# jinlinyi/PerspectiveFields

Hardware: NVIDIA H100
Metric: images/sec at 640x480 (Paramnet-360Cities-edina), H100 vs ref CPU (higher is better)
Workload: dtype f32 via 3x bf16 split MMA, fp32 accumulate

## Files before the change

### include/pf_b200.h

```cpp
#ifndef PF_B200_H_
#define PF_B200_H_

#include <stddef.h>
#include <stdint.h>

#ifdef __cplusplus
extern "C" {
#endif

#define PF_ABI_VERSION 2

typedef struct pf_engine* pf_handle;

enum pf_status { PF_OK = 0, PF_ERR_ARG = -1, PF_ERR_CUDA = -2, PF_ERR_WEIGHT = -3, PF_ERR_WORKSPACE = -4 };

enum pf_dtype { PF_F32 = 0, PF_BF16 = 1 };

enum pf_param_net { PF_PARAM_NONE = 0, PF_PARAM_CENTERED = 1 , PF_PARAM_UNCENTERED = 2  };

typedef struct pf_model_desc {
  int gravity_classes;
  int latitude_classes;
  int param_net;
  int param_input_size;
  float pixel_mean[3];
  float pixel_std[3];
} pf_model_desc;

typedef struct pf_batch {
  int n;
  const uint8_t* images_u8;
  const int64_t* image_offset;
  const float* images_chw;
  const int32_t* height;
  const int32_t* width;
  float* pred_gravity;
  float* pred_latitude;
  float* gravity_original;
  const int64_t* gravity_original_offset;
  float* latitude_original;
  const int64_t* latitude_original_offset;
  float* params;
} pf_batch;

int pf_abi_version(void);
const char* pf_last_error(void);

int64_t pf_kernel_launch_count(void);

int pf_create(int device, const pf_model_desc* desc, pf_handle* out);
int pf_destroy(pf_handle h);

int pf_set_weight(pf_handle h, const char* name, const void* dev_ptr, int64_t numel, int dtype);
int pf_finalize(pf_handle h);

int64_t pf_workspace_bytes(pf_handle h, int n, int max_h);

int pf_forward(pf_handle h, const pf_batch* batch, void* workspace, int64_t workspace_bytes, void* stream);

int pf_profile_enable(pf_handle h, int on );
int pf_profile_read(pf_handle h, double* out21);
int pf_profile_kernels_enable(pf_handle h, int max_launches);
int pf_profile_kernels_read(pf_handle h, char* buf, int cap);

int pf_set_option(pf_handle h, const char* name, int value);

int pf_debug_enable(pf_handle h, int on);
int pf_debug_count(pf_handle h);
const char* pf_debug_name(pf_handle h, int i);
int64_t pf_debug_numel(pf_handle h, const char* name);
int pf_debug_copy(pf_handle h, const char* name, float* dst_dev, int64_t numel, void* stream);

typedef struct pf_camera {
  int32_t height, width;
  double focal_rel;
  double elevation, roll;
  double cx_rel, cy_rel;
  int64_t up_offset;
  int64_t lat_offset;
} pf_camera;
int pf_camera_fields(int device, const pf_camera* cams, int n, float* up, float* lat, void* stream);

typedef struct pf_comm* pf_comm_handle;
int pf_comm_unique_id(void* id128);
int pf_comm_create(int device, int rank, int nranks, const void* id128, pf_comm_handle* out);
int pf_comm_destroy(pf_comm_handle c);
int pf_gather(pf_comm_handle c, int root, int count, void* const* dev_ptrs, const int64_t* bytes, const int32_t* peer, void* stream);

typedef struct pf_jpeg* pf_jpeg_handle;
int pf_jpeg_create(int device, int max_threads , pf_jpeg_handle* out);
int pf_jpeg_destroy(pf_jpeg_handle j);
int pf_jpeg_info(pf_jpeg_handle j, const uint8_t* data, int64_t length, int32_t* height, int32_t* width);
int pf_jpeg_decode_batch(pf_jpeg_handle j, int n, const uint8_t* const* data, const int64_t* length, const int32_t* height,
                         const int32_t* width, uint8_t* blob, const int64_t* offset, void* stream);


int pf_op_conv_gemm(const float* x, int B, int H, int W, int Cin, const void* whi, const void* wlo, const float* bias,
                    int N, int KH, int KW, int stride, int pad, int in_relu, int act, const float* res, int res_relu,
                    float* y, void* stream);
typedef struct pf_tma_pred { const float* w; const float* b; float* out; int nc, mode; } pf_tma_pred;
typedef struct pf_tma_op {
  int mode;
  int64_t M; int K;
  int B, H, W, Cin;
  int N, groups;
  const void* a_hi; const void* a_lo; int lda, a_c0, a_gc;
  const void* a2_hi; const void* a2_lo; int lda2, c_split, a2_c0;
  const void* w_hi; const void* w_lo; const float* bias; int bias_mode, bias_gstride;
  int act; const float* gamma;
  const float* res; int ldr, r_coff, r_gcoff, res_relu;
  const float* res2; int ldr2, r2_coff, r2_gcoff;
  float* C; int ldc, c_coff, c_gcoff;
  void* s_hi; void* s_lo; int lds, s_coff, s_gcoff, split_relu;
  int phase4;
  int npred; pf_tma_pred pred[2];
  int force_bn, force_kb;
  int picked_bn, picked_kb;
} pf_tma_op;
int pf_op_tma(pf_tma_op* op, void* stream);
int pf_op_conv1_ring(const void* c_hi, const void* c_lo, int B, int H, int W, const float* wf, const float* bias, float* out,
                     const float* pg_w, const float* pg_b, float* pg_out, const float* pl_w, const float* pl_b, float* pl_out, void* stream);
int pf_tma_pick_tile(int mode, int64_t M, int N, int K, int sm_count, int* bn, int* kb);
int pf_op_layernorm(const float* x, float* y, int64_t rows, int C, const float* w, const float* b, float eps, void* stream);
int pf_op_attention(const float* q, const float* kv, float* out, int B, int N, int C, int heads, void* stream);
int pf_op_attention_mma(const float* q, const float* kv, float* out, int B, int N, int C, int heads, void* stream);
int pf_op_attention_tc(const float* q, const float* kv, float* out, int B, int N, int C, int heads, void* stream);
int pf_op_dwconv3x3_gelu(const float* x, float* y, int B, int H, int W, int C, const float* w9c, const float* bias, void* stream);
int pf_op_dwconv7x7(const float* x, float* y, int B, int H, int W, int C, const float* w49c, const float* bias, void* stream);
int pf_op_upsample2x(const float* x, float* y, int B, int H, int W, int C, void* stream);
int pf_op_preprocess(const uint8_t* img_dev, int H, int W, const float* mean3, const float* std3, float* y, void* stream);
int pf_op_resize_u8(const uint8_t* img_dev, int H, int W, int new_h, int new_w, uint8_t* out_dev, void* stream);
int pf_op_resize_f32(const float* img_dev, int H, int W, int C, int new_h, int new_w, float* out_dev, void* stream);
int pf_op_fill_stream(float* dst, int64_t numel, float value, void* stream);
int pf_op_argmax_decode(const float* logits, float* field, int B, int HW, int NC, int is_gravity, void* stream);
int pf_op_pred_argmax_decode(const float* feat, int ld, int coff, const float* w, const float* bias, float* field, int B, int HW, int NC,
                             int is_gravity, void* stream);
int pf_op_postprocess(const float* vec, const float* lat, int n, const int32_t* height, const int32_t* width,
                      float* gravity_original, const int64_t* gravity_original_offset, float* latitude_original,
                      const int64_t* latitude_original_offset, int lat_is_sin, void* stream);

#ifdef __cplusplus
}
#endif
#endif
```

### perspectivefields_b200/_native.py

```python
import ctypes
import os
import subprocess

_HERE = os.path.dirname(os.path.abspath(__file__))
ROOT = os.path.dirname(_HERE)
LIB_PATH = os.path.join(_HERE, "libpf_b200.so")
SRC_DIR = os.path.join(_HERE, "csrc")
HEADER = os.path.join(ROOT, "include", "pf_b200.h")

PF_F32, PF_BF16 = 0, 1
PF_PARAM_NONE, PF_PARAM_CENTERED, PF_PARAM_UNCENTERED = 0, 1, 2

NVCC_FLAGS = ["-gencode", "arch=compute_90a,code=sm_90a", "-O3", "-lineinfo", "-std=c++17",
              "-Xcompiler", "-fPIC", "-shared", "-ldl"]


class pf_model_desc(ctypes.Structure):
    _fields_ = [("gravity_classes", ctypes.c_int), ("latitude_classes", ctypes.c_int), ("param_net", ctypes.c_int),
                ("param_input_size", ctypes.c_int), ("pixel_mean", ctypes.c_float * 3), ("pixel_std", ctypes.c_float * 3)]


class pf_camera(ctypes.Structure):
    _fields_ = [("height", ctypes.c_int32), ("width", ctypes.c_int32), ("focal_rel", ctypes.c_double), ("elevation", ctypes.c_double),
                ("roll", ctypes.c_double), ("cx_rel", ctypes.c_double), ("cy_rel", ctypes.c_double),
                ("up_offset", ctypes.c_int64), ("lat_offset", ctypes.c_int64)]


class pf_batch(ctypes.Structure):
    _fields_ = [("n", ctypes.c_int),
                ("images_u8", ctypes.c_void_p), ("image_offset", ctypes.POINTER(ctypes.c_int64)),
                ("images_chw", ctypes.c_void_p),
                ("height", ctypes.POINTER(ctypes.c_int32)), ("width", ctypes.POINTER(ctypes.c_int32)),
                ("pred_gravity", ctypes.c_void_p), ("pred_latitude", ctypes.c_void_p),
                ("gravity_original", ctypes.c_void_p), ("gravity_original_offset", ctypes.POINTER(ctypes.c_int64)),
                ("latitude_original", ctypes.c_void_p), ("latitude_original_offset", ctypes.POINTER(ctypes.c_int64)),
                ("params", ctypes.c_void_p)]


class pf_tma_pred(ctypes.Structure):
    _fields_ = [("w", ctypes.c_void_p), ("b", ctypes.c_void_p), ("out", ctypes.c_void_p), ("nc", ctypes.c_int), ("mode", ctypes.c_int)]


def _fields(spec):
    types = {"int": ctypes.c_int, "ptr": ctypes.c_void_p, "i64": ctypes.c_int64}
    out = []
    for decl in spec.split(";"):
        t, names = decl.split(None, 1)
        out += [(n.strip(), types[t]) for n in names.split(",")]
    return out


class pf_tma_op(ctypes.Structure):
    _fields_ = _fields("int mode; i64 M; int K, B, H, W, Cin, N, groups; ptr a_hi, a_lo; int lda, a_c0, a_gc; ptr a2_hi, a2_lo;"
                       "int lda2, c_split, a2_c0; ptr w_hi, w_lo, bias; int bias_mode, bias_gstride, act; ptr gamma, res;"
                       "int ldr, r_coff, r_gcoff, res_relu; ptr res2; int ldr2, r2_coff, r2_gcoff; ptr C; int ldc, c_coff, c_gcoff;"
                       "ptr s_hi, s_lo; int lds, s_coff, s_gcoff, split_relu, phase4, npred") + \
        [("pred", pf_tma_pred * 2)] + _fields("int force_bn, force_kb, picked_bn, picked_kb")


def _sources():
    return sorted(os.path.join(SRC_DIR, f) for f in os.listdir(SRC_DIR) if f.endswith((".cu", ".cuh"))) + [HEADER]


def needs_build():
    if not os.path.exists(LIB_PATH):
        return True
    t = os.path.getmtime(LIB_PATH)
    return any(os.path.getmtime(s) > t for s in _sources())


def build(force=False, verbose=False):
    if not force and not needs_build():
        return LIB_PATH
    nvcc = os.environ.get("NVCC", "/usr/local/cuda/bin/nvcc")
    cmd = [nvcc] + NVCC_FLAGS + [os.path.join(SRC_DIR, "pf_b200.cu"), "-o", LIB_PATH + ".tmp"]
    if verbose:
        cmd.insert(1, "-Xptxas=-v")
    r = subprocess.run(cmd, capture_output=True, text=True)
    if r.returncode != 0:
        raise RuntimeError("nvcc failed:\n" + " ".join(cmd) + "\n" + r.stdout + r.stderr)
    os.replace(LIB_PATH + ".tmp", LIB_PATH)
    if verbose:
        print(r.stderr)
    return LIB_PATH


_lib = None


def lib():
    global _lib
    if _lib is not None:
        return _lib
    if not os.path.exists(LIB_PATH):
        raise RuntimeError(f"{LIB_PATH} is missing: run `python -c 'import __graft_entry__ as g; g.build()'` "
                           "(perspectivefields_b200 has no CPU or PyTorch fallback)")
    L = ctypes.CDLL(os.environ.get("PF_B200_LIB") or LIB_PATH)
    vp, i32, i64, f32 = ctypes.c_void_p, ctypes.c_int, ctypes.c_int64, ctypes.c_float
    sig = {
        "pf_abi_version": (i32, []),
        "pf_last_error": (ctypes.c_char_p, []),
        "pf_kernel_launch_count": (i64, []),
        "pf_create": (i32, [i32, ctypes.POINTER(pf_model_desc), ctypes.POINTER(vp)]),
        "pf_destroy": (i32, [vp]),
        "pf_set_weight": (i32, [vp, ctypes.c_char_p, vp, i64, i32]),
        "pf_finalize": (i32, [vp]),
        "pf_workspace_bytes": (i64, [vp, i32, i32]),
        "pf_forward": (i32, [vp, ctypes.POINTER(pf_batch), vp, i64, vp]),
        "pf_profile_enable": (i32, [vp, i32]),
        "pf_profile_read": (i32, [vp, ctypes.POINTER(ctypes.c_double)]),
        "pf_profile_kernels_enable": (i32, [vp, i32]),
        "pf_profile_kernels_read": (i32, [vp, ctypes.c_char_p, i32]),
        "pf_debug_enable": (i32, [vp, i32]),
        "pf_debug_count": (i32, [vp]),
        "pf_debug_name": (ctypes.c_char_p, [vp, i32]),
        "pf_debug_numel": (i64, [vp, ctypes.c_char_p]),
        "pf_debug_copy": (i32, [vp, ctypes.c_char_p, vp, i64, vp]),
        "pf_op_conv_gemm": (i32, [vp, i32, i32, i32, i32, vp, vp, vp, i32, i32, i32, i32, i32, i32, i32, vp, i32, vp, vp]),
        "pf_op_tma": (i32, [ctypes.POINTER(pf_tma_op), vp]),
        "pf_op_conv1_ring": (i32, [vp, vp, i32, i32, i32, vp, vp, vp, vp, vp, vp, vp, vp, vp, vp]),
        "pf_tma_pick_tile": (i32, [i32, i64, i32, i32, i32, ctypes.POINTER(i32), ctypes.POINTER(i32)]),
        "pf_set_option": (i32, [vp, ctypes.c_char_p, i32]),
        "pf_camera_fields": (i32, [i32, ctypes.POINTER(pf_camera), i32, vp, vp, vp]),
        "pf_op_layernorm": (i32, [vp, vp, i64, i32, vp, vp, f32, vp]),
        "pf_op_attention": (i32, [vp, vp, vp, i32, i32, i32, i32, vp]),
        "pf_op_attention_mma": (i32, [vp, vp, vp, i32, i32, i32, i32, vp]),
        "pf_op_attention_tc": (i32, [vp, vp, vp, i32, i32, i32, i32, vp]),
        "pf_op_dwconv3x3_gelu": (i32, [vp, vp, i32, i32, i32, i32, vp, vp, vp]),
        "pf_op_dwconv7x7": (i32, [vp, vp, i32, i32, i32, i32, vp, vp, vp]),
        "pf_op_upsample2x": (i32, [vp, vp, i32, i32, i32, i32, vp]),
        "pf_op_preprocess": (i32, [vp, i32, i32, ctypes.POINTER(f32), ctypes.POINTER(f32), vp, vp]),
        "pf_op_resize_u8": (i32, [vp, i32, i32, i32, i32, vp, vp]),
        "pf_op_resize_f32": (i32, [vp, i32, i32, i32, i32, i32, vp, vp]),
        "pf_op_argmax_decode": (i32, [vp, vp, i32, i32, i32, i32, vp]),
        "pf_op_fill_stream": (i32, [vp, i64, f32, vp]),
        "pf_op_pred_argmax_decode": (i32, [vp, i32, i32, vp, vp, vp, i32, i32, i32, i32, vp]),
        "pf_op_postprocess": (i32, [vp, vp, i32, ctypes.POINTER(ctypes.c_int32), ctypes.POINTER(ctypes.c_int32), vp, ctypes.POINTER(i64), vp,
                                    ctypes.POINTER(i64), i32, vp]),
        "pf_comm_unique_id": (i32, [vp]),
        "pf_comm_create": (i32, [i32, i32, i32, vp, ctypes.POINTER(vp)]),
        "pf_comm_destroy": (i32, [vp]),
        "pf_gather": (i32, [vp, i32, i32, ctypes.POINTER(vp), ctypes.POINTER(i64), ctypes.POINTER(ctypes.c_int32), vp]),
        "pf_jpeg_create": (i32, [i32, i32, ctypes.POINTER(vp)]),
        "pf_jpeg_destroy": (i32, [vp]),
        "pf_jpeg_info": (i32, [vp, vp, i64, ctypes.POINTER(ctypes.c_int32), ctypes.POINTER(ctypes.c_int32)]),
        "pf_jpeg_decode_batch": (i32, [vp, i32, ctypes.POINTER(vp), ctypes.POINTER(i64), ctypes.POINTER(ctypes.c_int32),
                                       ctypes.POINTER(ctypes.c_int32), vp, ctypes.POINTER(i64), vp]),
    }
    for name, (res, args) in sig.items():
        try:
            fn = getattr(L, name)
        except AttributeError:
            if os.environ.get("PF_B200_LIB"):
                continue
            raise
        fn.restype, fn.argtypes = res, args
    if L.pf_abi_version() != 2:
        raise RuntimeError("libpf_b200.so ABI version mismatch")
    _lib = L
    return L


EXPORTS = ["pf_abi_version", "pf_last_error", "pf_kernel_launch_count", "pf_create", "pf_destroy", "pf_set_weight",
           "pf_finalize", "pf_workspace_bytes", "pf_forward", "pf_profile_enable", "pf_profile_read", "pf_profile_kernels_enable",
           "pf_profile_kernels_read", "pf_set_option", "pf_debug_enable", "pf_debug_count", "pf_debug_name", "pf_debug_numel",
           "pf_debug_copy", "pf_camera_fields", "pf_comm_unique_id", "pf_comm_create", "pf_comm_destroy", "pf_gather",
           "pf_jpeg_create", "pf_jpeg_destroy", "pf_jpeg_info", "pf_jpeg_decode_batch",
           "pf_op_conv_gemm", "pf_op_tma", "pf_op_conv1_ring", "pf_tma_pick_tile", "pf_op_layernorm", "pf_op_attention", "pf_op_attention_mma", "pf_op_attention_tc", "pf_op_dwconv3x3_gelu", "pf_op_dwconv7x7",
           "pf_op_upsample2x", "pf_op_preprocess", "pf_op_fill_stream", "pf_op_resize_u8", "pf_op_resize_f32", "pf_op_argmax_decode",
           "pf_op_pred_argmax_decode", "pf_op_postprocess"]


class PfError(RuntimeError):
    pass


def check(status):
    if status < 0:
        raise PfError(f"libpf_b200: {lib().pf_last_error().decode()} (status {status})")
    return status
```

### perspectivefields_b200/csrc/gemm_tma.cuh

```cuda
#pragma once
#include <cuda.h>

#include "tc_ptx.cuh"

namespace pf {

constexpr int MODE_GEMM = 0, MODE_HALO = 1;
constexpr int kTmaThreads = 384;
constexpr int kHaloBytes = 180 * 128;

struct TmaGemmParams {
  int M;
  int B, H, W;
  int Cin;
  int N, K;
  int a_c0, a_gc;
  int c_split, a2_c0;
  int groups;
  int b_row0;
  const float* bias; int bias_mode, bias_gstride;
  int act; const float* gamma;
  const float* res;  int ldr, r_coff, r_gcoff, res_relu;
  const float* res2; int ldr2, r2_coff, r2_gcoff;
  float* C; int ldc, c_coff, c_gcoff;
  __nv_bfloat16* Shi; __nv_bfloat16* Slo; int lds, s_coff, s_gcoff, split_relu;
  const float* pred_w; const float* pred_b; float* pred_out; int pred_nc, pred_mode;
  int phase4;
};

template <int BN, int MODE, int KB> struct TmaCfg {
  static_assert(KB == 32 || KB == 64, "KB");
  static_assert(BN % 32 == 0 && BN <= 256, "BN");
  static constexpr int kBPlane = BN * KB * 2;
  static constexpr int kAPlane = 128 * KB * 2;
  static constexpr int kStage = (MODE == MODE_GEMM ? 2 * kAPlane : 0) + 2 * kBPlane;
  static constexpr int kABuf = 2 * kHtPlaneBytes;
  static constexpr int kAccPitch = 68;
  static constexpr int kAccStage = 2 * 64 * kAccPitch * 4;
  static constexpr int kBudget = 225 * 1024 - kAccStage - (MODE == MODE_HALO ? 2 * kABuf : 0);
  static constexpr int kStagesRaw = kBudget / kStage;
  static constexpr int kStages = kStagesRaw > 16 ? 16 : kStagesRaw;
  static constexpr int kSmemBytes = (MODE == MODE_HALO ? 2 * kABuf : 0) + kStages * kStage + kAccStage + 512 + 1024;
  static_assert(kStages >= 2, "ring too shallow");
  static_assert(kSmemBytes <= 227 * 1024, "shared memory per block");
};

__device__ __forceinline__ void mbar_expect_tx(uint32_t bar, uint32_t bytes) {
  asm volatile("mbarrier.arrive.expect_tx.shared::cta.b64 _, [%0], %1;\n" ::"r"(bar), "r"(bytes) : "memory");
}
__device__ __forceinline__ void tma_load_2d(uint32_t dst, const CUtensorMap* map, uint32_t bar, int c0, int c1) {
  asm volatile("cp.async.bulk.tensor.2d.shared::cluster.global.mbarrier::complete_tx::bytes [%0], [%1, {%3, %4}], [%2];\n"
               ::"r"(dst), "l"(reinterpret_cast<uint64_t>(map)), "r"(bar), "r"(c0), "r"(c1) : "memory");
}
__device__ __forceinline__ void tma_load_4d(uint32_t dst, const CUtensorMap* map, uint32_t bar, int c0, int c1, int c2, int c3) {
  asm volatile("cp.async.bulk.tensor.4d.shared::cluster.global.mbarrier::complete_tx::bytes [%0], [%1, {%3, %4, %5, %6}], [%2];\n"
               ::"r"(dst), "l"(reinterpret_cast<uint64_t>(map)), "r"(bar), "r"(c0), "r"(c1), "r"(c2), "r"(c3) : "memory");
}
__device__ __forceinline__ void tma_prefetch_desc(const CUtensorMap* map) {
  asm volatile("prefetch.tensormap [%0];\n" ::"l"(reinterpret_cast<uint64_t>(map)) : "memory");
}

struct TmaMaps {
  CUtensorMap a_hi, a_lo, a2_hi, a2_lo, b_hi, b_lo;
};

template <int BN, int MODE, int KB>
__global__ void __launch_bounds__(kTmaThreads, 1) gemm_tma_kernel(const __grid_constant__ TmaMaps maps, const TmaGemmParams p, int tiles_x, int tiles_y) {
  using Cfg = TmaCfg<BN, MODE, KB>;
  constexpr int NS = Cfg::kStages;
  constexpr int SPC = 9 * (64 / KB);
  constexpr int kConsumerWarps = 8;
  extern __shared__ unsigned char smem_dyn[];
  const uint32_t raw = smem_u32(smem_dyn);
  const uint32_t sbase = (raw + 1023u) & ~1023u;
  unsigned char* sm = smem_dyn + (sbase - raw);
  const uint32_t a_base = sbase;
  const uint32_t ring = sbase + (MODE == MODE_HALO ? 2 * Cfg::kABuf : 0);
  const uint32_t acc_base = ring + NS * Cfg::kStage;
  const uint32_t bars = acc_base + Cfg::kAccStage;
  auto full_b = [&](int s) { return bars + 8u * s; };
  auto empty_b = [&](int s) { return bars + 8u * (NS + s); };
  auto full_a = [&](int i) { return bars + 8u * (2 * NS + i); };
  auto empty_a = [&](int i) { return bars + 8u * (2 * NS + 2 + i); };

  const int tid = threadIdx.x, lane = tid & 31, warp = tid >> 5;
  const int n_tiles = cdiv(p.N, BN);
  const int m_tiles = MODE == MODE_GEMM ? cdiv(p.M, 128) : p.B * tiles_x * tiles_y;
  const int total_tiles = m_tiles * n_tiles * p.groups;
  const int nchunks = MODE == MODE_HALO ? p.Cin / 64 : 0;
  const int nk = MODE == MODE_GEMM ? p.K / KB : nchunks * SPC;
  const bool b_resident = MODE == MODE_HALO && nchunks == 1 && SPC <= NS;

  if (tid == 0) {
    tma_prefetch_desc(&maps.a_hi); tma_prefetch_desc(&maps.a_lo); tma_prefetch_desc(&maps.b_hi); tma_prefetch_desc(&maps.b_lo);
    for (int s = 0; s < NS; ++s) { mbar_init(full_b(s), 1); mbar_init(empty_b(s), kConsumerWarps); }
    for (int i = 0; i < 2; ++i) { mbar_init(full_a(i), 1); mbar_init(empty_a(i), kConsumerWarps); }
    fence_mbar_init();
  }
  __syncthreads();
  pdl_wait();
  pdl_launch();

  auto decode = [&](int tile, int& mt, int& g, int& n0) {
    n0 = (tile % n_tiles) * BN;
    tile /= n_tiles;
    g = tile % p.groups;
    mt = tile / p.groups;
  };

  if (warp < 4) {
    asm volatile("setmaxnreg.dec.sync.aligned.u32 40;\n");
    if (warp == 0 && lane == 0) {
      int it = 0;
      for (int tile = blockIdx.x; tile < total_tiles; tile += gridDim.x) {
        int mt, g, n0;
        decode(tile, mt, g, n0);
        const int brow = p.b_row0 + g * p.N + n0;
        if (b_resident && it > 0) break;
        for (int kc = 0; kc < nk; ++kc, ++it) {
          const int s = it % NS;
          mbar_wait(empty_b(s), ((it / NS) & 1) ^ 1);
          mbar_expect_tx(full_b(s), Cfg::kStage);
          const uint32_t st = ring + s * Cfg::kStage;
          int kcol;
          if (MODE == MODE_GEMM) {
            kcol = kc * KB;
            tma_load_2d(st, &maps.a_hi, full_b(s), p.a_c0 + g * p.a_gc + kcol, mt * 128);
            tma_load_2d(st + Cfg::kAPlane, &maps.a_lo, full_b(s), p.a_c0 + g * p.a_gc + kcol, mt * 128);
          } else {
            const int c = kc / SPC, u = kc - c * SPC;
            kcol = KB == 32 ? (u >> 1) * p.Cin + c * 64 + (u & 1) * 32 : u * p.Cin + c * 64;
          }
          const uint32_t bdst = st + (MODE == MODE_GEMM ? 2 * Cfg::kAPlane : 0);
          tma_load_2d(bdst, &maps.b_hi, full_b(s), kcol, brow);
          tma_load_2d(bdst + Cfg::kBPlane, &maps.b_lo, full_b(s), kcol, brow);
        }
      }
    } else if (MODE == MODE_HALO && warp == 1 && lane == 0) {
      int ita = 0;
      for (int tile = blockIdx.x; tile < total_tiles; tile += gridDim.x) {
        int mt, g, n0;
        decode(tile, mt, g, n0);
        const int tx = mt % tiles_x, ty = (mt / tiles_x) % tiles_y, bimg = mt / (tiles_x * tiles_y);
        for (int c = 0; c < nchunks; ++c, ++ita) {
          const int buf = ita & 1;
          mbar_wait(empty_a(buf), ((ita >> 1) & 1) ^ 1);
          mbar_expect_tx(full_a(buf), 2 * kHaloBytes);
          const uint32_t dst = a_base + buf * Cfg::kABuf;
          const int ci = c * 64;
          if (p.c_split > 0 && ci >= p.c_split) {
            tma_load_4d(dst, &maps.a2_hi, full_a(buf), p.a2_c0 + ci - p.c_split, tx * kHtTileW - 1, ty * kHtTileH - 1, bimg);
            tma_load_4d(dst + kHtPlaneBytes, &maps.a2_lo, full_a(buf), p.a2_c0 + ci - p.c_split, tx * kHtTileW - 1, ty * kHtTileH - 1, bimg);
          } else {
            tma_load_4d(dst, &maps.a_hi, full_a(buf), p.a_c0 + g * p.a_gc + ci, tx * kHtTileW - 1, ty * kHtTileH - 1, bimg);
            tma_load_4d(dst + kHtPlaneBytes, &maps.a_lo, full_a(buf), p.a_c0 + g * p.a_gc + ci, tx * kHtTileW - 1, ty * kHtTileH - 1, bimg);
          }
        }
      }
    }
    return;
  }

  asm volatile("setmaxnreg.inc.sync.aligned.u32 232;\n");
  const int wg = (warp >> 2) - 1;
  const int wt = tid & 127;
  float* stage = reinterpret_cast<float*>(sm + (acc_base - sbase)) + wg * 64 * Cfg::kAccPitch;
  const int erow = wt & 63, eh = wt >> 6;
  const int r = wg * 64 + erow;
  float acc[BN / 2];
  int it = 0, ita = 0;
  for (int tile = blockIdx.x, tl = 0; tile < total_tiles; tile += gridDim.x, ++tl) {
    int mt, g, n0;
    decode(tile, mt, g, n0);
    int prev_s = -1, prev_buf = -1;
    fence_regs(acc);
    for (int kc = 0; kc < nk; ++kc, ++it) {
      const int s = it % NS;
      uint32_t a_hi, a_lo;
      bool chunk_end = false;
      int buf = 0;
      if (MODE == MODE_HALO) {
        const int c = kc / SPC, u = kc - c * SPC;
        const int tap = KB == 32 ? (u >> 1) : u, ky = tap / 3, kx = tap - ky * 3;
        buf = ita & 1;
        if (u == 0) mbar_wait(full_a(buf), (ita >> 1) & 1);
        a_hi = a_base + buf * Cfg::kABuf + ((ky + 8 * wg) * kHtHaloW + kx) * 128 + (KB == 32 ? (u & 1) * 64 : 0);
        a_lo = a_hi + kHtPlaneBytes;
        chunk_end = u == SPC - 1;
      } else {
        a_hi = ring + s * Cfg::kStage + wg * 64 * KB * 2;
        a_lo = a_hi + Cfg::kAPlane;
      }
      const int sb = b_resident ? kc : s;
      if (!b_resident || tl == 0) mbar_wait(full_b(sb), b_resident ? 0 : ((it / NS) & 1));
      const uint32_t b_hi = ring + sb * Cfg::kStage + (MODE == MODE_GEMM ? 2 * Cfg::kAPlane : 0);
      const uint64_t dah = MODE == MODE_HALO ? ht_a_desc(a_hi) : wgmma_tile_desc<KB>(a_hi);
      const uint64_t dal = MODE == MODE_HALO ? ht_a_desc(a_lo) : wgmma_tile_desc<KB>(a_lo);
      const uint64_t dbh = wgmma_tile_desc<KB>(b_hi);
      const uint64_t dbl = wgmma_tile_desc<KB>(b_hi + Cfg::kBPlane);
      constexpr uint64_t kChunk = (uint64_t)(64 * KB * 2) >> 4;
      wgmma_fence();
#pragma unroll
      for (int kk = 0; kk < KB / 16; ++kk) {
        const uint32_t first = (kc | kk) ? 1u : 0u;
#pragma unroll
        for (int j = 0; j < BN / 64; ++j) {
          wgmma_n64(acc + 32 * j, dal + 2 * kk, dbh + 2 * kk + j * kChunk, first);
          wgmma_n64(acc + 32 * j, dah + 2 * kk, dbl + 2 * kk + j * kChunk, 1u);
          wgmma_n64(acc + 32 * j, dah + 2 * kk, dbh + 2 * kk + j * kChunk, 1u);
        }
        if constexpr (BN % 64 != 0) {
          constexpr int j = BN / 64;
          wgmma_n32(acc + 32 * j, dal + 2 * kk, dbh + 2 * kk + j * kChunk, first);
          wgmma_n32(acc + 32 * j, dah + 2 * kk, dbl + 2 * kk + j * kChunk, 1u);
          wgmma_n32(acc + 32 * j, dah + 2 * kk, dbh + 2 * kk + j * kChunk, 1u);
        }
      }
      wgmma_commit();
      wgmma_wait<1>();
      if (lane == 0 && prev_s >= 0) {
        if (!b_resident) mbar_arrive(empty_b(prev_s));
        if (MODE == MODE_HALO && prev_buf >= 0) mbar_arrive(empty_a(prev_buf));
      }
      prev_s = s;
      prev_buf = chunk_end ? buf : -1;
      if (MODE == MODE_HALO && chunk_end) ++ita;
    }
    wgmma_wait<0>();
    fence_regs(acc);
    if (lane == 0 && prev_s >= 0) {
      if (!b_resident) mbar_arrive(empty_b(prev_s));
      if (MODE == MODE_HALO && prev_buf >= 0) mbar_arrive(empty_a(prev_buf));
    }

    long long m;
    bool valid;
    int cls_off = 0;
    int bimg = 0, oy = 0, ox = 0;
    if (MODE == MODE_GEMM) {
      m = (long long)mt * 128 + r;
      valid = m < p.M;
    } else {
      const int tx = mt % tiles_x, ty = (mt / tiles_x) % tiles_y;
      bimg = mt / (tiles_x * tiles_y);
      oy = ty * kHtTileH + (r >> 3); ox = tx * kHtTileW + (r & 7);
      valid = oy < p.H && ox < p.W;
      m = ((long long)bimg * p.H + oy) * p.W + ox;
      if (p.bias_mode == 2) {
        const int ry = oy == 0 ? 0 : (oy == p.H - 1 ? 2 : 1);
        const int rx = ox == 0 ? 0 : (ox == p.W - 1 ? 2 : 1);
        cls_off = (ry * 3 + rx) * p.N;
      }
    }
    const float* __restrict__ bias = p.bias ? p.bias + (long long)g * p.bias_gstride : nullptr;
    const int frow = (wt >> 5) * 16 + (lane >> 2), fcol = 2 * (lane & 3);
#pragma unroll
    for (int rd = 0; rd < (BN + 63) / 64; ++rd) {
      named_bar_sync(1 + wg, 128);
#pragma unroll
      for (int jb = 0; jb < 8; ++jb) {
        const int cb = rd * 8 + jb;
        if (cb < BN / 8) {
          float* d0 = stage + frow * Cfg::kAccPitch + jb * 8 + fcol;
          *reinterpret_cast<float2*>(d0) = make_float2(acc[4 * cb], acc[4 * cb + 1]);
          *reinterpret_cast<float2*>(d0 + 8 * Cfg::kAccPitch) = make_float2(acc[4 * cb + 2], acc[4 * cb + 3]);
        }
      }
      named_bar_sync(1 + wg, 128);
      const int ch = 2 * rd + eh;
      if (ch >= BN / 32) continue;
      const int nb = n0 + ch * 32;
      const bool ph4 = MODE == MODE_HALO && BN == 128 && p.phase4;
      const long long mo = ph4 ? ((long long)bimg * 2 * p.H + 2 * oy + (ch >> 1)) * (2 * p.W) + 2 * ox + (ch & 1) : m;
      const int nbo = ph4 ? 0 : nb;
      const bool chunk_ok = nb < p.N;
      float o[32];
      const float* srow = stage + erow * Cfg::kAccPitch + eh * 32;
#pragma unroll
      for (int j = 0; j < 32; j += 4) {
        const float4 t = *reinterpret_cast<const float4*>(srow + j);
        o[j] = t.x; o[j + 1] = t.y; o[j + 2] = t.z; o[j + 3] = t.w;
      }
      if (valid && chunk_ok) {
        if (p.bias_mode) {
#pragma unroll
          for (int j = 0; j < 32; j += 4) {
            const float4 bv = __ldg(reinterpret_cast<const float4*>(bias + cls_off + nb + j));
            o[j] += bv.x; o[j + 1] += bv.y; o[j + 2] += bv.z; o[j + 3] += bv.w;
          }
        }
        if (p.act == 1) {
#pragma unroll
          for (int j = 0; j < 32; ++j) o[j] = fmaxf(o[j], 0.f);
        } else if (p.act == 2) {
#pragma unroll
          for (int j = 0; j < 32; ++j) o[j] = gelu_erf(o[j]);
        }
        if (p.gamma) {
#pragma unroll
          for (int j = 0; j < 32; j += 4) {
            const float4 gv = __ldg(reinterpret_cast<const float4*>(p.gamma + nb + j));
            o[j] *= gv.x; o[j + 1] *= gv.y; o[j + 2] *= gv.z; o[j + 3] *= gv.w;
          }
        }
        if (p.res) {
          const float* rp = p.res + m * p.ldr + p.r_coff + g * p.r_gcoff + nb;
#pragma unroll
          for (int j = 0; j < 32; j += 4) {
            float4 rv = *reinterpret_cast<const float4*>(rp + j);
            if (p.res_relu) { rv.x = fmaxf(rv.x, 0.f); rv.y = fmaxf(rv.y, 0.f); rv.z = fmaxf(rv.z, 0.f); rv.w = fmaxf(rv.w, 0.f); }
            o[j] += rv.x; o[j + 1] += rv.y; o[j + 2] += rv.z; o[j + 3] += rv.w;
          }
        }
        if (p.res2) {
          const float* rp = p.res2 + m * p.ldr2 + p.r2_coff + g * p.r2_gcoff + nb;
#pragma unroll
          for (int j = 0; j < 32; j += 4) {
            const float4 rv = *reinterpret_cast<const float4*>(rp + j);
            o[j] += rv.x; o[j + 1] += rv.y; o[j + 2] += rv.z; o[j + 3] += rv.w;
          }
        }
        if (MODE == MODE_HALO && (BN == 32 || BN == 128) && p.pred_w) {
          float v0 = __ldg(p.pred_b), v1 = p.pred_nc > 1 ? __ldg(p.pred_b + 1) : 0.f;
#pragma unroll
          for (int j = 0; j < 32; j += 4) {
            const float4 w0 = __ldg(reinterpret_cast<const float4*>(p.pred_w + j));
            v0 = fmaf(o[j], w0.x, v0); v0 = fmaf(o[j + 1], w0.y, v0); v0 = fmaf(o[j + 2], w0.z, v0); v0 = fmaf(o[j + 3], w0.w, v0);
            if (p.pred_nc > 1) {
              const float4 w1 = __ldg(reinterpret_cast<const float4*>(p.pred_w + 32 + j));
              v1 = fmaf(o[j], w1.x, v1); v1 = fmaf(o[j + 1], w1.y, v1); v1 = fmaf(o[j + 2], w1.z, v1); v1 = fmaf(o[j + 3], w1.w, v1);
            }
          }
          const long long HWl = (long long)p.H * p.W * (ph4 ? 4 : 1);
          const long long bi = mo / HWl, pix = mo - bi * HWl;
          float* po = p.pred_out + bi * p.pred_nc * HWl + pix;
          if (p.pred_mode == 1) {
            const float nrm = fmaxf(sqrtf(v0 * v0 + v1 * v1), 1e-12f);
            po[0] = v0 / nrm; po[HWl] = v1 / nrm;
          } else {
            po[0] = fminf(fmaxf(v0, -1.f), 1.f);
          }
        }
      }
      if (chunk_ok && (p.C || p.Shi)) {
        const bool odd = lane & 1;
        const bool valid_p = __shfl_xor_sync(0xffffffffu, (int)valid, 1) != 0;
        const long long mo_p = mo + (odd ? -1 : 1) * (ph4 ? 2 : 1);
        const long long moA = odd ? mo_p : mo, moB = odd ? mo : mo_p;
        const bool vA = odd ? valid_p : valid, vB = odd ? valid : valid_p;
        if (p.C) {
          float* cA = p.C + moA * p.ldc + p.c_coff + g * p.c_gcoff + nbo + (odd ? 4 : 0);
          float* cB = p.C + moB * p.ldc + p.c_coff + g * p.c_gcoff + nbo + (odd ? 4 : 0);
#pragma unroll
          for (int t = 0; t < 4; ++t) {
            float k[4], rr[4];
#pragma unroll
            for (int e = 0; e < 4; ++e) {
              k[e] = odd ? o[8 * t + 4 + e] : o[8 * t + e];
              rr[e] = __shfl_xor_sync(0xffffffffu, odd ? o[8 * t + e] : o[8 * t + 4 + e], 1);
            }
            if (vA) *reinterpret_cast<float4*>(cA + 8 * t) = odd ? make_float4(rr[0], rr[1], rr[2], rr[3]) : make_float4(k[0], k[1], k[2], k[3]);
            if (vB) *reinterpret_cast<float4*>(cB + 8 * t) = odd ? make_float4(k[0], k[1], k[2], k[3]) : make_float4(rr[0], rr[1], rr[2], rr[3]);
          }
        }
        if (p.Shi) {
          const long long sA = moA * p.lds + p.s_coff + g * p.s_gcoff + nbo + (odd ? 8 : 0);
          const long long sB = moB * p.lds + p.s_coff + g * p.s_gcoff + nbo + (odd ? 8 : 0);
#pragma unroll
          for (int t = 0; t < 2; ++t) {
            float k[8], rr[8];
#pragma unroll
            for (int e = 0; e < 8; ++e) {
              const float mine = odd ? o[16 * t + 8 + e] : o[16 * t + e], give = odd ? o[16 * t + e] : o[16 * t + 8 + e];
              k[e] = p.split_relu ? fmaxf(mine, 0.f) : mine;
              rr[e] = __shfl_xor_sync(0xffffffffu, p.split_relu ? fmaxf(give, 0.f) : give, 1);
            }
            uint4 kh, kl, rh, rl;
            split_bf16x2(k[0], k[1], kh.x, kl.x); split_bf16x2(k[2], k[3], kh.y, kl.y);
            split_bf16x2(k[4], k[5], kh.z, kl.z); split_bf16x2(k[6], k[7], kh.w, kl.w);
            split_bf16x2(rr[0], rr[1], rh.x, rl.x); split_bf16x2(rr[2], rr[3], rh.y, rl.y);
            split_bf16x2(rr[4], rr[5], rh.z, rl.z); split_bf16x2(rr[6], rr[7], rh.w, rl.w);
            if (vA) {
              *reinterpret_cast<uint4*>(p.Shi + sA + 16 * t) = odd ? rh : kh;
              *reinterpret_cast<uint4*>(p.Slo + sA + 16 * t) = odd ? rl : kl;
            }
            if (vB) {
              *reinterpret_cast<uint4*>(p.Shi + sB + 16 * t) = odd ? kh : rh;
              *reinterpret_cast<uint4*>(p.Slo + sB + 16 * t) = odd ? kl : rl;
            }
          }
        }
      }
    }
  }
}

}
```

### perspectivefields_b200/csrc/pf_b200.cu

```cuda
#include "../../include/pf_b200.h"

#include <cuda_runtime.h>
#include <nvtx3/nvToolsExt.h>

#include <atomic>
#include <cctype>
#include <cmath>
#include <cstdarg>
#include <cstdio>
#include <cstdlib>
#include <cstring>
#include <map>
#include <mutex>
#include <string>
#include <functional>
#include <unordered_map>
#include <vector>

#include "common.cuh"
#include "tma_host.cuh"
#include "attention_mma.cuh"
#include "layers.cuh"
#include "prepost.cuh"
#include "comm.cuh"
#include "jpeg.cuh"

using namespace pf;

static thread_local std::string g_err;
static std::atomic<long long> g_launches{0};

static int fail(int code, const char* fmt, ...) {
  char buf[1024];
  va_list ap;
  va_start(ap, fmt);
  vsnprintf(buf, sizeof(buf), fmt, ap);
  va_end(ap);
  g_err = buf;
  return code;
}
#define CU(expr)                                                                                    \
  do {                                                                                              \
    cudaError_t e__ = (expr);                                                                       \
    if (e__ != cudaSuccess) return fail(PF_ERR_CUDA, "%s: %s (%s:%d)", #expr, cudaGetErrorString(e__), __FILE__, __LINE__); \
  } while (0)
static char g_crumb[96] = "";
static bool sync_debug() {
  static int v = -1;
  if (v < 0) v = getenv("PF_SYNC_DEBUG") ? 1 : 0;
  return v == 1;
}
struct KernelProf {
  bool on = false;
  cudaStream_t st = nullptr;
  std::vector<cudaEvent_t> pool;
  size_t used = 0;
  struct Rec { const char* expr; cudaEvent_t a, b; };
  std::vector<Rec> recs;
  cudaEvent_t next() { return used < pool.size() ? pool[used++] : nullptr; }
};
static thread_local KernelProf* tl_kp = nullptr;
#define LAUNCHED(expr)                                                                              \
  do {                                                                                              \
    KernelProf* kp__ = tl_kp;                                                                       \
    cudaEvent_t ka__ = (kp__ && kp__->on) ? kp__->next() : nullptr;                                 \
    if (ka__) cudaEventRecord(ka__, kp__->st);                                                      \
    cudaError_t e__ = (expr);                                                                       \
    g_launches.fetch_add(1, std::memory_order_relaxed);                                             \
    if (ka__) {                                                                                     \
      cudaEvent_t kb__ = kp__->next();                                                              \
      if (kb__) { cudaEventRecord(kb__, kp__->st); kp__->recs.push_back({#expr, ka__, kb__}); }     \
    }                                                                                               \
    if (e__ == cudaSuccess && sync_debug()) e__ = cudaDeviceSynchronize();                          \
    if (e__ != cudaSuccess) return fail(PF_ERR_CUDA, "%s: %s (%s:%d, after tap '%s')", #expr, cudaGetErrorString(e__), __FILE__, __LINE__, g_crumb); \
  } while (0)
struct NvtxRange {
  explicit NvtxRange(const char* name) { nvtxRangePushA(name); }
  ~NvtxRange() { nvtxRangePop(); }
};
#define TRY(expr)                \
  do {                           \
    int r__ = (expr);            \
    if (r__ != PF_OK) return r__; \
  } while (0)

static const int kMitDims[4] = {64, 128, 320, 512};
static const int kMitHeads[4] = {1, 2, 5, 8};
static const int kMitDepths[4] = {3, 4, 18, 3};
static const int kMitSr[4] = {8, 4, 2, 1};
static const int kMitRes[4] = {80, 40, 20, 10};
static const int kCnxDims[4] = {96, 192, 384, 768};
static const int kCnxDepths[4] = {3, 3, 9, 3};

struct WeightRef { const void* p; long long numel; int dtype; };
struct GemmW { const __nv_bfloat16* hi = nullptr; const __nv_bfloat16* lo = nullptr; const float* b = nullptr; };
struct LnW { const float* w = nullptr; const float* b = nullptr; };

struct MitBlockW { LnW ln1, srln, ln2; GemmW q, sr, kv, proj, fc1, fc2; const float* dw_w; const float* dw_b; };
struct CnxBlockW { const float* dw_w; const float* dw_b; LnW ln; GemmW pw1, pw2; const float* gamma; };

struct Arena {
  char* base = nullptr;
  long long cap = 0, off = 0, peak = 0;
  bool dry = false, keep = false;
  void* alloc(long long bytes) {
    off = (off + 255) & ~255LL;
    void* p = dry ? nullptr : base + off;
    off += bytes;
    if (off > peak) peak = off;
    return p;
  }
  float* f(long long n) { return (float*)alloc(n * 4); }
  long long mark() const { return off; }
  void release(long long m) { if (!keep) off = m; }
};

struct pf_engine {
  int device = 0;
  pf_model_desc desc{};
  bool finalized = false;
  std::unordered_map<std::string, WeightRef> weights;
  const float *embed1_w, *embed1_b, *llenc_w, *llenc_b;
  LnW embed_ln[4], stage_norm[4];
  GemmW embed[4];
  GemmW embed1g, llencg;
  std::vector<MitBlockW> blocks[4];
  GemmW proc[4];
  GemmW rcu[4][2][2];
  GemmW conv0, conv1;
  GemmW conv1p;
  const float *conv1f_w, *conv1f_b;
  bool use_fork = false;
  cudaStream_t side = nullptr;
  cudaEvent_t ev_fork = nullptr, ev_join = nullptr;
  bool use_dwln = false;
  bool use_pdl = true;
  bool decode_only = false;
  bool use_attn_split = true;
  bool use_phase = true;
  const float *pred_g_w, *pred_g_b, *pred_l_w, *pred_l_b;
  const float *pn_stem_w, *pn_stem_b;
  LnW pn_stem_ln, pn_ds_ln[4], pn_norm;
  GemmW pn_ds[4];
  std::vector<CnxBlockW> pn_blocks[4];
  const float *pn_head_w, *pn_head_b;
  struct DevTable { int ksize; int* bounds; int* coeffs; };
  std::map<int, DevTable> tables;
  char* table_dev = nullptr;
  char* table_host = nullptr;
  long long table_off = 0;
  KernelProf kp;
  struct MapKey {
    const void* base; long long d0, d1, d2; int kind, box, kb;
    bool operator==(const MapKey& o) const { return base == o.base && d0 == o.d0 && d1 == o.d1 && d2 == o.d2 && kind == o.kind && box == o.box && kb == o.kb; }
  };
  struct MapKeyHash {
    size_t operator()(const MapKey& k) const {
      size_t h = std::hash<const void*>()(k.base);
      for (long long v : {k.d0, k.d1, k.d2, (long long)k.kind, (long long)k.box, (long long)k.kb}) h = h * 1000003u ^ std::hash<long long>()(v);
      return h;
    }
  };
  std::unordered_map<MapKey, CUtensorMap, MapKeyHash> map_cache;
  bool use_stem_tc = true;
  bool use_attn_mma = true;
  int sm_count = 132;
  bool profile = false;
  struct ProfRec { cudaEvent_t a, b; double flops; int cfg; int M, N, K, KH, stride, groups, Cin; };
  std::vector<ProfRec> prof;
  std::vector<cudaEvent_t> ev_pool;
  bool debug = false;
  std::vector<std::pair<std::string, std::pair<const float*, long long>>> taps;
};

static int get_w(pf_engine* e, const std::string& name, int dtype, long long numel, const void** out) {
  auto it = e->weights.find(name);
  if (it == e->weights.end()) return fail(PF_ERR_WEIGHT, "missing weight '%s'", name.c_str());
  if (it->second.dtype != dtype) return fail(PF_ERR_WEIGHT, "weight '%s': wrong dtype", name.c_str());
  if (it->second.numel != numel) return fail(PF_ERR_WEIGHT, "weight '%s': numel %lld, expected %lld", name.c_str(), it->second.numel, numel);
  *out = it->second.p;
  return PF_OK;
}
static int get_f(pf_engine* e, const std::string& n, long long numel, const float** out) { return get_w(e, n, PF_F32, numel, (const void**)out); }
static int get_gemm(pf_engine* e, const std::string& n, long long N, long long K, long long nbias, GemmW* g, int groups = 1) {
  TRY(get_w(e, n + ".whi", PF_BF16, groups * N * K, (const void**)&g->hi));
  TRY(get_w(e, n + ".wlo", PF_BF16, groups * N * K, (const void**)&g->lo));
  TRY(get_f(e, n + ".b", groups * nbias, &g->b));
  return PF_OK;
}
static int get_ln(pf_engine* e, const std::string& n, int C, LnW* l) {
  TRY(get_f(e, n + ".w", C, &l->w));
  TRY(get_f(e, n + ".b", C, &l->b));
  return PF_OK;
}

static int resolve_weights(pf_engine* e) {
  char nm[128];
  TRY(get_f(e, "embed1.w", 147 * 64, &e->embed1_w));
  TRY(get_f(e, "embed1.b", 64, &e->embed1_b));
  TRY(get_f(e, "llenc.w", 147 * 64, &e->llenc_w));
  TRY(get_f(e, "llenc.b", 64, &e->llenc_b));
  TRY(get_gemm(e, "embed1g", 64, 160, 64, &e->embed1g));
  TRY(get_gemm(e, "llencg", 64, 160, 64, &e->llencg));
  for (int s = 0; s < 4; ++s) {
    const int C = kMitDims[s];
    snprintf(nm, sizeof nm, "embed%d.ln", s + 1);
    TRY(get_ln(e, nm, C, &e->embed_ln[s]));
    if (s > 0) {
      snprintf(nm, sizeof nm, "embed%d", s + 1);
      TRY(get_gemm(e, nm, C, 9LL * kMitDims[s - 1], C, &e->embed[s]));
    }
    e->blocks[s].resize(kMitDepths[s]);
    for (int i = 0; i < kMitDepths[s]; ++i) {
      MitBlockW& b = e->blocks[s][i];
      char p[64];
      snprintf(p, sizeof p, "s%d.b%d.", s + 1, i);
      std::string P(p);
      TRY(get_ln(e, P + "ln1", C, &b.ln1));
      TRY(get_gemm(e, P + "q", C, C, C, &b.q));
      if (kMitSr[s] > 1) {
        TRY(get_gemm(e, P + "sr", C, (long long)kMitSr[s] * kMitSr[s] * C, C, &b.sr));
        TRY(get_ln(e, P + "srln", C, &b.srln));
      }
      TRY(get_gemm(e, P + "kv", 2 * C, C, 2 * C, &b.kv));
      TRY(get_gemm(e, P + "proj", C, C, C, &b.proj));
      TRY(get_ln(e, P + "ln2", C, &b.ln2));
      TRY(get_gemm(e, P + "fc1", 4 * C, C, 4 * C, &b.fc1));
      TRY(get_f(e, P + "dw.w", 9LL * 4 * C, &b.dw_w));
      TRY(get_f(e, P + "dw.b", 4 * C, &b.dw_b));
      TRY(get_gemm(e, P + "fc2", C, 4 * C, C, &b.fc2));
    }
    snprintf(nm, sizeof nm, "s%d.norm", s + 1);
    TRY(get_ln(e, nm, C, &e->stage_norm[s]));
  }
  for (int l = 0; l < 4; ++l) {
    snprintf(nm, sizeof nm, "head.proc%d", l + 1);
    TRY(get_gemm(e, nm, 512, 9LL * kMitDims[l], 9 * 512, &e->proc[l]));
  }
  for (int f = 0; f < 4; ++f)
    for (int u = 0; u < 2; ++u) {
      if (f == 3 && u == 0) continue;
      for (int c = 0; c < 2; ++c) {
        snprintf(nm, sizeof nm, "head.f%d.u%d.c%d", f + 1, u + 1, c + 1);
        TRY(get_gemm(e, nm, 256, 2304, 256, &e->rcu[f][u][c], 2));
      }
    }
  TRY(get_gemm(e, "head.conv0", 64, 9 * 320, 64, &e->conv0, 2));
  TRY(get_gemm(e, "head.conv1", 32, 9 * 64, 32, &e->conv1, 2));
  TRY(get_gemm(e, "head.conv1p", 128, 9 * 64, 128, &e->conv1p, 2));
  TRY(get_f(e, "head.conv1f.w", 2LL * 9 * 64 * 32, &e->conv1f_w));
  TRY(get_f(e, "head.conv1f.b", 64, &e->conv1f_b));
  TRY(get_f(e, "head.pred_g.w", 32LL * e->desc.gravity_classes, &e->pred_g_w));
  TRY(get_f(e, "head.pred_g.b", e->desc.gravity_classes, &e->pred_g_b));
  TRY(get_f(e, "head.pred_l.w", 32LL * e->desc.latitude_classes, &e->pred_l_w));
  TRY(get_f(e, "head.pred_l.b", e->desc.latitude_classes, &e->pred_l_b));
  if (e->desc.param_net != PF_PARAM_NONE) {
    TRY(get_f(e, "pn.stem.w", 48 * 96, &e->pn_stem_w));
    TRY(get_f(e, "pn.stem.b", 96, &e->pn_stem_b));
    TRY(get_ln(e, "pn.stem.ln", 96, &e->pn_stem_ln));
    for (int k = 1; k < 4; ++k) {
      snprintf(nm, sizeof nm, "pn.ds%d.ln", k);
      TRY(get_ln(e, nm, kCnxDims[k - 1], &e->pn_ds_ln[k]));
      snprintf(nm, sizeof nm, "pn.ds%d", k);
      TRY(get_gemm(e, nm, kCnxDims[k], 4LL * kCnxDims[k - 1], kCnxDims[k], &e->pn_ds[k]));
    }
    for (int s = 0; s < 4; ++s) {
      const int C = kCnxDims[s];
      e->pn_blocks[s].resize(kCnxDepths[s]);
      for (int j = 0; j < kCnxDepths[s]; ++j) {
        CnxBlockW& b = e->pn_blocks[s][j];
        char p[64];
        snprintf(p, sizeof p, "pn.s%d.b%d.", s, j);
        std::string P(p);
        TRY(get_f(e, P + "dw.w", 49LL * C, &b.dw_w));
        TRY(get_f(e, P + "dw.b", C, &b.dw_b));
        TRY(get_ln(e, P + "ln", C, &b.ln));
        TRY(get_gemm(e, P + "pw1", 4 * C, C, 4 * C, &b.pw1));
        TRY(get_gemm(e, P + "pw2", C, 4 * C, C, &b.pw2));
        TRY(get_f(e, P + "gamma", C, &b.gamma));
      }
    }
    TRY(get_ln(e, "pn.norm", 768, &e->pn_norm));
    TRY(get_f(e, "pn.head.w", 5 * 768, &e->pn_head_w));
    TRY(get_f(e, "pn.head.b", 5, &e->pn_head_b));
  }
  return PF_OK;
}

struct Fwd {
  pf_engine* e;
  Arena ar;
  cudaStream_t st;
  bool dry;
  int n;

  int tap(const char* name, const float* p, long long numel) {
    if (!e->debug) return PF_OK;
    float* cp = ar.f(numel);
    if (dry) return PF_OK;
    snprintf(g_crumb, sizeof g_crumb, "%s", name);
    if (sync_debug()) fprintf(stderr, "[pf tap] %s cp=%p (+%lld of cap %lld) p=%p numel=%lld\n", name, (void*)cp, (long long)((char*)cp - ar.base), ar.cap, (const void*)p, numel);
    CU(cudaMemcpyAsync(cp, p, numel * 4, cudaMemcpyDeviceToDevice, st));
    if (sync_debug()) CU(cudaDeviceSynchronize());
    e->taps.push_back({name, {cp, numel}});
    return PF_OK;
  }
  int tapf(const float* p, long long numel, const char* fmt, ...) {
    if (!e->debug) return PF_OK;
    char buf[96];
    va_list ap;
    va_start(ap, fmt);
    vsnprintf(buf, sizeof buf, fmt, ap);
    va_end(ap);
    return tap(buf, p, numel);
  }

  SplitT salloc(long long pixels, int ld) {
    SplitT t;
    t.hi = (__nv_bfloat16*)ar.alloc(pixels * ld * 2);
    t.lo = (__nv_bfloat16*)ar.alloc(pixels * ld * 2);
    t.ld = ld;
    return t;
  }
  int tap_split(const char* name, const SplitT& t, long long numel) {
    if (!e->debug) return PF_OK;
    float* cp = ar.f(numel);
    if (dry) return PF_OK;
    snprintf(g_crumb, sizeof g_crumb, "%s", name);
    LAUNCHED((merge_split_kernel<<<(unsigned)cdivl(numel, 256), 256, 0, st>>>(t.hi, t.lo, cp, numel), cudaGetLastError()));
    e->taps.push_back({name, {cp, numel}});
    return PF_OK;
  }
  static cudaError_t gemm_tma_gemm_mode(const TmaMaps& maps, const TmaGemmParams& p, int bn, int kb, int sms, cudaStream_t st, const PredTail* pred) {
    return gemm_tma_launch(MODE_GEMM, maps, p, bn, kb, sms, st, pred);
  }
  static cudaError_t gemm_tma_halo_mode(const TmaMaps& maps, const TmaGemmParams& p, int bn, int kb, int sms, cudaStream_t st, const PredTail* pred) {
    return gemm_tma_launch(MODE_HALO, maps, p, bn, kb, sms, st, pred);
  }
  int force_bn = 0, force_kb = 0;
  int picked_bn = 0, picked_kb = 0;
  int pick_tile(int mode, const TmaGemmParams& p, const PredTail* pred, int& bn, int& kb) {
    tma_pick_tile(mode, p.M, p.N, p.K, e->sm_count, bn, kb);
    if (force_bn) { bn = force_bn; kb = tma_pick_kb(bn, p.K, mode); }
    if (force_kb) kb = force_kb;
    if (const char* msg = gemm_tma_check(mode, p, bn, kb, pred != nullptr)) return fail(PF_ERR_ARG, "TMA engine, %s (bn %d, kb %d): %s", mode == MODE_GEMM ? "GEMM mode" : "halo mode", bn, kb, msg);
    picked_bn = bn; picked_kb = kb;
    return PF_OK;
  }
  int launch_tma(int mode, const TmaMaps& maps, const TmaGemmParams& p, int bn, int kb, const PredTail* pred = nullptr) {
    if (e->profile) {
      pf_engine::ProfRec r{};
      for (cudaEvent_t* ev : {&r.a, &r.b}) {
        if (e->ev_pool.empty()) { CU(cudaEventCreate(ev)); }
        else { *ev = e->ev_pool.back(); e->ev_pool.pop_back(); }
      }
      const double Mrows = mode == MODE_GEMM ? (double)p.M : (double)p.B * p.H * p.W;
      r.flops = 2.0 * Mrows * (double)p.N * (double)p.K * (double)p.groups;
      r.cfg = mode == MODE_GEMM ? 5 : 6;
      r.M = (int)Mrows; r.N = p.N; r.K = p.K; r.KH = mode == MODE_GEMM ? 1 : 3; r.stride = 1; r.groups = p.groups; r.Cin = p.Cin;
      CU(cudaEventRecord(r.a, st));
      if (mode == MODE_GEMM) LAUNCHED(gemm_tma_gemm_mode(maps, p, bn, kb, e->sm_count, st, pred));
      else LAUNCHED(gemm_tma_halo_mode(maps, p, bn, kb, e->sm_count, st, pred));
      CU(cudaEventRecord(r.b, st));
      e->prof.push_back(r);
      return PF_OK;
    }
    if (mode == MODE_GEMM) LAUNCHED(gemm_tma_gemm_mode(maps, p, bn, kb, e->sm_count, st, pred));
    else LAUNCHED(gemm_tma_halo_mode(maps, p, bn, kb, e->sm_count, st, pred));
    return PF_OK;
  }
  struct Epi {
    float* C = nullptr; int ldc = 0, c_coff = 0, c_gcoff = 0;
    SplitT S; int s_coff = 0, s_gcoff = 0, split_relu = 0;
    int act = 0; const float* gamma = nullptr;
    const float* res = nullptr; int ldr = 0, r_coff = 0, r_gcoff = 0, res_relu = 0;
    const float* res2 = nullptr; int ldr2 = 0, r2_coff = 0, r2_gcoff = 0;
    int bias_mode = 1;
    int phase4 = 0;
  };
  static void fill_epi(TmaGemmParams& p, const GemmW& w, const Epi& o, int bias_gstride) {
    p.bias = w.b; p.bias_mode = w.b ? o.bias_mode : 0; p.bias_gstride = bias_gstride;
    p.act = o.act; p.gamma = o.gamma;
    p.res = o.res; p.ldr = o.ldr; p.r_coff = o.r_coff; p.r_gcoff = o.r_gcoff; p.res_relu = o.res_relu;
    p.res2 = o.res2; p.ldr2 = o.ldr2; p.r2_coff = o.r2_coff; p.r2_gcoff = o.r2_gcoff;
    p.C = o.C; p.ldc = o.ldc; p.c_coff = o.c_coff; p.c_gcoff = o.c_gcoff;
    p.Shi = o.S.hi; p.Slo = o.S.lo; p.lds = o.S.ld; p.s_coff = o.s_coff; p.s_gcoff = o.s_gcoff; p.split_relu = o.split_relu;
    p.phase4 = o.phase4;
  }
  template <class F>
  const char* cached_map(CUtensorMap* out, const pf_engine::MapKey& key, F&& make) {
    auto it = e->map_cache.find(key);
    if (it != e->map_cache.end()) { *out = it->second; return nullptr; }
    const char* msg = make(out);
    if (!msg) {
      if (e->map_cache.size() > 20000) e->map_cache.clear();
      e->map_cache.emplace(key, *out);
    }
    return msg;
  }
  const char* map2d(CUtensorMap* m, const void* base, long long cols, long long rows, long long ld, int box_rows, int kb) {
    return cached_map(m, pf_engine::MapKey{base, cols, rows, ld, 0, box_rows, kb}, [&](CUtensorMap* o) { return tma_map_2d(o, base, cols, rows, ld, box_rows, kb); });
  }
  const char* map_halo(CUtensorMap* m, const void* base, int B, int H, int W, int ld) {
    return cached_map(m, pf_engine::MapKey{base, ((long long)B << 32) | (unsigned)H, W, ld, 3, 0, 0}, [&](CUtensorMap* o) { return tma_map_halo(o, base, B, H, W, ld); });
  }
  int tgemm(const SplitT& A, long long M, int K, int a_c0, const GemmW& w, int N, const Epi& o) {
    if (dry) return PF_OK;
    if (K % 32 || N % 32 || A.ld % 8) return fail(PF_ERR_ARG, "tgemm: K/N must be multiples of 32");
    if (o.res2 || o.bias_mode == 2) return fail(PF_ERR_ARG, "tgemm: second residual / border-class bias are halo-mode features");
    TmaGemmParams p{};
    p.M = (int)M; p.Cin = K; p.N = N; p.K = K; p.a_c0 = a_c0; p.groups = 1;
    fill_epi(p, w, o, 0);
    TmaMaps maps{};
    int bn, kb;
    TRY(pick_tile(MODE_GEMM, p, nullptr, bn, kb));
    const char* msg = nullptr;
    if (!msg) msg = map2d(&maps.a_hi, A.hi, A.ld, M, A.ld, 128, kb);
    if (!msg) msg = map2d(&maps.a_lo, A.lo, A.ld, M, A.ld, 128, kb);
    if (!msg) msg = map2d(&maps.b_hi, w.hi, K, N, K, bn, kb);
    if (!msg) msg = map2d(&maps.b_lo, w.lo, K, N, K, bn, kb);
    if (msg) return fail(PF_ERR_CUDA, "%s", msg);
    maps.a2_hi = maps.a_hi; maps.a2_lo = maps.a_lo;
    return launch_tma(MODE_GEMM, maps, p, bn, kb);
  }
  int thalo(const SplitT& A, int a_c0, int a_gc, const SplitT* A2, int c_split, int a2_c0, int B, int H, int W, int Cin, const GemmW& w, int N,
            int groups, int bias_gstride, const Epi& o, const PredTail* pred = nullptr) {
    if (dry) return PF_OK;
    if (Cin % 64 || N % 32 || (A2 && c_split % 64)) return fail(PF_ERR_ARG, "thalo: Cin must be a multiple of 64, N of 32");
    if (w.b && o.bias_mode == 2 && (H < 2 || W < 2)) return fail(PF_ERR_ARG, "thalo: border-class bias needs H, W >= 2 (got %dx%d)", H, W);
    TmaGemmParams p{};
    p.B = B; p.H = H; p.W = W; p.Cin = Cin; p.N = N; p.K = 9 * Cin; p.a_c0 = a_c0; p.a_gc = a_gc; p.groups = groups;
    p.c_split = A2 ? c_split : 0; p.a2_c0 = a2_c0;
    fill_epi(p, w, o, bias_gstride);
    TmaMaps maps{};
    int bn, kb;
    TRY(pick_tile(MODE_HALO, p, pred, bn, kb));
    const char* msg = nullptr;
    if (!msg) msg = map_halo(&maps.a_hi, A.hi, B, H, W, A.ld);
    if (!msg) msg = map_halo(&maps.a_lo, A.lo, B, H, W, A.ld);
    if (A2) {
      if (!msg) msg = map_halo(&maps.a2_hi, A2->hi, B, H, W, A2->ld);
      if (!msg) msg = map_halo(&maps.a2_lo, A2->lo, B, H, W, A2->ld);
    } else { maps.a2_hi = maps.a_hi; maps.a2_lo = maps.a_lo; }
    if (!msg) msg = map2d(&maps.b_hi, w.hi, p.K, (long long)groups * N, p.K, bn, kb);
    if (!msg) msg = map2d(&maps.b_lo, w.lo, p.K, (long long)groups * N, p.K, bn, kb);
    if (msg) return fail(PF_ERR_CUDA, "%s", msg);
    return launch_tma(MODE_HALO, maps, p, bn, kb, pred);
  }
  int tconv_gather(const SplitT& A, int B, int H, int W, int Cin, int KH, int stride, int pad, const GemmW& w, int N, const Epi& o) {
    const int OH = (H + 2 * pad - KH) / stride + 1, OW = (W + 2 * pad - KH) / stride + 1;
    const long long M = (long long)B * OH * OW;
    const int K = KH * KH * Cin;
    const long long m = ar.mark();
    SplitT col = salloc(M, K);
    if (!dry) {
      if (Cin % 8) return fail(PF_ERR_ARG, "tconv_gather: Cin %% 8");
      LAUNCHED(launch_pdl(im2col_split_kernel, dim3(ew_grid(M * K / 8)), dim3(256), 0, st, A.hi, A.lo, A.ld, col.hi, col.lo, B, H, W, Cin, OH, OW, KH, stride, pad));
    }
    int r = tgemm(col, M, K, 0, w, N, o);
    ar.release(m);
    return r;
  }
  int ln_split(const float* x, const SplitT& y, long long rows, int C, const LnW& w, float eps, float* yf = nullptr) {
    if (dry) return PF_OK;
    LAUNCHED(layernorm_launch(x, yf, rows, C, w.w, w.b, eps, st, y));
    return PF_OK;
  }
  int ln_split_patch(const float* x, const SplitT& y, const SplitT& patch, long long rows, int C, const LnW& w, float eps, int R, int sr) {
    if (dry) return PF_OK;
    LAUNCHED(layernorm_launch(x, nullptr, rows, C, w.w, w.b, eps, st, y, patch, R, sr));
    return PF_OK;
  }
  int ln(const float* x, float* y, long long rows, int C, const LnW& w, float eps) {
    if (dry) return PF_OK;
    LAUNCHED(layernorm_launch(x, y, rows, C, w.w, w.b, eps, st));
    return PF_OK;
  }
};

constexpr long long kTableSlabBytes = 8LL << 20;
static int get_table(pf_engine* e, int in_size, pf_engine::DevTable* out, cudaStream_t st) {
  auto it = e->tables.find(in_size);
  if (it == e->tables.end()) {
    ResampleTable t = make_resample_table(in_size, kNet);
    const long long nb = (long long)t.bounds.size() * sizeof(int), nc = (long long)t.coeffs.size() * sizeof(int);
    const long long need = ((nb + 255) & ~255LL) + ((nc + 255) & ~255LL);
    if (need > kTableSlabBytes) return fail(PF_ERR_ARG, "image axis of %d pixels is too long for the resize tables", in_size);
    if (e->table_off + need > kTableSlabBytes) {
      CU(cudaStreamSynchronize(st));
      e->tables.clear();
      e->table_off = 0;
    }
    pf_engine::DevTable d{};
    d.ksize = t.ksize;
    const long long o0 = e->table_off, o1 = o0 + ((nb + 255) & ~255LL);
    memcpy(e->table_host + o0, t.bounds.data(), nb);
    memcpy(e->table_host + o1, t.coeffs.data(), nc);
    d.bounds = (int*)(e->table_dev + o0);
    d.coeffs = (int*)(e->table_dev + o1);
    CU(cudaMemcpyAsync(e->table_dev + o0, e->table_host + o0, need, cudaMemcpyHostToDevice, st));
    e->table_off += need;
    it = e->tables.emplace(in_size, d).first;
  }
  *out = it->second;
  return PF_OK;
}

static int pre_rows_needed(int H) {
  const double scale = (double)H / kNet;
  const double support = scale < 1.0 ? 1.0 : scale;
  return (int)(kPreRows * scale) + 2 * (int)ceil(support) + 3;
}
constexpr int kPreMaxSmemRows = 200 * 1024 / (kNet * 3);

static int fwd_preprocess(Fwd& F, const pf_batch* bt, float*& x0, PreImage*& d_pre, PostImage*& d_post) {
  pf_engine* e = F.e;
  const pf_model_desc& D = e->desc;
  const int n = F.n;
  const bool dry = F.dry;
  cudaStream_t st = F.st;
  Arena& ar = F.ar;
  x0 = ar.f((long long)n * kNet * kNet * 4);
  d_pre = (PreImage*)ar.alloc((long long)n * sizeof(PreImage));
  d_post = (PostImage*)ar.alloc((long long)n * sizeof(PostImage));
  if (!dry) {
    if (bt->images_u8) {
      std::vector<PreImage> pre(n);
      int max_h = 1;
      for (int i = 0; i < n; ++i) {
        const int H = bt->height[i], W = bt->width[i];
        if (H < 1 || W < 1) return fail(PF_ERR_ARG, "image %d has size %dx%d", i, H, W);
        pf_engine::DevTable tx, ty;
        TRY(get_table(e, W, &tx, st));
        TRY(get_table(e, H, &ty, st));
        if (ty.ksize + 1 > kPreMaxSmemRows) return fail(PF_ERR_ARG, "image %d is too tall (%d rows) for the resize kernel", i, H);
        pre[i] = PreImage{bt->image_offset[i], H, W, tx.ksize, ty.ksize, tx.bounds, tx.coeffs, ty.bounds, ty.coeffs};
        if (H > max_h) max_h = H;
      }
      CU(cudaMemcpyAsync(d_pre, pre.data(), n * sizeof(PreImage), cudaMemcpyHostToDevice, st));
      int rows = pre_rows_needed(max_h);
      if (rows > kPreMaxSmemRows) rows = kPreMaxSmemRows;
      const int smem = rows * kNet * 3;
      LAUNCHED((preprocess_kernel<<<dim3(kNet / kPreRows, n), kNet, smem, st>>>(bt->images_u8, d_pre, x0, D.pixel_mean[0], D.pixel_mean[1],
                                                                               D.pixel_mean[2], D.pixel_std[0], D.pixel_std[1], D.pixel_std[2], rows),
                cudaGetLastError()));
    } else {
      const long long total = (long long)n * kNet * kNet;
      LAUNCHED((normalize_chw_kernel<<<(unsigned)cdivl(total, 256), 256, 0, st>>>(bt->images_chw, x0, n, D.pixel_mean[0], D.pixel_mean[1],
                                                                                 D.pixel_mean[2], D.pixel_std[0], D.pixel_std[1], D.pixel_std[2]),
                cudaGetLastError()));
    }
  }
  return PF_OK;
}

static int launch_postprocess(const float* vec, const float* lat, int n, const int32_t* height, const int32_t* width, const int64_t* g_off,
                              const int64_t* l_off, float* g_out, float* l_out, int lat_is_sin, PostImage* d_post, cudaStream_t st) {
  std::vector<PostImage> post(n);
  long long total = 0;
  int max_h = 1, max_wp = 4;
  for (int i = 0; i < n; ++i) {
    if (height[i] < 1 || width[i] < 1) return fail(PF_ERR_ARG, "image %d has size %dx%d", i, height[i], width[i]);
    post[i] = PostImage{height[i], width[i], g_off[i], l_off[i], total};
    total += (long long)height[i] * width[i];
    if (height[i] > max_h) max_h = height[i];
    const int wp = (width[i] + 3) / 4 * 4;
    if (wp <= kPostMaxW && wp > max_wp) max_wp = wp;
  }
  CU(cudaMemcpyAsync(d_post, post.data(), n * sizeof(PostImage), cudaMemcpyHostToDevice, st));
  const int smem = max_wp * 8;
  LAUNCHED((postprocess_kernel<<<dim3((unsigned)cdiv(max_h, kPostBand), (unsigned)n), kPostThreads, smem, st>>>(vec, lat, d_post, g_out, l_out, lat_is_sin),
            cudaGetLastError()));
  return PF_OK;
}

static int fwd_tails_post(Fwd& F, const pf_batch* bt, const float* conv1_out, PostImage* d_post, bool pred_done = false) {
  pf_engine* e = F.e;
  const pf_model_desc& D = e->desc;
  const int n = F.n;
  const bool dry = F.dry;
  cudaStream_t st = F.st;
  Arena& ar = F.ar;
  const int HW = kNet * kNet;
  const bool cls_g = D.gravity_classes != 2, cls_l = D.latitude_classes != 1;
  const bool fused_decode = e->decode_only && (cls_g || cls_l);
  if (e->decode_only && cls_g != cls_l) return fail(PF_ERR_ARG, "decode_only needs both heads to be classification heads");
  const float* vec = dry ? nullptr : bt->pred_gravity;
  const float* lat = dry ? nullptr : bt->pred_latitude;
  if (e->debug) {
    float* rg = ar.f((long long)n * D.gravity_classes * HW);
    float* rl = ar.f((long long)n * D.latitude_classes * HW);
    if (!dry) {
      const unsigned grid = (unsigned)cdivl((long long)n * HW, 128);
      LAUNCHED((pred_tail_kernel<<<grid, 128, D.gravity_classes * 33 * 4, st>>>(conv1_out, 64, 0, e->pred_g_w, e->pred_g_b, rg, n, HW, D.gravity_classes, 0), cudaGetLastError()));
      LAUNCHED((pred_tail_kernel<<<grid, 128, D.latitude_classes * 33 * 4, st>>>(conv1_out, 64, 32, e->pred_l_w, e->pred_l_b, rl, n, HW, D.latitude_classes, 0), cudaGetLastError()));
    }
    TRY(F.tap("head.raw_g", rg, (long long)n * D.gravity_classes * HW));
    TRY(F.tap("head.raw_l", rl, (long long)n * D.latitude_classes * HW));
  }
  if (fused_decode) {
    if (!dry) {
      const unsigned grid = ew_grid((long long)n * HW * 4);
      LAUNCHED((pred_argmax_decode_kernel<<<grid, 256, D.gravity_classes * 37 * 4, st>>>(conv1_out, 64, 0, e->pred_g_w, e->pred_g_b, bt->pred_gravity, n, HW,
                                                                                      D.gravity_classes, 1), cudaGetLastError()));
      LAUNCHED((pred_argmax_decode_kernel<<<grid, 256, D.latitude_classes * 37 * 4, st>>>(conv1_out, 64, 32, e->pred_l_w, e->pred_l_b, bt->pred_latitude, n, HW,
                                                                                       D.latitude_classes, 0), cudaGetLastError()));
    }
  } else {
    if (!dry && !pred_done) {
      const unsigned grid = (unsigned)cdivl((long long)n * HW, 128);
      LAUNCHED((pred_tail_kernel<<<grid, 128, D.gravity_classes * 33 * 4, st>>>(conv1_out, 64, 0, e->pred_g_w, e->pred_g_b, bt->pred_gravity, n, HW,
                                                                             D.gravity_classes, D.gravity_classes == 2 ? 1 : 0), cudaGetLastError()));
      LAUNCHED((pred_tail_kernel<<<grid, 128, D.latitude_classes * 33 * 4, st>>>(conv1_out, 64, 32, e->pred_l_w, e->pred_l_b, bt->pred_latitude, n, HW,
                                                                              D.latitude_classes, D.latitude_classes == 1 ? 2 : 0), cudaGetLastError()));
    }
    if (cls_g) {
      float* dv = ar.f((long long)n * 2 * HW);
      if (!dry) LAUNCHED((argmax_decode_kernel<<<(unsigned)cdivl((long long)n * HW, 256), 256, 0, st>>>(bt->pred_gravity, dv, n, HW, D.gravity_classes, 1), cudaGetLastError()));
      vec = dv;
    }
    if (cls_l) {
      float* dl = ar.f((long long)n * HW);
      if (!dry) LAUNCHED((argmax_decode_kernel<<<(unsigned)cdivl((long long)n * HW, 256), 256, 0, st>>>(bt->pred_latitude, dl, n, HW, D.latitude_classes, 0), cudaGetLastError()));
      lat = dl;
    }
  }
  if (!dry)
    TRY(launch_postprocess(vec, lat, n, bt->height, bt->width, bt->gravity_original_offset, bt->latitude_original_offset, bt->gravity_original,
                           bt->latitude_original, cls_l ? 0 : 1, d_post, st));
  return PF_OK;
}

static int run_forward_tma(Fwd& F, const pf_batch* bt) {
  pf_engine* e = F.e;
  const pf_model_desc& D = e->desc;
  const int n = F.n;
  const bool dry = F.dry;
  cudaStream_t st = F.st;
  Arena& ar = F.ar;
  using Epi = Fwd::Epi;

  float* x0; PreImage* d_pre; PostImage* d_post;
  {
    NvtxRange r_("pf:preprocess");
    TRY(fwd_preprocess(F, bt, x0, d_pre, d_post));
  }
  TRY(F.tap("pre", x0, (long long)n * kNet * kNet * 4));

  NvtxRange* sect = new NvtxRange("pf:ll_enc");
  struct SectGuard { NvtxRange*& p; ~SectGuard() { delete p; } } sect_guard{sect};
  auto section = [&](const char* name) { delete sect; sect = nullptr; sect = new NvtxRange(name); };
  SplitT cfeat[4];
  for (int s = 0; s < 4; ++s) cfeat[s] = F.salloc((long long)n * kMitRes[s] * kMitRes[s], kMitDims[s]);
  SplitT ll = F.salloc((long long)n * 160 * 160, 64);
  if (e->use_stem_tc) {
    const long long m = ar.mark();
    const long long M = (long long)n * 160 * 160;
    SplitT col = F.salloc(M, 160);
    if (!dry) LAUNCHED(launch_pdl(stem_gather_kernel, dim3(ew_grid(stem_gather_threads(n, 160, 160))), dim3(256), 0, st, x0, col.hi, col.lo, n, 160, 160, 2));
    Epi o; o.S = ll; o.act = 1;
    TRY(F.tgemm(col, M, 160, 0, e->llencg, 64, o));
    ar.release(m);
  } else if (!dry) {
    LAUNCHED((stem_conv_launch<7, 7, 2, 3, 64>(x0, 4, n, kNet, kNet, e->llenc_w, e->llenc_b, nullptr, 1, st, ll)));
  }
  TRY(F.tap_split("ll", ll, (long long)n * 160 * 160 * 64));

  for (int s = 0; s < 4; ++s) {
    { char nm[32]; snprintf(nm, sizeof nm, "pf:mit.stage%d", s + 1); section(nm); }
    const int C = kMitDims[s], R = kMitRes[s], N = R * R, heads = kMitHeads[s], sr = kMitSr[s];
    const long long rows = (long long)n * N;
    const long long m = ar.mark();
    float* x = ar.f(rows * C);
    float* tf = ar.f(rows * C);
    SplitT t1 = F.salloc(rows, C);
    SplitT t1p;
    if (sr > 1) t1p = F.salloc((long long)n * 100, sr * sr * C);
    SplitT q = F.salloc(rows, C);
    SplitT a = F.salloc(rows, C);
    float* t2f = ar.f((long long)n * 100 * C);
    SplitT t2 = F.salloc((long long)n * 100, C);
    SplitT kv = F.salloc((long long)n * 100, 2 * C);
    const bool qkv_split = e->use_attn_mma && e->use_attn_split;
    float* qf = qkv_split ? nullptr : ar.f(rows * C);
    float* kvf = qkv_split ? nullptr : ar.f((long long)n * 100 * 2 * C);
    float* h1 = ar.f(rows * 4 * C);
    SplitT h2 = F.salloc(rows, 4 * C);
    if (s == 0 && e->use_stem_tc) {
      const long long mm = ar.mark();
      SplitT col = F.salloc(rows, 160);
      if (!dry) LAUNCHED(launch_pdl(stem_gather_kernel, dim3(ew_grid(stem_gather_threads(n, 80, 80))), dim3(256), 0, st, x0, col.hi, col.lo, n, 80, 80, 4));
      Epi o; o.C = tf; o.ldc = C;
      TRY(F.tgemm(col, rows, 160, 0, e->embed1g, 64, o));
      ar.release(mm);
    } else if (s == 0) {
      if (!dry) LAUNCHED((stem_conv_launch<7, 7, 4, 3, 64>(x0, 4, n, kNet, kNet, e->embed1_w, e->embed1_b, tf, 0, st)));
    } else {
      Epi o; o.C = tf; o.ldc = C;
      TRY(F.tconv_gather(cfeat[s - 1], n, kMitRes[s - 1], kMitRes[s - 1], kMitDims[s - 1], 3, 2, 1, e->embed[s], C, o));
    }
    TRY(F.ln(tf, x, rows, C, e->embed_ln[s], 1e-5f));
    TRY(F.tapf(x, rows * C, "mit.s%d.embed", s + 1));
    for (int i = 0; i < kMitDepths[s]; ++i) {
      const MitBlockW& b = e->blocks[s][i];
      if (sr > 1) TRY(F.ln_split_patch(x, t1, t1p, rows, C, b.ln1, 1e-6f, R, sr));
      else TRY(F.ln_split(x, t1, rows, C, b.ln1, 1e-6f));
      Epi oq, okv;
      if (qkv_split) { oq.S = q; okv.S = kv; } else { oq.C = qf; oq.ldc = C; okv.C = kvf; okv.ldc = 2 * C; }
      const bool fork = !dry && sr > 1 && e->use_fork && e->side && !e->kp.on && !e->profile && !sync_debug() && !e->debug;
      if (fork) {
        CU(cudaEventRecord(e->ev_fork, st));
        CU(cudaStreamWaitEvent(e->side, e->ev_fork, 0));
        F.st = e->side;
      }
      if (sr > 1) {
        { Epi o; o.C = t2f; o.ldc = C; TRY(F.tgemm(t1p, (long long)n * 100, sr * sr * C, 0, b.sr, C, o)); }
        TRY(F.ln_split(t2f, t2, (long long)n * 100, C, b.srln, 1e-5f));
        TRY(F.tgemm(t2, (long long)n * 100, C, 0, b.kv, 2 * C, okv));
      }
      if (fork) {
        CU(cudaEventRecord(e->ev_join, e->side));
        F.st = st;
      }
      TRY(F.tgemm(t1, rows, C, 0, b.q, C, oq));
      if (fork) CU(cudaStreamWaitEvent(st, e->ev_join, 0));
      if (sr > 1) {
      } else {
        TRY(F.tgemm(t1, rows, C, 0, b.kv, 2 * C, okv));
      }
      if (!dry) {
        if (qkv_split) LAUNCHED(attention_mma_launch(nullptr, nullptr, nullptr, n, N, C, heads, st, a, q, kv));
        else if (e->use_attn_mma) LAUNCHED(attention_mma_launch(qf, kvf, nullptr, n, N, C, heads, st, a));
        else LAUNCHED(attention_launch(qf, kvf, nullptr, n, N, C, heads, st, a));
      }
      { Epi o; o.C = x; o.ldc = C; o.res = x; o.ldr = C; TRY(F.tgemm(a, rows, C, 0, b.proj, C, o)); }
      TRY(F.tapf(x, rows * C, "mit.s%d.b%d.attn", s + 1, i));
      TRY(F.ln_split(x, t1, rows, C, b.ln2, 1e-6f));
      { Epi o; o.C = h1; o.ldc = 4 * C; TRY(F.tgemm(t1, rows, C, 0, b.fc1, 4 * C, o)); }
      if (!dry) LAUNCHED(launch_pdl(dwconv3x3_gelu_kernel, dim3(ew_grid((long long)n * ((R + 1) / 2) * ((R + PF_DW3_PX - 1) / PF_DW3_PX) * C)), dim3(256), 0, st, h1, nullptr, n, R, R, 4 * C, b.dw_w, b.dw_b, h2.hi, h2.lo));
      { Epi o; o.C = x; o.ldc = C; o.res = x; o.ldr = C; TRY(F.tgemm(h2, rows, 4 * C, 0, b.fc2, C, o)); }
      TRY(F.tapf(x, rows * C, "mit.s%d.b%d", s + 1, i));
    }
    TRY(F.ln_split(x, cfeat[s], rows, C, e->stage_norm[s], 1e-6f));
    { char nm[32]; snprintf(nm, sizeof nm, "mit.c%d", s + 1); TRY(F.tap_split(nm, cfeat[s], rows * C)); }
    ar.release(m);
  }

  float* conv1_out = ar.f((long long)n * kNet * kNet * 64);
  bool fuse_pred = false;
  {
    const long long m = ar.mark();
    float* fused = nullptr;
    SplitT fused_s;
    for (int lvl = 4; lvl >= 1; --lvl) {
      { char nm[32]; snprintf(nm, sizeof nm, "pf:heads.level%d", lvl); section(nm); }
      const int r = kMitRes[lvl - 1], Cin = kMitDims[lvl - 1];
      const long long px = (long long)n * r * r;
      float* t = ar.f(px * 512);
      SplitT rt = F.salloc(px, 512);
      SplitT u = F.salloc(px, 512);
      float* v = ar.f(px * 512);
      SplitT rv = F.salloc(px, 512);
      float* w2 = ar.f(px * 512);
      {
        Epi o; o.C = t; o.ldc = 512; o.S = rt; o.split_relu = 1; o.bias_mode = 2;
        TRY(F.thalo(cfeat[lvl - 1], 0, 0, nullptr, 0, 0, n, r, r, Cin, e->proc[lvl - 1], 512, 1, 0, o));
        TRY(F.tapf(t, px * 512, "head.proc%d", lvl));
      }
      auto rcu = [&](const SplitT& A, const GemmW& w, Epi o) {
        o.c_gcoff = 256; o.s_gcoff = 256; o.r_gcoff = 256; o.r2_gcoff = 256;
        return F.thalo(A, 0, 256, nullptr, 0, 0, n, r, r, 256, w, 256, 2, 256, o);
      };
      const float* of = t;
      const SplitT* os = &rt;
      if (lvl < 4) {
        { Epi o; o.S = u; o.act = 1; TRY(rcu(rt, e->rcu[lvl - 1][0][0], o)); }
        { Epi o; o.C = v; o.ldc = 512; o.S = rv; o.split_relu = 1; o.res = t; o.ldr = 512; o.res_relu = 1; o.res2 = fused; o.ldr2 = 512;
          TRY(rcu(u, e->rcu[lvl - 1][0][1], o)); }
        of = v; os = &rv;
      }
      { Epi o; o.S = u; o.act = 1; TRY(rcu(*os, e->rcu[lvl - 1][1][0], o)); }
      { Epi o; o.C = w2; o.ldc = 512; o.res = of; o.ldr = 512; o.res_relu = 1; TRY(rcu(u, e->rcu[lvl - 1][1][1], o)); }
      if (lvl > 1) {
        float* up = ar.f(px * 4 * 512);
        if (!dry) LAUNCHED(launch_pdl(upsample2x_kernel, dim3(ew_grid(upsample2x_threads(n, r, r, 512))), dim3(256), 0, st, w2, 512, 0, up, 512, 0, n, r, r, 512, nullptr, nullptr));
        fused = up;
        TRY(F.tapf(up, px * 4 * 512, "head.fusion%d", lvl));
      } else {
        fused_s = F.salloc(px * 4, 512);
        if (!dry) LAUNCHED(launch_pdl(upsample2x_kernel, dim3(ew_grid(upsample2x_threads(n, r, r, 512))), dim3(256), 0, st, w2, 512, 0, nullptr, 512, 0, n, r, r, 512, fused_s.hi, fused_s.lo));
        TRY(F.tap_split("head.fusion1", fused_s, px * 4 * 512));
      }
    }
    section("pf:heads.fuse_convs");
    fuse_pred = D.gravity_classes == 2 && D.latitude_classes == 1;
    const bool keep_conv1 = !fuse_pred || e->debug;
    PredTail pt[2] = {{e->pred_g_w, e->pred_g_b, dry ? nullptr : bt->pred_gravity, 2, 1}, {e->pred_l_w, e->pred_l_b, dry ? nullptr : bt->pred_latitude, 1, 2}};
    if (e->use_phase) {
      SplitT c0s = F.salloc((long long)n * 160 * 160, 128);
      {
        Epi o; o.S = c0s; o.s_gcoff = 64; o.act = 1;
        TRY(F.thalo(fused_s, 0, 256, &ll, 256, 0, n, 160, 160, 320, e->conv0, 64, 2, 64, o));
        TRY(F.tap_split("head.conv0", c0s, (long long)n * 160 * 160 * 128));
      }
      Epi o; o.ldc = 64; o.c_gcoff = 32; o.act = 1; o.phase4 = 1;
      if (keep_conv1) o.C = conv1_out;
      TRY(F.thalo(c0s, 0, 64, nullptr, 0, 0, n, 160, 160, 64, e->conv1p, 128, 2, 128, o, fuse_pred ? pt : nullptr));
      if (!dry) {
        const dim3 grid((unsigned)cdiv(conv1_ring_count(kNet, kNet), kRingPx), (unsigned)n);
        LAUNCHED((conv1_ring_kernel<<<grid, 256, kRingSmem, st>>>(c0s.hi, c0s.lo, 160, 160, e->conv1f_w, e->conv1f_b, keep_conv1 ? conv1_out : nullptr,
                                                                 fuse_pred ? e->pred_g_w : nullptr, e->pred_g_b, bt->pred_gravity,
                                                                 fuse_pred ? e->pred_l_w : nullptr, e->pred_l_b, bt->pred_latitude), cudaGetLastError()));
      }
    } else {
      float* c0 = ar.f((long long)n * 160 * 160 * 128);
      {
        Epi o; o.C = c0; o.ldc = 128; o.c_gcoff = 64; o.act = 1;
        TRY(F.thalo(fused_s, 0, 256, &ll, 256, 0, n, 160, 160, 320, e->conv0, 64, 2, 64, o));
        TRY(F.tap("head.conv0", c0, (long long)n * 160 * 160 * 128));
      }
      SplitT c0u = F.salloc((long long)n * kNet * kNet, 128);
      if (!dry) LAUNCHED(launch_pdl(upsample2x_kernel, dim3(ew_grid(upsample2x_threads(n, 160, 160, 128))), dim3(256), 0, st, c0, 128, 0, nullptr, 128, 0, n, 160, 160, 128, c0u.hi, c0u.lo));
      Epi o; o.ldc = 64; o.c_gcoff = 32; o.act = 1;
      if (keep_conv1) o.C = conv1_out;
      TRY(F.thalo(c0u, 0, 64, nullptr, 0, 0, n, kNet, kNet, 64, e->conv1, 32, 2, 32, o, fuse_pred ? pt : nullptr));
    }
    if (keep_conv1) TRY(F.tap("head.conv1", conv1_out, (long long)n * kNet * kNet * 64));
    ar.release(m);
  }
  section("pf:tails_postprocess");
  TRY(fwd_tails_post(F, bt, conv1_out, d_post, fuse_pred));

  if (D.param_net != PF_PARAM_NONE) {
    section("pf:paramnet");
    if (D.gravity_classes != 2 || D.latitude_classes != 1) return fail(PF_ERR_ARG, "ParamNet needs regression heads");
    const int S = D.param_net == PF_PARAM_CENTERED ? kNet : D.param_input_size;
    float* pin = ar.f((long long)n * S * S * 4);
    if (!dry) LAUNCHED((pack_fields_kernel<<<(unsigned)cdivl((long long)n * S * S, 256), 256, 0, st>>>(bt->pred_gravity, bt->pred_latitude, pin, n, S), cudaGetLastError()));
    int r = S / 4;
    float* x = ar.f((long long)n * r * r * 96);
    if (!dry) LAUNCHED((stem_conv_launch<4, 4, 4, 0, 96>(pin, 4, n, S, S, e->pn_stem_w, e->pn_stem_b, x, 0, st)));
    TRY(F.ln(x, x, (long long)n * r * r, 96, e->pn_stem_ln, 1e-6f));
    for (int s = 0; s < 4; ++s) {
      const int C = kCnxDims[s];
      if (s > 0) {
        const int r2 = r / 2;
        SplitT y = F.salloc((long long)n * r2 * r2, 4 * kCnxDims[s - 1]);
        TRY(F.ln_split_patch(x, SplitT(), y, (long long)n * r * r, kCnxDims[s - 1], e->pn_ds_ln[s], 1e-6f, r, 2));
        float* xn = ar.f((long long)n * r2 * r2 * C);
        Epi o; o.C = xn; o.ldc = C;
        TRY(F.tgemm(y, (long long)n * r2 * r2, 4 * kCnxDims[s - 1], 0, e->pn_ds[s], C, o));
        x = xn; r = r2;
      }
      const long long rows = (long long)n * r * r;
      float* yf = ar.f(rows * C);
      SplitT y = F.salloc(rows, C);
      SplitT h = F.salloc(rows, 4 * C);
      for (int j = 0; j < kCnxDepths[s]; ++j) {
        const CnxBlockW& b = e->pn_blocks[s][j];
        if (e->use_dwln) {
          if (!dry) LAUNCHED(dwconv7x7_ln_launch(x, n, r, r, C, b.dw_w, b.dw_b, b.ln.w, b.ln.b, 1e-6f, y, st));
        } else {
          if (!dry) LAUNCHED(launch_pdl(dwconv7x7_kernel, dim3(ew_grid((long long)n * ((r + 1) / 2) * ((r + PF_DW7_PX - 1) / PF_DW7_PX) * (C / 4))), dim3(256), 0, st, x, yf, n, r, r, C, b.dw_w, b.dw_b));
          TRY(F.ln_split(yf, y, rows, C, b.ln, 1e-6f));
        }
        { Epi o; o.S = h; o.act = 2; TRY(F.tgemm(y, rows, C, 0, b.pw1, 4 * C, o)); }
        { Epi o; o.C = x; o.ldc = C; o.res = x; o.ldr = C; o.gamma = b.gamma; TRY(F.tgemm(h, rows, 4 * C, 0, b.pw2, C, o)); }
      }
      TRY(F.tapf(x, rows * C, "cnx.s%d", s));
    }
    if (!dry) {
      if (!bt->params) return fail(PF_ERR_ARG, "params output is NULL");
      LAUNCHED((param_tail_kernel<<<n, 256, 0, st>>>(x, r * r, e->pn_norm.w, e->pn_norm.b, e->pn_head_w, e->pn_head_b, bt->params, D.param_net), cudaGetLastError()));
    }
  }
  return PF_OK;
}

extern "C" {

int pf_abi_version(void) { return PF_ABI_VERSION; }
const char* pf_last_error(void) { return g_err.c_str(); }
int64_t pf_kernel_launch_count(void) { return g_launches.load(); }

static int configure_device(int device) {
  static std::mutex mu;
  static std::vector<char> done;
  std::lock_guard<std::mutex> lock(mu);
  if (device < (int)done.size() && done[device]) return PF_OK;
  CU(gemm_tma_configure_device());
  CU(attention_mma_configure_device());
  CU(cudaFuncSetAttribute(attention_kernel, cudaFuncAttributeMaxDynamicSharedMemorySize, kAttnSmem));
  CU(cudaFuncSetAttribute(conv1_ring_kernel, cudaFuncAttributeMaxDynamicSharedMemorySize, kRingSmem));
  CU(cudaFuncSetAttribute(preprocess_kernel, cudaFuncAttributeMaxDynamicSharedMemorySize, kPreMaxSmemRows * kNet * 3));
  if (device >= (int)done.size()) done.resize(device + 1, 0);
  done[device] = 1;
  return PF_OK;
}
static int configure_current_device() {
  int dev = 0;
  CU(cudaGetDevice(&dev));
  return configure_device(dev);
}

int pf_create(int device, const pf_model_desc* desc, pf_handle* out) {
  if (!desc || !out) return fail(PF_ERR_ARG, "pf_create: null argument");
  if (!((desc->gravity_classes == 2 || desc->gravity_classes == 73) && (desc->latitude_classes == 1 || desc->latitude_classes == 180)))
    return fail(PF_ERR_ARG, "pf_create: unsupported head widths %d/%d", desc->gravity_classes, desc->latitude_classes);
  if (desc->param_net < 0 || desc->param_net > 2) return fail(PF_ERR_ARG, "pf_create: bad param_net");
  if (desc->param_net == PF_PARAM_UNCENTERED && (desc->param_input_size < 32 || desc->param_input_size > kNet || desc->param_input_size % 32))
    return fail(PF_ERR_ARG, "pf_create: param_input_size must be a multiple of 32 in [32, 320]");
  int count = 0;
  CU(cudaGetDeviceCount(&count));
  if (device < 0 || device >= count) return fail(PF_ERR_CUDA, "pf_create: no CUDA device %d (found %d)", device, count);
  CU(cudaSetDevice(device));
  cudaDeviceProp prop;
  CU(cudaGetDeviceProperties(&prop, device));
  if (prop.major != 9 || prop.minor != 0) return fail(PF_ERR_CUDA, "pf_create: device %d is sm_%d%d; this library is built for sm_90a only", device, prop.major, prop.minor);
  TRY(configure_device(device));
  pf_engine* e = new pf_engine();
  e->device = device;
  e->sm_count = prop.multiProcessorCount;
  e->desc = *desc;
  if (cudaMalloc(&e->table_dev, kTableSlabBytes) != cudaSuccess || cudaMallocHost(&e->table_host, kTableSlabBytes) != cudaSuccess) {
    const int r = fail(PF_ERR_CUDA, "pf_create: resize-table slab: %s", cudaGetErrorString(cudaGetLastError()));
    cudaFree(e->table_dev);
    delete e;
    return r;
  }
  if (cudaStreamCreateWithFlags(&e->side, cudaStreamNonBlocking) != cudaSuccess || cudaEventCreateWithFlags(&e->ev_fork, cudaEventDisableTiming) != cudaSuccess ||
      cudaEventCreateWithFlags(&e->ev_join, cudaEventDisableTiming) != cudaSuccess) {
    const int r = fail(PF_ERR_CUDA, "pf_create: side stream / events: %s", cudaGetErrorString(cudaGetLastError()));
    pf_destroy(e);
    return r;
  }
  *out = e;
  return PF_OK;
}

int pf_destroy(pf_handle h) {
  if (!h) return PF_OK;
  cudaSetDevice(h->device);
  if (h->side) { cudaStreamSynchronize(h->side); cudaStreamDestroy(h->side); }
  if (h->ev_fork) cudaEventDestroy(h->ev_fork);
  if (h->ev_join) cudaEventDestroy(h->ev_join);
  cudaFree(h->table_dev);
  cudaFreeHost(h->table_host);
  for (auto& r : h->prof) { cudaEventDestroy(r.a); cudaEventDestroy(r.b); }
  for (auto ev : h->ev_pool) cudaEventDestroy(ev);
  for (auto ev : h->kp.pool) cudaEventDestroy(ev);
  delete h;
  return PF_OK;
}

int pf_set_weight(pf_handle h, const char* name, const void* dev_ptr, int64_t numel, int dtype) {
  if (!h || !name || !dev_ptr) return fail(PF_ERR_ARG, "pf_set_weight: null argument");
  if (((uintptr_t)dev_ptr & 15) != 0) return fail(PF_ERR_ARG, "pf_set_weight: '%s' is not 16-byte aligned", name);
  h->weights[name] = WeightRef{dev_ptr, numel, dtype};
  h->finalized = false;
  return PF_OK;
}

int pf_finalize(pf_handle h) {
  if (!h) return fail(PF_ERR_ARG, "pf_finalize: null handle");
  TRY(resolve_weights(h));
  h->finalized = true;
  return PF_OK;
}

int64_t pf_workspace_bytes(pf_handle h, int n, int max_h) {
  if (!h || n < 1) return fail(PF_ERR_ARG, "pf_workspace_bytes: bad argument");
  Fwd F{h, Arena{}, nullptr, true, n};
  F.ar.dry = true;
  F.ar.keep = h->debug;
  (void)max_h;
  int r = run_forward_tma(F, nullptr);
  if (r != PF_OK) return r;
  return F.ar.peak + 4096;
}

int pf_forward(pf_handle h, const pf_batch* bt, void* workspace, int64_t workspace_bytes, void* stream) {
  if (!h || !bt || !workspace) return fail(PF_ERR_ARG, "pf_forward: null argument");
  if (!h->finalized) return fail(PF_ERR_WEIGHT, "pf_forward: pf_finalize has not succeeded");
  if (bt->n < 1) return fail(PF_ERR_ARG, "pf_forward: empty batch");
  if ((bt->images_u8 != nullptr) == (bt->images_chw != nullptr)) return fail(PF_ERR_ARG, "pf_forward: exactly one of images_u8 / images_chw");
  if (bt->images_u8 && !bt->image_offset) return fail(PF_ERR_ARG, "pf_forward: image_offset is NULL");
  if (!bt->height || !bt->width || !bt->pred_gravity || !bt->pred_latitude || !bt->gravity_original || !bt->latitude_original ||
      !bt->gravity_original_offset || !bt->latitude_original_offset)
    return fail(PF_ERR_ARG, "pf_forward: null input/output pointer");
  CU(cudaSetDevice(h->device));
  Fwd F{h, Arena{}, (cudaStream_t)stream, false, bt->n};
  F.ar.base = (char*)workspace;
  F.ar.cap = workspace_bytes;
  F.ar.keep = h->debug;
  {
    Fwd T{h, Arena{}, nullptr, true, bt->n};
    T.ar.dry = true; T.ar.keep = h->debug;
    TRY(run_forward_tma(T, nullptr));
    if (T.ar.peak > workspace_bytes) return fail(PF_ERR_WORKSPACE, "pf_forward: workspace %lld B < required %lld B", (long long)workspace_bytes, T.ar.peak);
  }
  if (((uintptr_t)workspace & 255) != 0) return fail(PF_ERR_ARG, "pf_forward: workspace must be 256-byte aligned");
  h->taps.clear();
  h->kp.st = (cudaStream_t)stream;
  tl_kp = &h->kp;
  pdl_enabled() = h->use_pdl && !h->kp.on && !h->profile && !sync_debug();
  const int r = run_forward_tma(F, bt);
  pdl_enabled() = false;
  tl_kp = nullptr;
  return r;
}

int pf_profile_enable(pf_handle h, int on) {
  if (!h) return fail(PF_ERR_ARG, "null handle");
  h->profile = on != 0;
  while (on > 1 && (long long)h->ev_pool.size() < 2LL * on) {
    cudaEvent_t ev;
    CU(cudaEventCreate(&ev));
    h->ev_pool.push_back(ev);
  }
  return PF_OK;
}
int pf_profile_kernels_enable(pf_handle h, int max_launches) {
  if (!h) return fail(PF_ERR_ARG, "null handle");
  CU(cudaSetDevice(h->device));
  KernelProf& kp = h->kp;
  kp.on = max_launches > 0;
  kp.used = 0;
  kp.recs.clear();
  while ((long long)kp.pool.size() < 2LL * max_launches) {
    cudaEvent_t ev;
    CU(cudaEventCreate(&ev));
    kp.pool.push_back(ev);
  }
  return PF_OK;
}
int pf_profile_kernels_read(pf_handle h, char* buf, int cap) {
  if (!h || !buf || cap < 1) return fail(PF_ERR_ARG, "pf_profile_kernels_read: bad argument");
  std::map<std::string, std::pair<int, double>> agg;
  std::vector<std::string> order;
  for (const auto& r : h->kp.recs) {
    float ms = 0.f;
    CU(cudaEventElapsedTime(&ms, r.a, r.b));
    const char* c = r.expr;
    while (*c == '(' || *c == ' ') ++c;
    const char* e = c;
    while (*e && (isalnum((unsigned char)*e) || *e == '_')) ++e;
    std::string name(c, e);
    if (name == "launch_pdl" && *e == '(') {
      c = e + 1;
      e = c;
      while (*e && (isalnum((unsigned char)*e) || *e == '_')) ++e;
      name.assign(c, e);
    }
    if (*e == '<' && e[1] != '<') { const char* t = strchr(e, '>'); if (t) name.append(e, t + 1); }
    auto it = agg.find(name);
    if (it == agg.end()) { order.push_back(name); it = agg.emplace(name, std::make_pair(0, 0.0)).first; }
    it->second.first += 1;
    it->second.second += ms;
  }
  std::string out = "kernel,launches,ms\n";
  for (const auto& n : order) {
    char line[256];
    snprintf(line, sizeof line, "%s,%d,%.4f\n", n.c_str(), agg[n].first, agg[n].second);
    out += line;
  }
  if ((int)out.size() + 1 > cap) return fail(PF_ERR_ARG, "pf_profile_kernels_read: buffer too small (%d needed)", (int)out.size() + 1);
  memcpy(buf, out.c_str(), out.size() + 1);
  h->kp.used = 0;
  h->kp.recs.clear();
  return (int)out.size();
}
int pf_set_option(pf_handle h, const char* name, int value) {
  if (!h || !name) return fail(PF_ERR_ARG, "pf_set_option: null argument");
  if (!strcmp(name, "attn_mma")) { h->use_attn_mma = value != 0; return PF_OK; }
  if (!strcmp(name, "stem_tc")) { h->use_stem_tc = value != 0; return PF_OK; }
  if (!strcmp(name, "phase_conv1")) { h->use_phase = value != 0; return PF_OK; }
  if (!strcmp(name, "attn_split")) { h->use_attn_split = value != 0; return PF_OK; }
  if (!strcmp(name, "decode_only")) { h->decode_only = value != 0; return PF_OK; }
  if (!strcmp(name, "pdl")) { h->use_pdl = value != 0; return PF_OK; }
  if (!strcmp(name, "dw_ln")) { h->use_dwln = value != 0; return PF_OK; }
  if (!strcmp(name, "fork")) { h->use_fork = value != 0; return PF_OK; }
  return fail(PF_ERR_ARG, "pf_set_option: unknown option '%s'", name);
}
int pf_profile_read(pf_handle h, double* out9) {
  if (!h || !out9) return fail(PF_ERR_ARG, "pf_profile_read: null argument");
  for (int i = 0; i < 21; ++i) out9[i] = 0.0;
  FILE* csv = nullptr;
  if (const char* path = getenv("PF_PROFILE_CSV")) {
    csv = fopen(path, "w");
    if (csv) fprintf(csv, "engine_cfg,M,N,K,Cin,KH,stride,groups,ms,algorithmic_tflops\n");
  }
  for (auto& r : h->prof) {
    float ms = 0.f;
    CU(cudaEventSynchronize(r.b));
    CU(cudaEventElapsedTime(&ms, r.a, r.b));
    if (csv) fprintf(csv, "%d,%d,%d,%d,%d,%d,%d,%d,%.4f,%.1f\n", r.cfg, r.M, r.N, r.K, r.Cin, r.KH, r.stride, r.groups, ms, r.flops / (ms * 1e9));
    out9[r.cfg * 3 + 0] += ms;
    out9[r.cfg * 3 + 1] += r.flops;
    out9[r.cfg * 3 + 2] += 1.0;
    h->ev_pool.push_back(r.a);
    h->ev_pool.push_back(r.b);
  }
  if (csv) fclose(csv);
  h->prof.clear();
  return PF_OK;
}

int pf_debug_enable(pf_handle h, int on) {
  if (!h) return fail(PF_ERR_ARG, "null handle");
  h->debug = on != 0;
  h->taps.clear();
  return PF_OK;
}
int pf_debug_count(pf_handle h) { return h ? (int)h->taps.size() : 0; }
const char* pf_debug_name(pf_handle h, int i) { return (h && i >= 0 && i < (int)h->taps.size()) ? h->taps[i].first.c_str() : ""; }
int64_t pf_debug_numel(pf_handle h, const char* name) {
  if (!h || !name) return -1;
  for (auto& t : h->taps) if (t.first == name) return t.second.second;
  return -1;
}
int pf_debug_copy(pf_handle h, const char* name, float* dst, int64_t numel, void* stream) {
  if (!h || !name || !dst) return fail(PF_ERR_ARG, "pf_debug_copy: null argument");
  for (auto& t : h->taps)
    if (t.first == name) {
      if (numel != t.second.second) return fail(PF_ERR_ARG, "pf_debug_copy: '%s' has %lld elements", name, t.second.second);
      CU(cudaMemcpyAsync(dst, t.second.first, numel * 4, cudaMemcpyDeviceToDevice, (cudaStream_t)stream));
      return PF_OK;
    }
  return fail(PF_ERR_ARG, "pf_debug_copy: no tap '%s'", name);
}

#define NCCL_TRY(expr)                                                                                              \
  do {                                                                                                              \
    int r__ = (expr);                                                                                               \
    if (r__ != kNcclSuccess) return fail(PF_ERR_CUDA, "%s: %s", #expr, api.GetErrorString ? api.GetErrorString(r__) : "NCCL error"); \
  } while (0)
int pf_comm_unique_id(void* id128) {
  if (!id128) return fail(PF_ERR_ARG, "pf_comm_unique_id: null argument");
  const NcclApi& api = nccl_api();
  if (api.error) return fail(PF_ERR_CUDA, "%s", api.error);
  static_assert(sizeof(NcclUniqueId) == 128, "ncclUniqueId is 128 bytes");
  NCCL_TRY(api.GetUniqueId((NcclUniqueId*)id128));
  return PF_OK;
}
int pf_comm_create(int device, int rank, int nranks, const void* id128, pf_comm_handle* out) {
  if (!id128 || !out || nranks < 1 || rank < 0 || rank >= nranks) return fail(PF_ERR_ARG, "pf_comm_create: bad argument");
  const NcclApi& api = nccl_api();
  if (api.error) return fail(PF_ERR_CUDA, "%s", api.error);
  CU(cudaSetDevice(device));
  NcclUniqueId id;
  memcpy(&id, id128, sizeof id);
  pf_comm* c = new pf_comm();
  c->device = device; c->rank = rank; c->nranks = nranks;
  const int r = api.CommInitRank(&c->comm, nranks, id, rank);
  if (r != kNcclSuccess) { delete c; return fail(PF_ERR_CUDA, "ncclCommInitRank: %s", api.GetErrorString(r)); }
  *out = c;
  return PF_OK;
}
int pf_comm_destroy(pf_comm_handle c) {
  if (!c) return PF_OK;
  const NcclApi& api = nccl_api();
  cudaSetDevice(c->device);
  if (c->comm && api.CommDestroy) api.CommDestroy(c->comm);
  delete c;
  return PF_OK;
}
int pf_gather(pf_comm_handle c, int root, int count, void* const* dev_ptrs, const int64_t* bytes, const int32_t* peer, void* stream) {
  if (!c || count < 0 || root < 0 || root >= c->nranks || (count > 0 && (!dev_ptrs || !bytes))) return fail(PF_ERR_ARG, "pf_gather: bad argument");
  if (c->rank == root && count > 0 && !peer) return fail(PF_ERR_ARG, "pf_gather: the root needs the source rank of every segment");
  const NcclApi& api = nccl_api();
  CU(cudaSetDevice(c->device));
  if (count == 0) return PF_OK;
  NCCL_TRY(api.GroupStart());
  for (int i = 0; i < count; ++i) {
    int r;
    if (c->rank == root) {
      if (peer[i] < 0 || peer[i] >= c->nranks || peer[i] == root) { api.GroupEnd(); return fail(PF_ERR_ARG, "pf_gather: segment %d comes from rank %d", i, peer[i]); }
      r = api.Recv(dev_ptrs[i], (size_t)bytes[i], kNcclUint8, peer[i], c->comm, (cudaStream_t)stream);
    } else {
      r = api.Send(dev_ptrs[i], (size_t)bytes[i], kNcclUint8, root, c->comm, (cudaStream_t)stream);
    }
    if (r != kNcclSuccess) { api.GroupEnd(); return fail(PF_ERR_CUDA, "ncclSend/Recv: %s", api.GetErrorString(r)); }
  }
  NCCL_TRY(api.GroupEnd());
  return PF_OK;
}

int pf_jpeg_create(int device, int max_threads, pf_jpeg_handle* out) {
  if (!out) return fail(PF_ERR_ARG, "pf_jpeg_create: null argument");
  const NvjpegApi& api = nvjpeg_api();
  if (api.error) return fail(PF_ERR_CUDA, "%s", api.error);
  CU(cudaSetDevice(device));
  pf_jpeg* j = new pf_jpeg();
  j->device = device;
  if (api.CreateSimple(&j->handle) != NVJPEG_STATUS_SUCCESS) { delete j; return fail(PF_ERR_CUDA, "nvjpegCreateSimple failed"); }
  int nt = max_threads > 0 ? max_threads : (int)std::thread::hardware_concurrency() / 2;
  nt = nt < 1 ? 1 : (nt > 32 ? 32 : nt);
  j->workers.resize(nt);
  bool ok = cudaEventCreateWithFlags(&j->start, cudaEventDisableTiming) == cudaSuccess;
  for (auto& w : j->workers) {
    ok = ok && api.StateCreate(j->handle, &w.state) == NVJPEG_STATUS_SUCCESS;
    ok = ok && cudaStreamCreateWithFlags(&w.stream, cudaStreamNonBlocking) == cudaSuccess;
    ok = ok && cudaEventCreateWithFlags(&w.done, cudaEventDisableTiming) == cudaSuccess;
  }
  if (!ok) { pf_jpeg_destroy(j); return fail(PF_ERR_CUDA, "pf_jpeg_create: decoder state / stream creation failed"); }
  *out = j;
  return PF_OK;
}
int pf_jpeg_destroy(pf_jpeg_handle j) {
  if (!j) return PF_OK;
  const NvjpegApi& api = nvjpeg_api();
  cudaSetDevice(j->device);
  for (auto& w : j->workers) {
    if (w.stream) cudaStreamSynchronize(w.stream);
    if (w.state) api.StateDestroy(w.state);
    if (w.stream) cudaStreamDestroy(w.stream);
    if (w.done) cudaEventDestroy(w.done);
  }
  if (j->start) cudaEventDestroy(j->start);
  if (j->handle) api.Destroy(j->handle);
  delete j;
  return PF_OK;
}
int pf_jpeg_info(pf_jpeg_handle j, const uint8_t* data, int64_t length, int32_t* height, int32_t* width) {
  if (!j || !data || length < 4 || !height || !width) return fail(PF_ERR_ARG, "pf_jpeg_info: bad argument");
  const NvjpegApi& api = nvjpeg_api();
  int nc = 0, ws[NVJPEG_MAX_COMPONENT] = {0}, hs[NVJPEG_MAX_COMPONENT] = {0};
  nvjpegChromaSubsampling_t ss;
  if (api.GetImageInfo(j->handle, data, (size_t)length, &nc, &ss, ws, hs) != NVJPEG_STATUS_SUCCESS) return fail(PF_ERR_ARG, "pf_jpeg_info: not a decodable JPEG stream");
  *height = hs[0]; *width = ws[0];
  return PF_OK;
}
int pf_jpeg_decode_batch(pf_jpeg_handle j, int n, const uint8_t* const* data, const int64_t* length, const int32_t* height, const int32_t* width,
                         uint8_t* blob, const int64_t* offset, void* stream) {
  if (!j || n < 1 || !data || !length || !height || !width || !blob || !offset) return fail(PF_ERR_ARG, "pf_jpeg_decode_batch: bad argument");
  const NvjpegApi& api = nvjpeg_api();
  CU(cudaSetDevice(j->device));
  cudaStream_t st = (cudaStream_t)stream;
  CU(cudaEventRecord(j->start, st));
  const int nt = (int)j->workers.size() < n ? (int)j->workers.size() : n;
  std::atomic<int> next{0}, failed{-1};
  auto work = [&](int t) {
    cudaSetDevice(j->device);
    pf_jpeg::Worker& w = j->workers[t];
    cudaStreamWaitEvent(w.stream, j->start, 0);
    for (int i = next.fetch_add(1); i < n; i = next.fetch_add(1)) {
      nvjpegImage_t dst{};
      dst.channel[0] = blob + offset[i];
      dst.pitch[0] = (size_t)width[i] * 3;
      if (api.Decode(j->handle, w.state, data[i], (size_t)length[i], NVJPEG_OUTPUT_BGRI, &dst, w.stream) != NVJPEG_STATUS_SUCCESS) failed.store(i);
    }
    cudaEventRecord(w.done, w.stream);
  };
  std::vector<std::thread> threads;
  for (int t = 1; t < nt; ++t) threads.emplace_back(work, t);
  work(0);
  for (auto& th : threads) th.join();
  for (int t = 0; t < nt; ++t) CU(cudaStreamWaitEvent(st, j->workers[t].done, 0));
  if (failed.load() >= 0) return fail(PF_ERR_ARG, "pf_jpeg_decode_batch: image %d could not be decoded", failed.load());
  return PF_OK;
}

int pf_op_conv_gemm(const float* x, int B, int H, int W, int Cin, const void* whi, const void* wlo, const float* bias, int N, int KH, int KW,
                    int stride, int pad, int in_relu, int act, const float* res, int res_relu, float* y, void* stream) {
  if (!x || !whi || !wlo || !y) return fail(PF_ERR_ARG, "pf_op_conv_gemm: null argument");
  if (KH != KW) return fail(PF_ERR_ARG, "pf_op_conv_gemm: square filters only");
  TRY(configure_current_device());
  cudaStream_t st = (cudaStream_t)stream;
  int dev = 0;
  CU(cudaGetDevice(&dev));
  cudaDeviceProp prop;
  CU(cudaGetDeviceProperties(&prop, dev));
  pf_engine tmp;
  tmp.device = dev;
  tmp.sm_count = prop.multiProcessorCount;
  const int OH = (H + 2 * pad - KH) / stride + 1, OW = (W + 2 * pad - KW) / stride + 1;
  const long long nx = (long long)B * H * W * Cin;
  const long long colb = (long long)B * OH * OW * KH * KW * Cin * 4 + (1 << 20);
  char* scratch = nullptr;
  CU(cudaMalloc(&scratch, nx * 4 + colb + 4096));
  Fwd F{&tmp, Arena{}, st, false, B};
  F.ar.base = scratch; F.ar.cap = nx * 4 + colb + 4096;
  SplitT A = F.salloc((long long)B * H * W, Cin);
  int r = PF_OK;
  {
    cudaError_t le = (split_kernel<<<(unsigned)cdivl(nx, 256), 256, 0, st>>>(x, A.hi, A.lo, nx, in_relu), cudaGetLastError());
    g_launches.fetch_add(1, std::memory_order_relaxed);
    if (le != cudaSuccess) r = fail(PF_ERR_CUDA, "split_kernel: %s", cudaGetErrorString(le));
  }
  GemmW w{(const __nv_bfloat16*)whi, (const __nv_bfloat16*)wlo, bias};
  Fwd::Epi o;
  o.C = y; o.ldc = N; o.act = act; o.res = res; o.ldr = N; o.res_relu = res_relu;
  if (r == PF_OK) {
    if (KH == 3 && stride == 1 && pad == 1 && Cin % 64 == 0) r = F.thalo(A, 0, 0, nullptr, 0, 0, B, H, W, Cin, w, N, 1, 0, o);
    else if (KH == 1 && stride == 1 && pad == 0) r = F.tgemm(A, (long long)B * H * W, Cin, 0, w, N, o);
    else r = F.tconv_gather(A, B, H, W, Cin, KH, stride, pad, w, N, o);
  }
  cudaError_t se = cudaStreamSynchronize(st);
  cudaFree(scratch);
  if (r != PF_OK) return r;
  if (se != cudaSuccess) return fail(PF_ERR_CUDA, "pf_op_conv_gemm: %s", cudaGetErrorString(se));
  return PF_OK;
}
int pf_op_tma(pf_tma_op* op, void* stream) {
  if (!op || !op->a_hi || !op->a_lo || !op->w_hi || !op->w_lo) return fail(PF_ERR_ARG, "pf_op_tma: null argument");
  const pf_tma_op& q = *op;
  if (q.mode != MODE_GEMM && q.mode != MODE_HALO) return fail(PF_ERR_ARG, "pf_op_tma: mode %d", q.mode);
  if (!q.C && !q.s_hi) return fail(PF_ERR_ARG, "pf_op_tma: no output (C and S are both NULL)");
  if (!q.s_hi != !q.s_lo || !q.a2_hi != !q.a2_lo) return fail(PF_ERR_ARG, "pf_op_tma: a split pair needs both planes");
  if (q.bias_mode < 0 || q.bias_mode > 2 || q.act < 0 || q.act > 2) return fail(PF_ERR_ARG, "pf_op_tma: bias_mode %d / act %d", q.bias_mode, q.act);
  if (q.groups < 1 || q.groups > 2 || q.N < 1) return fail(PF_ERR_ARG, "pf_op_tma: groups %d, N %d", q.groups, q.N);
  if (q.npred != 0 && q.npred != q.groups) return fail(PF_ERR_ARG, "pf_op_tma: npred must be 0 or groups");
  if (q.mode == MODE_GEMM && (q.groups != 1 || q.a2_hi || q.phase4 || q.npred || q.M < 1 || q.M > INT32_MAX))
    return fail(PF_ERR_ARG, "pf_op_tma: GEMM mode runs one group of 1..2^31-1 rows without A2, phase4 or prediction tail");
  if (q.mode == MODE_HALO && (q.B < 1 || q.H < 1 || q.W < 1)) return fail(PF_ERR_ARG, "pf_op_tma: image size %dx%dx%d", q.B, q.H, q.W);
  TRY(configure_current_device());
  int dev = 0;
  CU(cudaGetDevice(&dev));
  cudaDeviceProp prop;
  CU(cudaGetDeviceProperties(&prop, dev));
  pf_engine tmp;
  tmp.device = dev;
  tmp.sm_count = prop.multiProcessorCount;
  Fwd F{&tmp, Arena{}, (cudaStream_t)stream, false, q.B};
  F.force_bn = q.force_bn; F.force_kb = q.force_kb;
  const SplitT A{(__nv_bfloat16*)q.a_hi, (__nv_bfloat16*)q.a_lo, q.lda};
  const SplitT A2{(__nv_bfloat16*)q.a2_hi, (__nv_bfloat16*)q.a2_lo, q.lda2};
  const GemmW w{(const __nv_bfloat16*)q.w_hi, (const __nv_bfloat16*)q.w_lo, q.bias};
  Fwd::Epi o;
  o.C = q.C; o.ldc = q.ldc; o.c_coff = q.c_coff; o.c_gcoff = q.c_gcoff;
  o.S = SplitT{(__nv_bfloat16*)q.s_hi, (__nv_bfloat16*)q.s_lo, q.lds}; o.s_coff = q.s_coff; o.s_gcoff = q.s_gcoff; o.split_relu = q.split_relu;
  o.act = q.act; o.gamma = q.gamma;
  o.res = q.res; o.ldr = q.ldr; o.r_coff = q.r_coff; o.r_gcoff = q.r_gcoff; o.res_relu = q.res_relu;
  o.res2 = q.res2; o.ldr2 = q.ldr2; o.r2_coff = q.r2_coff; o.r2_gcoff = q.r2_gcoff;
  o.bias_mode = q.bias_mode; o.phase4 = q.phase4;
  PredTail pt[2];
  for (int g = 0; g < q.npred; ++g) {
    const pf_tma_pred& s = q.pred[g];
    if (!s.w || !s.b || !s.out || !(s.mode == 1 ? s.nc == 2 : (s.mode == 2 && s.nc == 1))) return fail(PF_ERR_ARG, "pf_op_tma: prediction tail %d", g);
    pt[g] = PredTail{s.w, s.b, s.out, s.nc, s.mode};
  }
  op->picked_bn = op->picked_kb = 0;
  const int r = q.mode == MODE_GEMM ? F.tgemm(A, q.M, q.K, q.a_c0, w, q.N, o)
                                    : F.thalo(A, q.a_c0, q.a_gc, q.a2_hi ? &A2 : nullptr, q.c_split, q.a2_c0, q.B, q.H, q.W, q.Cin, w, q.N, q.groups,
                                              q.bias_gstride, o, q.npred ? pt : nullptr);
  if (r == PF_OK) { op->picked_bn = F.picked_bn; op->picked_kb = F.picked_kb; }
  return r;
}
int pf_op_conv1_ring(const void* c_hi, const void* c_lo, int B, int H, int W, const float* wf, const float* bias, float* out,
                     const float* pg_w, const float* pg_b, float* pg_out, const float* pl_w, const float* pl_b, float* pl_out, void* stream) {
  if (!c_hi || !c_lo || !wf || !bias) return fail(PF_ERR_ARG, "pf_op_conv1_ring: null argument");
  const bool tail = pg_w || pg_b || pg_out || pl_w || pl_b || pl_out;
  if (tail && !(pg_w && pg_b && pg_out && pl_w && pl_b && pl_out)) return fail(PF_ERR_ARG, "pf_op_conv1_ring: the prediction tail needs all six pointers");
  if (!out && !tail) return fail(PF_ERR_ARG, "pf_op_conv1_ring: no output");
  if (B < 1 || H < 2 || W < 2) return fail(PF_ERR_ARG, "pf_op_conv1_ring: needs B >= 1 and H, W >= 2 (got %dx%dx%d)", B, H, W);
  TRY(configure_current_device());
  const dim3 grid((unsigned)cdiv(conv1_ring_count(2 * H, 2 * W), kRingPx), (unsigned)B);
  LAUNCHED((conv1_ring_kernel<<<grid, 256, kRingSmem, (cudaStream_t)stream>>>((const __nv_bfloat16*)c_hi, (const __nv_bfloat16*)c_lo, H, W, wf, bias, out,
                                                                             pg_w, pg_b, pg_out, pl_w, pl_b, pl_out), cudaGetLastError()));
  return PF_OK;
}
int pf_tma_pick_tile(int mode, int64_t M, int N, int K, int sm_count, int* bn, int* kb) {
  if (!bn || !kb || (mode != MODE_GEMM && mode != MODE_HALO) || N < 1 || K < 1 || sm_count < 1) return fail(PF_ERR_ARG, "pf_tma_pick_tile: bad argument");
  tma_pick_tile(mode, M, N, K, sm_count, *bn, *kb);
  return PF_OK;
}
int pf_camera_fields(int device, const pf_camera* cams, int n, float* up, float* lat, void* stream) {
  if (!cams || n < 1 || (!up && !lat)) return fail(PF_ERR_ARG, "pf_camera_fields: bad argument");
  CU(cudaSetDevice(device));
  for (int i0 = 0; i0 < n; i0 += kCamChunk) {
    const int m = n - i0 < kCamChunk ? n - i0 : kCamChunk;
    CamBatch b{};
    long long max_q = 1;
    for (int i = 0; i < m; ++i) {
      const pf_camera& c = cams[i0 + i];
      if (c.height < 1 || c.width < 1 || !(c.focal_rel != 0.0)) return fail(PF_ERR_ARG, "pf_camera_fields: image %d: size %dx%d, focal %g", i0 + i, c.height, c.width, c.focal_rel);
      if ((c.up_offset & 1) != 0) return fail(PF_ERR_ARG, "pf_camera_fields: up_offset must be even (8-byte stores)");
      CamImage& o = b.im[i];
      o.H = c.height; o.W = c.width;
      o.f = c.focal_rel * c.height;
      o.cx = (c.cx_rel + 0.5) * c.width; o.cy = (c.cy_rel + 0.5) * c.height;
      o.sr = sin(c.roll); o.cr = cos(c.roll); o.se = sin(c.elevation); o.ce = cos(c.elevation);
      o.sgn = c.elevation > 0 ? 1.0 : (c.elevation < 0 ? -1.0 : 0.0);
      o.up_off = c.up_offset; o.lat_off = c.lat_offset;
      const long long qd = (long long)c.height * ((c.width + 3) / 4);
      if (qd > max_q) max_q = qd;
    }
    const dim3 grid((unsigned)cdivl(max_q, 256), (unsigned)m);
    LAUNCHED((camera_fields_kernel<<<grid, 256, 0, (cudaStream_t)stream>>>(b, up, lat), cudaGetLastError()));
  }
  return PF_OK;
}

static int upload_table(const ResampleTable& t, int** bounds, int** coeffs) {
  CU(cudaMalloc(bounds, t.bounds.size() * 4));
  CU(cudaMalloc(coeffs, t.coeffs.size() * 4));
  CU(cudaMemcpy(*bounds, t.bounds.data(), t.bounds.size() * 4, cudaMemcpyHostToDevice));
  CU(cudaMemcpy(*coeffs, t.coeffs.data(), t.coeffs.size() * 4, cudaMemcpyHostToDevice));
  return PF_OK;
}
int pf_op_resize_u8(const uint8_t* img, int H, int W, int new_h, int new_w, uint8_t* out, void* stream) {
  if (!img || !out || H < 1 || W < 1 || new_h < 1 || new_w < 1) return fail(PF_ERR_ARG, "pf_op_resize_u8: bad argument");
  cudaStream_t st = (cudaStream_t)stream;
  if (H == new_h && W == new_w) {
    CU(cudaMemcpyAsync(out, img, (size_t)H * W * 3, cudaMemcpyDeviceToDevice, st));
    return PF_OK;
  }
  ResampleTable tx = make_resample_table(W, new_w), ty = make_resample_table(H, new_h);
  int *bx = nullptr, *cx = nullptr, *by = nullptr, *cy = nullptr;
  unsigned char* tmp = nullptr;
  int r = upload_table(tx, &bx, &cx);
  if (r == PF_OK) r = upload_table(ty, &by, &cy);
  if (r == PF_OK && cudaMalloc(&tmp, (size_t)H * new_w * 3) != cudaSuccess) r = fail(PF_ERR_CUDA, "pf_op_resize_u8: cudaMalloc");
  if (r == PF_OK) {
    cudaError_t le = (resize_u8_h_kernel<<<(unsigned)cdivl((long long)H * new_w, 256), 256, 0, st>>>(img, H, W, new_w, bx, cx, tx.ksize, tmp), cudaGetLastError());
    if (le == cudaSuccess) le = (resize_u8_v_kernel<<<(unsigned)cdivl((long long)new_h * new_w, 256), 256, 0, st>>>(tmp, H, new_w, new_h, by, cy, ty.ksize, out), cudaGetLastError());
    g_launches.fetch_add(2, std::memory_order_relaxed);
    if (le == cudaSuccess) le = cudaStreamSynchronize(st);
    if (le != cudaSuccess) r = fail(PF_ERR_CUDA, "pf_op_resize_u8: %s", cudaGetErrorString(le));
  }
  cudaFree(bx); cudaFree(cx); cudaFree(by); cudaFree(cy); cudaFree(tmp);
  return r;
}
int pf_op_resize_f32(const float* img, int H, int W, int C, int new_h, int new_w, float* out, void* stream) {
  if (!img || !out || H < 1 || W < 1 || C < 1 || new_h < 1 || new_w < 1) return fail(PF_ERR_ARG, "pf_op_resize_f32: bad argument");
  LAUNCHED((resize_f32_kernel<<<(unsigned)cdivl((long long)new_h * new_w * C, 256), 256, 0, (cudaStream_t)stream>>>(img, H, W, C, new_h, new_w, out), cudaGetLastError()));
  return PF_OK;
}
int pf_op_argmax_decode(const float* logits, float* field, int B, int HW, int NC, int is_gravity, void* stream) {
  if (!logits || !field || B < 1 || HW < 1 || NC < 1) return fail(PF_ERR_ARG, "pf_op_argmax_decode: bad argument");
  LAUNCHED((argmax_decode_kernel<<<(unsigned)cdivl((long long)B * HW, 256), 256, 0, (cudaStream_t)stream>>>(logits, field, B, HW, NC, is_gravity), cudaGetLastError()));
  return PF_OK;
}
int pf_op_pred_argmax_decode(const float* feat, int ld, int coff, const float* w, const float* bias, float* field, int B, int HW, int NC, int is_gravity,
                             void* stream) {
  if (!feat || !w || !bias || !field || B < 1 || HW < 1 || NC < 1 || NC > 256 || (ld & 3) || (coff & 3)) return fail(PF_ERR_ARG, "pf_op_pred_argmax_decode: bad argument");
  LAUNCHED((pred_argmax_decode_kernel<<<ew_grid((long long)B * HW * 4), 256, NC * 37 * 4, (cudaStream_t)stream>>>(feat, ld, coff, w, bias, field, B, HW, NC, is_gravity),
            cudaGetLastError()));
  return PF_OK;
}
int pf_op_postprocess(const float* vec, const float* lat, int n, const int32_t* height, const int32_t* width, float* gravity_original,
                      const int64_t* gravity_original_offset, float* latitude_original, const int64_t* latitude_original_offset, int lat_is_sin,
                      void* stream) {
  if (!vec || !lat || n < 1 || !height || !width || !gravity_original || !gravity_original_offset || !latitude_original || !latitude_original_offset)
    return fail(PF_ERR_ARG, "pf_op_postprocess: bad argument");
  PostImage* d_post = nullptr;
  CU(cudaMalloc(&d_post, n * sizeof(PostImage)));
  int r = launch_postprocess(vec, lat, n, height, width, gravity_original_offset, latitude_original_offset, gravity_original, latitude_original,
                             lat_is_sin, d_post, (cudaStream_t)stream);
  cudaError_t se = cudaStreamSynchronize((cudaStream_t)stream);
  cudaFree(d_post);
  if (r == PF_OK && se != cudaSuccess) r = fail(PF_ERR_CUDA, "pf_op_postprocess: %s", cudaGetErrorString(se));
  return r;
}

int pf_op_fill_stream(float* dst, int64_t numel, float value, void* stream) {
  if (!dst || numel < 4 || (numel & 3) || ((uintptr_t)dst & 15)) return fail(PF_ERR_ARG, "pf_op_fill_stream: bad argument");
  LAUNCHED((fill_stream_kernel<<<132 * 16, 256, 0, (cudaStream_t)stream>>>(reinterpret_cast<float4*>(dst), numel / 4, value), cudaGetLastError()));
  return PF_OK;
}
int pf_op_layernorm(const float* x, float* y, int64_t rows, int C, const float* w, const float* b, float eps, void* stream) {
  LAUNCHED(layernorm_launch(x, y, rows, C, w, b, eps, (cudaStream_t)stream));
  return PF_OK;
}
int pf_op_attention(const float* q, const float* kv, float* out, int B, int N, int C, int heads, void* stream) {
  TRY(configure_current_device());
  if (C != heads * kAttnD) return fail(PF_ERR_ARG, "pf_op_attention: head_dim must be 64");
  LAUNCHED(attention_launch(q, kv, out, B, N, C, heads, (cudaStream_t)stream));
  return PF_OK;
}
int pf_op_attention_mma(const float* q, const float* kv, float* out, int B, int N, int C, int heads, void* stream) {
  TRY(configure_current_device());
  if (C != heads * kAmD) return fail(PF_ERR_ARG, "pf_op_attention_mma: head_dim must be 64");
  LAUNCHED(attention_mma_launch(q, kv, out, B, N, C, heads, (cudaStream_t)stream));
  return PF_OK;
}
int pf_op_attention_tc(const float* q, const float* kv, float* out, int B, int N, int C, int heads, void* stream) {
  if (!q || !kv || !out || C != heads * kAmD) return fail(PF_ERR_ARG, "pf_op_attention_tc: head_dim must be 64");
  TRY(configure_current_device());
  cudaStream_t st = (cudaStream_t)stream;
  int dev = 0;
  CU(cudaGetDevice(&dev));
  cudaDeviceProp prop;
  CU(cudaGetDeviceProperties(&prop, dev));
  pf_engine tmp;
  tmp.device = dev;
  tmp.sm_count = prop.multiProcessorCount;
  const long long nq = (long long)B * N * C, nkv = (long long)B * kAmKeys * 2 * C;
  char* scratch = nullptr;
  CU(cudaMalloc(&scratch, (2 * nq + nkv) * 4 + 8192));
  Fwd F{&tmp, Arena{}, st, false, B};
  F.ar.base = scratch; F.ar.cap = (2 * nq + nkv) * 4 + 8192;
  SplitT qs = F.salloc((long long)B * N, C), kvs = F.salloc((long long)B * kAmKeys, 2 * C), as = F.salloc((long long)B * N, C);
  int r = PF_OK;
  cudaError_t le = (split_kernel<<<(unsigned)cdivl(nq, 256), 256, 0, st>>>(q, qs.hi, qs.lo, nq, 0), cudaGetLastError());
  if (le == cudaSuccess) le = (split_kernel<<<(unsigned)cdivl(nkv, 256), 256, 0, st>>>(kv, kvs.hi, kvs.lo, nkv, 0), cudaGetLastError());
  if (le != cudaSuccess) r = fail(PF_ERR_CUDA, "split_kernel: %s", cudaGetErrorString(le));
  if (r == PF_OK) {
    le = attention_mma_launch(nullptr, nullptr, nullptr, B, N, C, heads, st, as, qs, kvs);
    if (le != cudaSuccess) r = fail(PF_ERR_CUDA, "attention_mma_launch: %s", cudaGetErrorString(le));
  }
  if (r == PF_OK) {
    le = (merge_split_kernel<<<(unsigned)cdivl(nq, 256), 256, 0, st>>>(as.hi, as.lo, out, nq), cudaGetLastError());
    if (le != cudaSuccess) r = fail(PF_ERR_CUDA, "merge_split_kernel: %s", cudaGetErrorString(le));
  }
  cudaError_t se = cudaStreamSynchronize(st);
  cudaFree(scratch);
  if (r == PF_OK && se != cudaSuccess) r = fail(PF_ERR_CUDA, "pf_op_attention_tc: %s", cudaGetErrorString(se));
  return r;
}
int pf_op_dwconv3x3_gelu(const float* x, float* y, int B, int H, int W, int C, const float* w, const float* bias, void* stream) {
  if (C % 4) return fail(PF_ERR_ARG, "C %% 4");
  LAUNCHED(launch_pdl(dwconv3x3_gelu_kernel, dim3(ew_grid((long long)B * ((H + 1) / 2) * ((W + PF_DW3_PX - 1) / PF_DW3_PX) * (C / 4))), dim3(256), 0, (cudaStream_t)stream, x, y, B, H, W, C, w, bias, nullptr, nullptr));
  return PF_OK;
}
int pf_op_dwconv7x7(const float* x, float* y, int B, int H, int W, int C, const float* w, const float* bias, void* stream) {
  if (C % 4) return fail(PF_ERR_ARG, "C %% 4");
  LAUNCHED(launch_pdl(dwconv7x7_kernel, dim3(ew_grid((long long)B * ((H + 1) / 2) * ((W + PF_DW7_PX - 1) / PF_DW7_PX) * (C / 4))), dim3(256), 0, (cudaStream_t)stream, x, y, B, H, W, C, w, bias));
  return PF_OK;
}
int pf_op_upsample2x(const float* x, float* y, int B, int H, int W, int C, void* stream) {
  if (C % 4) return fail(PF_ERR_ARG, "C %% 4");
  LAUNCHED(launch_pdl(upsample2x_kernel, dim3(ew_grid(upsample2x_threads(B, H, W, C))), dim3(256), 0, (cudaStream_t)stream, x, C, 0, y, C, 0, B, H, W, C, nullptr, nullptr));
  return PF_OK;
}
int pf_op_preprocess(const uint8_t* img, int H, int W, const float* mean3, const float* std3, float* y, void* stream) {
  TRY(configure_current_device());
  ResampleTable tx = make_resample_table(W, kNet), ty = make_resample_table(H, kNet);
  if (ty.ksize + 1 > kPreMaxSmemRows) return fail(PF_ERR_ARG, "image too tall");
  int *bx, *cx, *by, *cy;
  PreImage* d;
  CU(cudaMalloc(&bx, tx.bounds.size() * 4)); CU(cudaMalloc(&cx, tx.coeffs.size() * 4));
  CU(cudaMalloc(&by, ty.bounds.size() * 4)); CU(cudaMalloc(&cy, ty.coeffs.size() * 4));
  CU(cudaMalloc(&d, sizeof(PreImage)));
  CU(cudaMemcpy(bx, tx.bounds.data(), tx.bounds.size() * 4, cudaMemcpyHostToDevice));
  CU(cudaMemcpy(cx, tx.coeffs.data(), tx.coeffs.size() * 4, cudaMemcpyHostToDevice));
  CU(cudaMemcpy(by, ty.bounds.data(), ty.bounds.size() * 4, cudaMemcpyHostToDevice));
  CU(cudaMemcpy(cy, ty.coeffs.data(), ty.coeffs.size() * 4, cudaMemcpyHostToDevice));
  PreImage pi{0, H, W, tx.ksize, ty.ksize, bx, cx, by, cy};
  CU(cudaMemcpy(d, &pi, sizeof pi, cudaMemcpyHostToDevice));
  int rows = pre_rows_needed(H);
  if (rows > kPreMaxSmemRows) rows = kPreMaxSmemRows;
  const int smem = rows * kNet * 3;
  LAUNCHED((preprocess_kernel<<<dim3(kNet / kPreRows, 1), kNet, smem, (cudaStream_t)stream>>>(img, d, y, mean3[0], mean3[1], mean3[2], std3[0], std3[1], std3[2], rows),
            cudaGetLastError()));
  CU(cudaStreamSynchronize((cudaStream_t)stream));
  cudaFree(bx); cudaFree(cx); cudaFree(by); cudaFree(cy); cudaFree(d);
  return PF_OK;
}

}
```

### perspectivefields_b200/csrc/tc_ptx.cuh

```cuda
#pragma once
#include "common.cuh"

namespace pf {

constexpr int kHtTileH = 16, kHtTileW = 8;
constexpr int kHtHaloW = kHtTileW + 2, kHtHaloH = kHtTileH + 2;
constexpr int kHtHaloPix = kHtHaloW * kHtHaloH;
constexpr int kHtPlaneBytes = 23 * 1024;

__device__ __forceinline__ void mbar_init(uint32_t bar, uint32_t count) {
  asm volatile("mbarrier.init.shared::cta.b64 [%0], %1;\n" ::"r"(bar), "r"(count) : "memory");
}
__device__ __forceinline__ void mbar_arrive(uint32_t bar) {
  asm volatile("mbarrier.arrive.shared::cta.b64 _, [%0];\n" ::"r"(bar) : "memory");
}
__device__ __forceinline__ uint32_t mbar_try_wait(uint32_t bar, uint32_t parity) {
  uint32_t ok;
  asm volatile("{\n\t.reg .pred p;\n\tmbarrier.try_wait.parity.shared::cta.b64 p, [%1], %2;\n\tselp.u32 %0, 1, 0, p;\n\t}\n"
               : "=r"(ok) : "r"(bar), "r"(parity) : "memory");
  return ok;
}
__device__ __forceinline__ void mbar_wait(uint32_t bar, uint32_t parity) {
  if (mbar_try_wait(bar, parity)) return;
  const long long t0 = clock64();
  while (!mbar_try_wait(bar, parity)) {
    if (clock64() - t0 > 4000000000LL) __trap();
  }
}
__device__ __forceinline__ void fence_mbar_init() { asm volatile("fence.mbarrier_init.release.cluster;\n" ::: "memory"); }
__device__ __forceinline__ void named_bar_sync(int id, int count) { asm volatile("bar.sync %0, %1;\n" ::"r"(id), "r"(count) : "memory"); }

__device__ __forceinline__ void wgmma_fence() { asm volatile("wgmma.fence.sync.aligned;\n" ::: "memory"); }
__device__ __forceinline__ void wgmma_commit() { asm volatile("wgmma.commit_group.sync.aligned;\n" ::: "memory"); }
template <int N>
__device__ __forceinline__ void wgmma_wait() { asm volatile("wgmma.wait_group.sync.aligned %0;\n" ::"n"(N) : "memory"); }
template <int R>
__device__ __forceinline__ void fence_regs(float (&d)[R]) {
#pragma unroll
  for (int i = 0; i < R; ++i) asm volatile("" : "+f"(d[i])::"memory");
}

#define PF_R8(i) "+f"(d[i]), "+f"(d[i + 1]), "+f"(d[i + 2]), "+f"(d[i + 3]), "+f"(d[i + 4]), "+f"(d[i + 5]), "+f"(d[i + 6]), "+f"(d[i + 7])
__device__ __forceinline__ void wgmma_n64(float* d, uint64_t adesc, uint64_t bdesc, uint32_t scale_d) {
  asm volatile(
      "{\n\t.reg .pred p;\n\tsetp.ne.b32 p, %34, 0;\n\t"
      "wgmma.mma_async.sync.aligned.m64n64k16.f32.bf16.bf16 "
      "{%0,%1,%2,%3,%4,%5,%6,%7,%8,%9,%10,%11,%12,%13,%14,%15,%16,%17,%18,%19,%20,%21,%22,%23,%24,%25,%26,%27,%28,%29,%30,%31}, "
      "%32, %33, p, 1, 1, 0, 0;\n\t}\n"
      : PF_R8(0), PF_R8(8), PF_R8(16), PF_R8(24)
      : "l"(adesc), "l"(bdesc), "r"(scale_d));
}
__device__ __forceinline__ void wgmma_n32(float* d, uint64_t adesc, uint64_t bdesc, uint32_t scale_d) {
  asm volatile(
      "{\n\t.reg .pred p;\n\tsetp.ne.b32 p, %18, 0;\n\t"
      "wgmma.mma_async.sync.aligned.m64n32k16.f32.bf16.bf16 "
      "{%0,%1,%2,%3,%4,%5,%6,%7,%8,%9,%10,%11,%12,%13,%14,%15}, %16, %17, p, 1, 1, 0, 0;\n\t}\n"
      : PF_R8(0), PF_R8(8)
      : "l"(adesc), "l"(bdesc), "r"(scale_d));
}
#undef PF_R8

template <int KB>
__device__ __forceinline__ uint64_t wgmma_tile_desc(uint32_t smem_addr) {
  constexpr uint64_t sbo = KB == 32 ? 512 : 1024, layout = KB == 32 ? 2 : 1;
  return (uint64_t)((smem_addr >> 4) & 0x3FFFu) | ((uint64_t)1 << 16) | ((sbo >> 4) << 32) | (layout << 62);
}
__device__ __forceinline__ uint64_t ht_a_desc(uint32_t smem_addr) {
  return (uint64_t)((smem_addr >> 4) & 0x3FFFu) | ((uint64_t)1 << 16) | ((uint64_t)((kHtHaloW * 128) >> 4) << 32) |
         ((uint64_t)1 << 62);
}

}
```

### perspectivefields_b200/csrc/tma_host.cuh

```cuda
#pragma once
#include <cuda.h>
#include <cuda_runtime.h>

#include <cstdlib>
#include <string>

#include "gemm_tma.cuh"

namespace pf {

typedef CUresult (*PFN_tensorMapEncodeTiled)(CUtensorMap*, CUtensorMapDataType, cuuint32_t, void*, const cuuint64_t*, const cuuint64_t*,
                                             const cuuint32_t*, const cuuint32_t*, CUtensorMapInterleave, CUtensorMapSwizzle,
                                             CUtensorMapL2promotion, CUtensorMapFloatOOBfill);

inline PFN_tensorMapEncodeTiled tma_encoder() {
  static PFN_tensorMapEncodeTiled fn = nullptr;
  if (!fn) {
    void* p = nullptr;
    cudaDriverEntryPointQueryResult q;
    if (cudaGetDriverEntryPoint("cuTensorMapEncodeTiled", &p, cudaEnableDefault, &q) == cudaSuccess && q == cudaDriverEntryPointSuccess)
      fn = (PFN_tensorMapEncodeTiled)p;
  }
  return fn;
}

inline const char* tma_map_2d(CUtensorMap* m, const void* base, long long cols, long long rows, long long ld, int box_rows, int kb) {
  PFN_tensorMapEncodeTiled enc = tma_encoder();
  if (!enc) return "cuTensorMapEncodeTiled entry point not available";
  cuuint64_t dims[2] = {(cuuint64_t)cols, (cuuint64_t)rows};
  cuuint64_t strides[1] = {(cuuint64_t)ld * 2};
  cuuint32_t box[2] = {(cuuint32_t)kb, (cuuint32_t)box_rows};
  cuuint32_t es[2] = {1, 1};
  if (((uintptr_t)base & 15) || (strides[0] & 15) || box_rows < 1 || box_rows > 256) return "tma_map_2d: alignment / box";
  CUresult r = enc(m, CU_TENSOR_MAP_DATA_TYPE_BFLOAT16, 2, const_cast<void*>(base), dims, strides, box, es, CU_TENSOR_MAP_INTERLEAVE_NONE,
                   kb == 32 ? CU_TENSOR_MAP_SWIZZLE_64B : CU_TENSOR_MAP_SWIZZLE_128B, CU_TENSOR_MAP_L2_PROMOTION_L2_128B,
                   CU_TENSOR_MAP_FLOAT_OOB_FILL_NONE);
  return r == CUDA_SUCCESS ? nullptr : "cuTensorMapEncodeTiled (2d) failed";
}

inline const char* tma_map_halo(CUtensorMap* m, const void* base, int B, int H, int W, int ld) {
  PFN_tensorMapEncodeTiled enc = tma_encoder();
  if (!enc) return "cuTensorMapEncodeTiled entry point not available";
  cuuint64_t dims[4] = {(cuuint64_t)ld, (cuuint64_t)W, (cuuint64_t)H, (cuuint64_t)B};
  cuuint64_t strides[3] = {(cuuint64_t)ld * 2, (cuuint64_t)W * ld * 2, (cuuint64_t)H * W * ld * 2};
  cuuint32_t box[4] = {64, (cuuint32_t)kHtHaloW, (cuuint32_t)kHtHaloH, 1};
  cuuint32_t es[4] = {1, 1, 1, 1};
  if (((uintptr_t)base & 15) || (strides[0] & 15)) return "tma_map_halo: alignment";
  CUresult r = enc(m, CU_TENSOR_MAP_DATA_TYPE_BFLOAT16, 4, const_cast<void*>(base), dims, strides, box, es, CU_TENSOR_MAP_INTERLEAVE_NONE,
                   CU_TENSOR_MAP_SWIZZLE_128B, CU_TENSOR_MAP_L2_PROMOTION_L2_128B, CU_TENSOR_MAP_FLOAT_OOB_FILL_NONE);
  return r == CUDA_SUCCESS ? nullptr : "cuTensorMapEncodeTiled (halo) failed";
}

inline int tma_pick_bn(int N, int mode) {
  const int tiles = cdiv(N, 256);
  int bn = cdiv(cdiv(N, tiles), 32) * 32;
  if (mode == MODE_HALO) bn = bn <= 32 ? 32 : (bn <= 64 ? 64 : (bn <= 128 ? 128 : 256));
  return bn;
}

inline int tma_pick_bn_gemm(long long M, int N, int K, int sm_count) {
  const int base = tma_pick_bn(N, MODE_GEMM);
  const long long mt = cdivl(M, 128);
  if (mt * cdiv(N, base) * 4 > 3LL * sm_count) return base;
  int best = base;
  double best_cost = 1e30;
  for (int bn = base; bn >= 32; bn -= 32) {
    const long long tiles = mt * cdiv(N, bn);
    const double waves = (double)cdivl(tiles, sm_count);
    const double mma = 3.0 * bn, load = 1.6 * (128 + bn);
    const double cost = waves * ((K / 16) * (mma > load ? mma : load) + 3000.0);
    if (cost < best_cost - 1e-9) { best_cost = cost; best = bn; }
  }
  return best;
}

inline int tma_pick_kb(int bn, int K, int mode) {
  const int lim = mode == MODE_HALO ? 128 : 64;
  return (bn <= lim && K % 64 == 0) ? 64 : 32;
}

inline void tma_pick_tile(int mode, long long M, int N, int K, int sm_count, int& bn, int& kb) {
  bn = mode == MODE_GEMM ? tma_pick_bn_gemm(M, N, K, sm_count) : tma_pick_bn(N, mode);
  kb = tma_pick_kb(bn, K, mode);
}

struct PredTail { const float* w; const float* b; float* out; int nc, mode; };

template <int BN, int MODE, int KB>
inline cudaError_t gemm_tma_launch_bn(const TmaMaps& maps, const TmaGemmParams& p, int sm_count, cudaStream_t st, const PredTail* pred) {
  using Cfg = TmaCfg<BN, MODE, KB>;
  const int tiles_x = MODE == MODE_HALO ? cdiv(p.W, kHtTileW) : 0, tiles_y = MODE == MODE_HALO ? cdiv(p.H, kHtTileH) : 0;
  const long long m_tiles = MODE == MODE_GEMM ? cdiv(p.M, 128) : (long long)p.B * tiles_x * tiles_y;
  const long long total = m_tiles * cdiv(p.N, BN) * p.groups;
  const unsigned grid = (unsigned)(total < sm_count ? total : sm_count);
  if (MODE == MODE_HALO && ((p.Cin == 64 && 9 * (64 / KB) <= Cfg::kStages && (p.groups > 1 || cdiv(p.N, BN) > 1)) || pred)) {
    cudaError_t last = cudaSuccess;
    for (int g = 0; g < p.groups; ++g)
      for (int nt = 0; nt < cdiv(p.N, BN); ++nt) {
        TmaGemmParams q = p;
        q.groups = 1;
        q.a_c0 = p.a_c0 + g * p.a_gc;
        q.bias = p.bias ? p.bias + (long long)g * p.bias_gstride : nullptr;
        q.c_coff = p.c_coff + g * p.c_gcoff; q.s_coff = p.s_coff + g * p.s_gcoff;
        q.r_coff = p.r_coff + g * p.r_gcoff; q.r2_coff = p.r2_coff + g * p.r2_gcoff;
        q.b_row0 = g * p.N;
        if (pred) { q.pred_w = pred[g].w; q.pred_b = pred[g].b; q.pred_out = pred[g].out; q.pred_nc = pred[g].nc; q.pred_mode = pred[g].mode; }
        if (cdiv(p.N, BN) > 1) return cudaErrorInvalidValue;
        const unsigned gr = (unsigned)(m_tiles < sm_count ? m_tiles : sm_count);
        last = launch_pdl(gemm_tma_kernel<BN, MODE, KB>, dim3(gr), dim3(kTmaThreads), Cfg::kSmemBytes, st, maps, q, tiles_x, tiles_y);
        if (last != cudaSuccess) return last;
      }
    return last;
  }
  return launch_pdl(gemm_tma_kernel<BN, MODE, KB>, dim3(grid), dim3(kTmaThreads), Cfg::kSmemBytes, st, maps, p, tiles_x, tiles_y);
}

#define PF_TMA_VARIANTS(X)                                                                                                  \
  X(256, MODE_GEMM, 32) X(224, MODE_GEMM, 32) X(192, MODE_GEMM, 32) X(160, MODE_GEMM, 32) X(128, MODE_GEMM, 32) X(96, MODE_GEMM, 32) \
  X(64, MODE_GEMM, 32) X(32, MODE_GEMM, 32) X(64, MODE_GEMM, 64) X(32, MODE_GEMM, 64)                                        \
  X(256, MODE_HALO, 32) X(128, MODE_HALO, 64) X(64, MODE_HALO, 64) X(32, MODE_HALO, 64)

inline cudaError_t gemm_tma_configure_device() {
  cudaError_t e = cudaSuccess;
#define PF_TMA_CFG(BN_, MODE_, KB_)                                                                                          \
  if (e == cudaSuccess) e = cudaFuncSetAttribute(gemm_tma_kernel<BN_, MODE_, KB_>, cudaFuncAttributeMaxDynamicSharedMemorySize, TmaCfg<BN_, MODE_, KB_>::kSmemBytes);
  PF_TMA_VARIANTS(PF_TMA_CFG)
#undef PF_TMA_CFG
  return e;
}

inline int tma_stages(int mode, int bn, int kb) {
#define PF_TMA_NS(BN_, MODE_, KB_) if (mode == MODE_ && bn == BN_ && kb == KB_) return TmaCfg<BN_, MODE_, KB_>::kStages;
  PF_TMA_VARIANTS(PF_TMA_NS)
#undef PF_TMA_NS
  return 0;
}

inline const char* gemm_tma_check(int mode, const TmaGemmParams& p, int bn, int kb, bool pred) {
  const int ns = tma_stages(mode, bn, kb);
  if (!ns) return "no engine instantiation for this (mode, bn, kb)";
  if (mode == MODE_GEMM) return p.K % kb ? "GEMM mode: K must be a multiple of the K step" : nullptr;
  if (p.phase4 && (p.N != 128 || bn != 128)) return "phase4 needs N = 128 in one 128-wide tile";
  if (pred && bn != (p.phase4 ? 128 : 32)) return "the fused prediction tail needs N = 32 (phase4: 128) in one tile";
  const bool resident = p.Cin == 64 && 9 * (64 / kb) <= ns;
  if ((resident || pred) && cdiv(p.N, bn) > 1) return "resident weights (Cin = 64) and the prediction tail need one N tile per launch";
  return nullptr;
}

inline cudaError_t gemm_tma_launch(int mode,const TmaMaps& maps, const TmaGemmParams& p, int bn, int kb, int sm_count, cudaStream_t st,
                                   const PredTail* pred = nullptr) {
#define PF_TMA_CASE(BN_, MODE_, KB_) if (mode == MODE_ && bn == BN_ && kb == KB_) return gemm_tma_launch_bn<BN_, MODE_, KB_>(maps, p, sm_count, st, pred);
  PF_TMA_VARIANTS(PF_TMA_CASE)
#undef PF_TMA_CASE
  return cudaErrorInvalidValue;
}

}
```

Before: 677.9.

## Add ping-pong warpgroup schedule for TMA GEMM with 64-row tiles

```diff
diff --git a/include/pf_b200.h b/include/pf_b200.h
--- a/include/pf_b200.h
+++ b/include/pf_b200.h
@@ -116,6 +116,7 @@
   int npred; pf_tma_pred pred[2];
   int force_bn, force_kb;
   int picked_bn, picked_kb;
+  int force_sched, picked_sched;
 } pf_tma_op;
 int pf_op_tma(pf_tma_op* op, void* stream);
 int pf_op_conv1_ring(const void* c_hi, const void* c_lo, int B, int H, int W, const float* wf, const float* bias, float* out,
diff --git a/perspectivefields_b200/_native.py b/perspectivefields_b200/_native.py
--- a/perspectivefields_b200/_native.py
+++ b/perspectivefields_b200/_native.py
@@ -55,7 +55,7 @@
                        "int lda2, c_split, a2_c0; ptr w_hi, w_lo, bias; int bias_mode, bias_gstride, act; ptr gamma, res;"
                        "int ldr, r_coff, r_gcoff, res_relu; ptr res2; int ldr2, r2_coff, r2_gcoff; ptr C; int ldc, c_coff, c_gcoff;"
                        "ptr s_hi, s_lo; int lds, s_coff, s_gcoff, split_relu, phase4, npred") + \
-        [("pred", pf_tma_pred * 2)] + _fields("int force_bn, force_kb, picked_bn, picked_kb")
+        [("pred", pf_tma_pred * 2)] + _fields("int force_bn, force_kb, picked_bn, picked_kb, force_sched, picked_sched")
 
 
 def _sources():
diff --git a/perspectivefields_b200/csrc/gemm_tma.cuh b/perspectivefields_b200/csrc/gemm_tma.cuh
--- a/perspectivefields_b200/csrc/gemm_tma.cuh
+++ b/perspectivefields_b200/csrc/gemm_tma.cuh
@@ -28,11 +28,13 @@
   int phase4;
 };
 
-template <int BN, int MODE, int KB> struct TmaCfg {
+template <int BN, int MODE, int KB, bool PP = false> struct TmaCfg {
   static_assert(KB == 32 || KB == 64, "KB");
   static_assert(BN % 32 == 0 && BN <= 256, "BN");
+  static_assert(!PP || MODE == MODE_GEMM, "the ping-pong schedule is a GEMM-mode schedule");
+  static constexpr int kTileM = PP ? 64 : 128;
   static constexpr int kBPlane = BN * KB * 2;
-  static constexpr int kAPlane = 128 * KB * 2;
+  static constexpr int kAPlane = kTileM * KB * 2;
   static constexpr int kStage = (MODE == MODE_GEMM ? 2 * kAPlane : 0) + 2 * kBPlane;
   static constexpr int kABuf = 2 * kHtPlaneBytes;
   static constexpr int kAccPitch = 68;
@@ -64,12 +66,12 @@
   CUtensorMap a_hi, a_lo, a2_hi, a2_lo, b_hi, b_lo;
 };
 
-template <int BN, int MODE, int KB>
+template <int BN, int MODE, int KB, bool PP = false>
 __global__ void __launch_bounds__(kTmaThreads, 1) gemm_tma_kernel(const __grid_constant__ TmaMaps maps, const TmaGemmParams p, int tiles_x, int tiles_y) {
-  using Cfg = TmaCfg<BN, MODE, KB>;
+  using Cfg = TmaCfg<BN, MODE, KB, PP>;
   constexpr int NS = Cfg::kStages;
   constexpr int SPC = 9 * (64 / KB);
-  constexpr int kConsumerWarps = 8;
+  constexpr int kConsumerWarps = PP ? 4 : 8;
   extern __shared__ unsigned char smem_dyn[];
   const uint32_t raw = smem_u32(smem_dyn);
   const uint32_t sbase = (raw + 1023u) & ~1023u;
@@ -82,10 +84,11 @@
   auto empty_b = [&](int s) { return bars + 8u * (NS + s); };
   auto full_a = [&](int i) { return bars + 8u * (2 * NS + i); };
   auto empty_a = [&](int i) { return bars + 8u * (2 * NS + 2 + i); };
+  auto order_b = [&](int w) { return bars + 8u * (2 * NS + 4 + w); };
 
   const int tid = threadIdx.x, lane = tid & 31, warp = tid >> 5;
   const int n_tiles = cdiv(p.N, BN);
-  const int m_tiles = MODE == MODE_GEMM ? cdiv(p.M, 128) : p.B * tiles_x * tiles_y;
+  const int m_tiles = MODE == MODE_GEMM ? cdiv(p.M, Cfg::kTileM) : p.B * tiles_x * tiles_y;
   const int total_tiles = m_tiles * n_tiles * p.groups;
   const int nchunks = MODE == MODE_HALO ? p.Cin / 64 : 0;
   const int nk = MODE == MODE_GEMM ? p.K / KB : nchunks * SPC;
@@ -94,7 +97,7 @@
   if (tid == 0) {
     tma_prefetch_desc(&maps.a_hi); tma_prefetch_desc(&maps.a_lo); tma_prefetch_desc(&maps.b_hi); tma_prefetch_desc(&maps.b_lo);
     for (int s = 0; s < NS; ++s) { mbar_init(full_b(s), 1); mbar_init(empty_b(s), kConsumerWarps); }
-    for (int i = 0; i < 2; ++i) { mbar_init(full_a(i), 1); mbar_init(empty_a(i), kConsumerWarps); }
+    for (int i = 0; i < 2; ++i) { mbar_init(full_a(i), 1); mbar_init(empty_a(i), kConsumerWarps); mbar_init(order_b(i), 4); }
     fence_mbar_init();
   }
   __syncthreads();
@@ -125,8 +128,8 @@
           int kcol;
           if (MODE == MODE_GEMM) {
             kcol = kc * KB;
-            tma_load_2d(st, &maps.a_hi, full_b(s), p.a_c0 + g * p.a_gc + kcol, mt * 128);
-            tma_load_2d(st + Cfg::kAPlane, &maps.a_lo, full_b(s), p.a_c0 + g * p.a_gc + kcol, mt * 128);
+            tma_load_2d(st, &maps.a_hi, full_b(s), p.a_c0 + g * p.a_gc + kcol, mt * Cfg::kTileM);
+            tma_load_2d(st + Cfg::kAPlane, &maps.a_lo, full_b(s), p.a_c0 + g * p.a_gc + kcol, mt * Cfg::kTileM);
           } else {
             const int c = kc / SPC, u = kc - c * SPC;
             kcol = KB == 32 ? (u >> 1) * p.Cin + c * 64 + (u & 1) * 32 : u * p.Cin + c * 64;
@@ -166,12 +169,17 @@
   const int wt = tid & 127;
   float* stage = reinterpret_cast<float*>(sm + (acc_base - sbase)) + wg * 64 * Cfg::kAccPitch;
   const int erow = wt & 63, eh = wt >> 6;
-  const int r = wg * 64 + erow;
+  const int r = PP ? erow : wg * 64 + erow;
+  constexpr int kTileStep = PP ? 2 : 1;
   float acc[BN / 2];
   int it = 0, ita = 0;
-  for (int tile = blockIdx.x, tl = 0; tile < total_tiles; tile += gridDim.x, ++tl) {
+  for (int tl = PP ? wg : 0, tile = blockIdx.x + tl * gridDim.x; tile < total_tiles; tile += kTileStep * gridDim.x, tl += kTileStep) {
     int mt, g, n0;
     decode(tile, mt, g, n0);
+    if (PP) {
+      it = tl * nk;
+      if (tl > 0) mbar_wait(order_b(wg ^ 1), ((tl - 1) >> 1) & 1);
+    }
     int prev_s = -1, prev_buf = -1;
     fence_regs(acc);
     for (int kc = 0; kc < nk; ++kc, ++it) {
@@ -188,7 +196,7 @@
         a_lo = a_hi + kHtPlaneBytes;
         chunk_end = u == SPC - 1;
       } else {
-        a_hi = ring + s * Cfg::kStage + wg * 64 * KB * 2;
+        a_hi = ring + s * Cfg::kStage + (PP ? 0 : wg * 64 * KB * 2);
         a_lo = a_hi + Cfg::kAPlane;
       }
       const int sb = b_resident ? kc : s;
@@ -198,23 +206,13 @@
       const uint64_t dal = MODE == MODE_HALO ? ht_a_desc(a_lo) : wgmma_tile_desc<KB>(a_lo);
       const uint64_t dbh = wgmma_tile_desc<KB>(b_hi);
       const uint64_t dbl = wgmma_tile_desc<KB>(b_hi + Cfg::kBPlane);
-      constexpr uint64_t kChunk = (uint64_t)(64 * KB * 2) >> 4;
       wgmma_fence();
 #pragma unroll
       for (int kk = 0; kk < KB / 16; ++kk) {
         const uint32_t first = (kc | kk) ? 1u : 0u;
-#pragma unroll
-        for (int j = 0; j < BN / 64; ++j) {
-          wgmma_n64(acc + 32 * j, dal + 2 * kk, dbh + 2 * kk + j * kChunk, first);
-          wgmma_n64(acc + 32 * j, dah + 2 * kk, dbl + 2 * kk + j * kChunk, 1u);
-          wgmma_n64(acc + 32 * j, dah + 2 * kk, dbh + 2 * kk + j * kChunk, 1u);
-        }
-        if constexpr (BN % 64 != 0) {
-          constexpr int j = BN / 64;
-          wgmma_n32(acc + 32 * j, dal + 2 * kk, dbh + 2 * kk + j * kChunk, first);
-          wgmma_n32(acc + 32 * j, dah + 2 * kk, dbl + 2 * kk + j * kChunk, 1u);
-          wgmma_n32(acc + 32 * j, dah + 2 * kk, dbh + 2 * kk + j * kChunk, 1u);
-        }
+        wgmma_bf16<BN>(acc, dal + 2 * kk, dbh + 2 * kk, first);
+        wgmma_bf16<BN>(acc, dah + 2 * kk, dbl + 2 * kk, 1u);
+        wgmma_bf16<BN>(acc, dah + 2 * kk, dbh + 2 * kk, 1u);
       }
       wgmma_commit();
       wgmma_wait<1>();
@@ -226,6 +224,7 @@
       prev_buf = chunk_end ? buf : -1;
       if (MODE == MODE_HALO && chunk_end) ++ita;
     }
+    if (PP && lane == 0) mbar_arrive(order_b(wg));
     wgmma_wait<0>();
     fence_regs(acc);
     if (lane == 0 && prev_s >= 0) {
@@ -238,7 +237,7 @@
     int cls_off = 0;
     int bimg = 0, oy = 0, ox = 0;
     if (MODE == MODE_GEMM) {
-      m = (long long)mt * 128 + r;
+      m = (long long)mt * Cfg::kTileM + r;
       valid = m < p.M;
     } else {
       const int tx = mt % tiles_x, ty = (mt / tiles_x) % tiles_y;
@@ -268,127 +267,168 @@
       }
       named_bar_sync(1 + wg, 128);
       const int ch = 2 * rd + eh;
-      if (ch >= BN / 32) continue;
-      const int nb = n0 + ch * 32;
       const bool ph4 = MODE == MODE_HALO && BN == 128 && p.phase4;
-      const long long mo = ph4 ? ((long long)bimg * 2 * p.H + 2 * oy + (ch >> 1)) * (2 * p.W) + 2 * ox + (ch & 1) : m;
-      const int nbo = ph4 ? 0 : nb;
-      const bool chunk_ok = nb < p.N;
+      const bool staged_split = p.Shi && !ph4;
       float o[32];
-      const float* srow = stage + erow * Cfg::kAccPitch + eh * 32;
-#pragma unroll
-      for (int j = 0; j < 32; j += 4) {
-        const float4 t = *reinterpret_cast<const float4*>(srow + j);
-        o[j] = t.x; o[j + 1] = t.y; o[j + 2] = t.z; o[j + 3] = t.w;
-      }
-      if (valid && chunk_ok) {
-        if (p.bias_mode) {
-#pragma unroll
-          for (int j = 0; j < 32; j += 4) {
-            const float4 bv = __ldg(reinterpret_cast<const float4*>(bias + cls_off + nb + j));
-            o[j] += bv.x; o[j + 1] += bv.y; o[j + 2] += bv.z; o[j + 3] += bv.w;
-          }
-        }
-        if (p.act == 1) {
-#pragma unroll
-          for (int j = 0; j < 32; ++j) o[j] = fmaxf(o[j], 0.f);
-        } else if (p.act == 2) {
-#pragma unroll
-          for (int j = 0; j < 32; ++j) o[j] = gelu_erf(o[j]);
-        }
-        if (p.gamma) {
-#pragma unroll
-          for (int j = 0; j < 32; j += 4) {
-            const float4 gv = __ldg(reinterpret_cast<const float4*>(p.gamma + nb + j));
-            o[j] *= gv.x; o[j + 1] *= gv.y; o[j + 2] *= gv.z; o[j + 3] *= gv.w;
-          }
-        }
-        if (p.res) {
-          const float* rp = p.res + m * p.ldr + p.r_coff + g * p.r_gcoff + nb;
-#pragma unroll
-          for (int j = 0; j < 32; j += 4) {
-            float4 rv = *reinterpret_cast<const float4*>(rp + j);
-            if (p.res_relu) { rv.x = fmaxf(rv.x, 0.f); rv.y = fmaxf(rv.y, 0.f); rv.z = fmaxf(rv.z, 0.f); rv.w = fmaxf(rv.w, 0.f); }
-            o[j] += rv.x; o[j + 1] += rv.y; o[j + 2] += rv.z; o[j + 3] += rv.w;
-          }
-        }
-        if (p.res2) {
-          const float* rp = p.res2 + m * p.ldr2 + p.r2_coff + g * p.r2_gcoff + nb;
-#pragma unroll
-          for (int j = 0; j < 32; j += 4) {
-            const float4 rv = *reinterpret_cast<const float4*>(rp + j);
-            o[j] += rv.x; o[j + 1] += rv.y; o[j + 2] += rv.z; o[j + 3] += rv.w;
-          }
-        }
-        if (MODE == MODE_HALO && (BN == 32 || BN == 128) && p.pred_w) {
-          float v0 = __ldg(p.pred_b), v1 = p.pred_nc > 1 ? __ldg(p.pred_b + 1) : 0.f;
-#pragma unroll
-          for (int j = 0; j < 32; j += 4) {
-            const float4 w0 = __ldg(reinterpret_cast<const float4*>(p.pred_w + j));
-            v0 = fmaf(o[j], w0.x, v0); v0 = fmaf(o[j + 1], w0.y, v0); v0 = fmaf(o[j + 2], w0.z, v0); v0 = fmaf(o[j + 3], w0.w, v0);
-            if (p.pred_nc > 1) {
-              const float4 w1 = __ldg(reinterpret_cast<const float4*>(p.pred_w + 32 + j));
-              v1 = fmaf(o[j], w1.x, v1); v1 = fmaf(o[j + 1], w1.y, v1); v1 = fmaf(o[j + 2], w1.z, v1); v1 = fmaf(o[j + 3], w1.w, v1);
-            }
-          }
-          const long long HWl = (long long)p.H * p.W * (ph4 ? 4 : 1);
-          const long long bi = mo / HWl, pix = mo - bi * HWl;
-          float* po = p.pred_out + bi * p.pred_nc * HWl + pix;
-          if (p.pred_mode == 1) {
-            const float nrm = fmaxf(sqrtf(v0 * v0 + v1 * v1), 1e-12f);
-            po[0] = v0 / nrm; po[HWl] = v1 / nrm;
+      if (ch < BN / 32) {
+        const int nb = n0 + ch * 32;
+        const long long mo = ph4 ? ((long long)bimg * 2 * p.H + 2 * oy + (ch >> 1)) * (2 * p.W) + 2 * ox + (ch & 1) : m;
+        const int nbo = ph4 ? 0 : nb;
+        const bool chunk_ok = nb < p.N;
+        const float* srow = stage + erow * Cfg::kAccPitch + eh * 32;
+#pragma unroll
+        for (int j = 0; j < 32; j += 4) {
+          const float4 t = *reinterpret_cast<const float4*>(srow + j);
+          o[j] = t.x; o[j + 1] = t.y; o[j + 2] = t.z; o[j + 3] = t.w;
+        }
+        if (valid && chunk_ok) {
+          if (p.bias_mode) {
+#pragma unroll
+            for (int j = 0; j < 32; j += 4) {
+              const float4 bv = __ldg(reinterpret_cast<const float4*>(bias + cls_off + nb + j));
+              o[j] += bv.x; o[j + 1] += bv.y; o[j + 2] += bv.z; o[j + 3] += bv.w;
+            }
+          }
+          if (p.act == 1) {
+#pragma unroll
+            for (int j = 0; j < 32; ++j) o[j] = fmaxf(o[j], 0.f);
+          } else if (p.act == 2) {
+#pragma unroll
+            for (int j = 0; j < 32; ++j) o[j] = gelu_erf(o[j]);
+          }
+          if (p.gamma) {
+#pragma unroll
+            for (int j = 0; j < 32; j += 4) {
+              const float4 gv = __ldg(reinterpret_cast<const float4*>(p.gamma + nb + j));
+              o[j] *= gv.x; o[j + 1] *= gv.y; o[j + 2] *= gv.z; o[j + 3] *= gv.w;
+            }
+          }
+          if (p.res) {
+            const float* rp = p.res + m * p.ldr + p.r_coff + g * p.r_gcoff + nb;
+#pragma unroll
+            for (int j = 0; j < 32; j += 4) {
+              float4 rv = *reinterpret_cast<const float4*>(rp + j);
+              if (p.res_relu) { rv.x = fmaxf(rv.x, 0.f); rv.y = fmaxf(rv.y, 0.f); rv.z = fmaxf(rv.z, 0.f); rv.w = fmaxf(rv.w, 0.f); }
+              o[j] += rv.x; o[j + 1] += rv.y; o[j + 2] += rv.z; o[j + 3] += rv.w;
+            }
+          }
+          if (p.res2) {
+            const float* rp = p.res2 + m * p.ldr2 + p.r2_coff + g * p.r2_gcoff + nb;
+#pragma unroll
+            for (int j = 0; j < 32; j += 4) {
+              const float4 rv = *reinterpret_cast<const float4*>(rp + j);
+              o[j] += rv.x; o[j + 1] += rv.y; o[j + 2] += rv.z; o[j + 3] += rv.w;
+            }
+          }
+          if (MODE == MODE_HALO && (BN == 32 || BN == 128) && p.pred_w) {
+            float v0 = __ldg(p.pred_b), v1 = p.pred_nc > 1 ? __ldg(p.pred_b + 1) : 0.f;
+#pragma unroll
+            for (int j = 0; j < 32; j += 4) {
+              const float4 w0 = __ldg(reinterpret_cast<const float4*>(p.pred_w + j));
+              v0 = fmaf(o[j], w0.x, v0); v0 = fmaf(o[j + 1], w0.y, v0); v0 = fmaf(o[j + 2], w0.z, v0); v0 = fmaf(o[j + 3], w0.w, v0);
+              if (p.pred_nc > 1) {
+                const float4 w1 = __ldg(reinterpret_cast<const float4*>(p.pred_w + 32 + j));
+                v1 = fmaf(o[j], w1.x, v1); v1 = fmaf(o[j + 1], w1.y, v1); v1 = fmaf(o[j + 2], w1.z, v1); v1 = fmaf(o[j + 3], w1.w, v1);
+              }
+            }
+            const long long HWl = (long long)p.H * p.W * (ph4 ? 4 : 1);
+            const long long bi = mo / HWl, pix = mo - bi * HWl;
+            float* po = p.pred_out + bi * p.pred_nc * HWl + pix;
+            if (p.pred_mode == 1) {
+              const float nrm = fmaxf(sqrtf(v0 * v0 + v1 * v1), 1e-12f);
+              po[0] = v0 / nrm; po[HWl] = v1 / nrm;
+            } else {
+              po[0] = fminf(fmaxf(v0, -1.f), 1.f);
+            }
+          }
+        }
+        if (chunk_ok && (p.C || (p.Shi && !staged_split))) {
+          const bool odd = lane & 1;
+          const bool valid_p = __shfl_xor_sync(0xffffffffu, (int)valid, 1) != 0;
+          const long long mo_p = mo + (odd ? -1 : 1) * (ph4 ? 2 : 1);
+          const long long moA = odd ? mo_p : mo, moB = odd ? mo : mo_p;
+          const bool vA = odd ? valid_p : valid, vB = odd ? valid : valid_p;
+          if (p.C) {
+            float* cA = p.C + moA * p.ldc + p.c_coff + g * p.c_gcoff + nbo + (odd ? 4 : 0);
+            float* cB = p.C + moB * p.ldc + p.c_coff + g * p.c_gcoff + nbo + (odd ? 4 : 0);
+#pragma unroll
+            for (int t = 0; t < 4; ++t) {
+              float k[4], rr[4];
+#pragma unroll
+              for (int e = 0; e < 4; ++e) {
+                k[e] = odd ? o[8 * t + 4 + e] : o[8 * t + e];
+                rr[e] = __shfl_xor_sync(0xffffffffu, odd ? o[8 * t + e] : o[8 * t + 4 + e], 1);
+              }
+              if (vA) *reinterpret_cast<float4*>(cA + 8 * t) = odd ? make_float4(rr[0], rr[1], rr[2], rr[3]) : make_float4(k[0], k[1], k[2], k[3]);
+              if (vB) *reinterpret_cast<float4*>(cB + 8 * t) = odd ? make_float4(k[0], k[1], k[2], k[3]) : make_float4(rr[0], rr[1], rr[2], rr[3]);
+            }
+          }
+          if (p.Shi && !staged_split) {
+            const long long sA = moA * p.lds + p.s_coff + g * p.s_gcoff + nbo + (odd ? 8 : 0);
+            const long long sB = moB * p.lds + p.s_coff + g * p.s_gcoff + nbo + (odd ? 8 : 0);
+#pragma unroll
+            for (int t = 0; t < 2; ++t) {
+              float k[8], rr[8];
+#pragma unroll
+              for (int e = 0; e < 8; ++e) {
+                const float mine = odd ? o[16 * t + 8 + e] : o[16 * t + e], give = odd ? o[16 * t + e] : o[16 * t + 8 + e];
+                k[e] = p.split_relu ? fmaxf(mine, 0.f) : mine;
+                rr[e] = __shfl_xor_sync(0xffffffffu, p.split_relu ? fmaxf(give, 0.f) : give, 1);
+              }
+              uint4 kh, kl, rh, rl;
+              split_bf16x2(k[0], k[1], kh.x, kl.x); split_bf16x2(k[2], k[3], kh.y, kl.y);
+              split_bf16x2(k[4], k[5], kh.z, kl.z); split_bf16x2(k[6], k[7], kh.w, kl.w);
+              split_bf16x2(rr[0], rr[1], rh.x, rl.x); split_bf16x2(rr[2], rr[3], rh.y, rl.y);
+              split_bf16x2(rr[4], rr[5], rh.z, rl.z); split_bf16x2(rr[6], rr[7], rh.w, rl.w);
+              if (vA) {
+                *reinterpret_cast<uint4*>(p.Shi + sA + 16 * t) = odd ? rh : kh;
+                *reinterpret_cast<uint4*>(p.Slo + sA + 16 * t) = odd ? rl : kl;
+              }
+              if (vB) {
+                *reinterpret_cast<uint4*>(p.Shi + sB + 16 * t) = odd ? kh : rh;
+                *reinterpret_cast<uint4*>(p.Slo + sB + 16 * t) = odd ? kl : rl;
+              }
+            }
+          }
+        }
+      }
+      if (staged_split) {
+        named_bar_sync(1 + wg, 128);
+        unsigned char* sS = reinterpret_cast<unsigned char*>(stage);
+        if (ch < BN / 32) {
+#pragma unroll
+          for (int t = 0; t < 4; ++t) {
+            uint4 h, l;
+            float k[8];
+#pragma unroll
+            for (int e = 0; e < 8; ++e) k[e] = p.split_relu ? fmaxf(o[8 * t + e], 0.f) : o[8 * t + e];
+            split_bf16x2(k[0], k[1], h.x, l.x); split_bf16x2(k[2], k[3], h.y, l.y);
+            split_bf16x2(k[4], k[5], h.z, l.z); split_bf16x2(k[6], k[7], h.w, l.w);
+            const int off = erow * 128 + (((eh * 4 + t) ^ (erow & 7)) << 4);
+            *reinterpret_cast<uint4*>(sS + off) = h;
+            *reinterpret_cast<uint4*>(sS + 64 * 128 + off) = l;
+          }
+        }
+        named_bar_sync(1 + wg, 128);
+#pragma unroll
+        for (int i = wt; i < 2 * 64 * 8; i += 128) {
+          const int lo_plane = i >> 9, rr = (i >> 3) & 63, pc = i & 7;
+          const int col = rd * 64 + pc * 8;
+          if (col >= BN || n0 + col >= p.N) continue;
+          long long mr;
+          bool vr;
+          if (MODE == MODE_GEMM) {
+            mr = (long long)mt * Cfg::kTileM + (PP ? 0 : wg * 64) + rr;
+            vr = mr < p.M;
           } else {
-            po[0] = fminf(fmaxf(v0, -1.f), 1.f);
-          }
-        }
-      }
-      if (chunk_ok && (p.C || p.Shi)) {
-        const bool odd = lane & 1;
-        const bool valid_p = __shfl_xor_sync(0xffffffffu, (int)valid, 1) != 0;
-        const long long mo_p = mo + (odd ? -1 : 1) * (ph4 ? 2 : 1);
-        const long long moA = odd ? mo_p : mo, moB = odd ? mo : mo_p;
-        const bool vA = odd ? valid_p : valid, vB = odd ? valid : valid_p;
-        if (p.C) {
-          float* cA = p.C + moA * p.ldc + p.c_coff + g * p.c_gcoff + nbo + (odd ? 4 : 0);
-          float* cB = p.C + moB * p.ldc + p.c_coff + g * p.c_gcoff + nbo + (odd ? 4 : 0);
-#pragma unroll
-          for (int t = 0; t < 4; ++t) {
-            float k[4], rr[4];
-#pragma unroll
-            for (int e = 0; e < 4; ++e) {
-              k[e] = odd ? o[8 * t + 4 + e] : o[8 * t + e];
-              rr[e] = __shfl_xor_sync(0xffffffffu, odd ? o[8 * t + e] : o[8 * t + 4 + e], 1);
-            }
-            if (vA) *reinterpret_cast<float4*>(cA + 8 * t) = odd ? make_float4(rr[0], rr[1], rr[2], rr[3]) : make_float4(k[0], k[1], k[2], k[3]);
-            if (vB) *reinterpret_cast<float4*>(cB + 8 * t) = odd ? make_float4(k[0], k[1], k[2], k[3]) : make_float4(rr[0], rr[1], rr[2], rr[3]);
-          }
-        }
-        if (p.Shi) {
-          const long long sA = moA * p.lds + p.s_coff + g * p.s_gcoff + nbo + (odd ? 8 : 0);
-          const long long sB = moB * p.lds + p.s_coff + g * p.s_gcoff + nbo + (odd ? 8 : 0);
-#pragma unroll
-          for (int t = 0; t < 2; ++t) {
-            float k[8], rr[8];
-#pragma unroll
-            for (int e = 0; e < 8; ++e) {
-              const float mine = odd ? o[16 * t + 8 + e] : o[16 * t + e], give = odd ? o[16 * t + e] : o[16 * t + 8 + e];
-              k[e] = p.split_relu ? fmaxf(mine, 0.f) : mine;
-              rr[e] = __shfl_xor_sync(0xffffffffu, p.split_relu ? fmaxf(give, 0.f) : give, 1);
-            }
-            uint4 kh, kl, rh, rl;
-            split_bf16x2(k[0], k[1], kh.x, kl.x); split_bf16x2(k[2], k[3], kh.y, kl.y);
-            split_bf16x2(k[4], k[5], kh.z, kl.z); split_bf16x2(k[6], k[7], kh.w, kl.w);
-            split_bf16x2(rr[0], rr[1], rh.x, rl.x); split_bf16x2(rr[2], rr[3], rh.y, rl.y);
-            split_bf16x2(rr[4], rr[5], rh.z, rl.z); split_bf16x2(rr[6], rr[7], rh.w, rl.w);
-            if (vA) {
-              *reinterpret_cast<uint4*>(p.Shi + sA + 16 * t) = odd ? rh : kh;
-              *reinterpret_cast<uint4*>(p.Slo + sA + 16 * t) = odd ? rl : kl;
-            }
-            if (vB) {
-              *reinterpret_cast<uint4*>(p.Shi + sB + 16 * t) = odd ? kh : rh;
-              *reinterpret_cast<uint4*>(p.Slo + sB + 16 * t) = odd ? kl : rl;
-            }
-          }
+            const int rt = wg * 64 + rr, tx = mt % tiles_x, ty = (mt / tiles_x) % tiles_y;
+            const int py = ty * kHtTileH + (rt >> 3), px = tx * kHtTileW + (rt & 7);
+            vr = py < p.H && px < p.W;
+            mr = ((long long)bimg * p.H + py) * p.W + px;
+          }
+          if (!vr) continue;
+          const uint4 v = *reinterpret_cast<const uint4*>(sS + lo_plane * 64 * 128 + rr * 128 + ((pc ^ (rr & 7)) << 4));
+          *reinterpret_cast<uint4*>((lo_plane ? p.Slo : p.Shi) + mr * p.lds + p.s_coff + g * p.s_gcoff + n0 + col) = v;
         }
       }
     }
diff --git a/perspectivefields_b200/csrc/pf_b200.cu b/perspectivefields_b200/csrc/pf_b200.cu
--- a/perspectivefields_b200/csrc/pf_b200.cu
+++ b/perspectivefields_b200/csrc/pf_b200.cu
@@ -331,23 +331,25 @@
     e->taps.push_back({name, {cp, numel}});
     return PF_OK;
   }
-  static cudaError_t gemm_tma_gemm_mode(const TmaMaps& maps, const TmaGemmParams& p, int bn, int kb, int sms, cudaStream_t st, const PredTail* pred) {
-    return gemm_tma_launch(MODE_GEMM, maps, p, bn, kb, sms, st, pred);
-  }
-  static cudaError_t gemm_tma_halo_mode(const TmaMaps& maps, const TmaGemmParams& p, int bn, int kb, int sms, cudaStream_t st, const PredTail* pred) {
-    return gemm_tma_launch(MODE_HALO, maps, p, bn, kb, sms, st, pred);
+  static cudaError_t gemm_tma_gemm_mode(const TmaMaps& maps, const TmaGemmParams& p, int bn, int kb, bool pp, int sms, cudaStream_t st, const PredTail* pred) {
+    return gemm_tma_launch(MODE_GEMM, maps, p, bn, kb, pp, sms, st, pred);
+  }
+  static cudaError_t gemm_tma_halo_mode(const TmaMaps& maps, const TmaGemmParams& p, int bn, int kb, bool pp, int sms, cudaStream_t st, const PredTail* pred) {
+    return gemm_tma_launch(MODE_HALO, maps, p, bn, kb, pp, sms, st, pred);
   }
   int force_bn = 0, force_kb = 0;
-  int picked_bn = 0, picked_kb = 0;
-  int pick_tile(int mode, const TmaGemmParams& p, const PredTail* pred, int& bn, int& kb) {
+  int force_sched = 0;
+  int picked_bn = 0, picked_kb = 0, picked_sched = 0;
+  int pick_tile(int mode, const TmaGemmParams& p, const PredTail* pred, int& bn, int& kb, bool& pp) {
     tma_pick_tile(mode, p.M, p.N, p.K, e->sm_count, bn, kb);
     if (force_bn) { bn = force_bn; kb = tma_pick_kb(bn, p.K, mode); }
     if (force_kb) kb = force_kb;
-    if (const char* msg = gemm_tma_check(mode, p, bn, kb, pred != nullptr)) return fail(PF_ERR_ARG, "TMA engine, %s (bn %d, kb %d): %s", mode == MODE_GEMM ? "GEMM mode" : "halo mode", bn, kb, msg);
-    picked_bn = bn; picked_kb = kb;
+    pp = mode == MODE_GEMM && (force_sched ? force_sched == 2 : tma_pick_pingpong(p.M, p.N, p.K, bn, e->sm_count));
+    if (const char* msg = gemm_tma_check(mode, p, bn, kb, pred != nullptr, pp)) return fail(PF_ERR_ARG, "TMA engine, %s (bn %d, kb %d): %s", mode == MODE_GEMM ? "GEMM mode" : "halo mode", bn, kb, msg);
+    picked_bn = bn; picked_kb = kb; picked_sched = mode == MODE_GEMM ? (pp ? 2 : 1) : 0;
     return PF_OK;
   }
-  int launch_tma(int mode, const TmaMaps& maps, const TmaGemmParams& p, int bn, int kb, const PredTail* pred = nullptr) {
+  int launch_tma(int mode, const TmaMaps& maps, const TmaGemmParams& p, int bn, int kb, bool pp, const PredTail* pred = nullptr) {
     if (e->profile) {
       pf_engine::ProfRec r{};
       for (cudaEvent_t* ev : {&r.a, &r.b}) {
@@ -359,14 +361,14 @@
       r.cfg = mode == MODE_GEMM ? 5 : 6;
       r.M = (int)Mrows; r.N = p.N; r.K = p.K; r.KH = mode == MODE_GEMM ? 1 : 3; r.stride = 1; r.groups = p.groups; r.Cin = p.Cin;
       CU(cudaEventRecord(r.a, st));
-      if (mode == MODE_GEMM) LAUNCHED(gemm_tma_gemm_mode(maps, p, bn, kb, e->sm_count, st, pred));
-      else LAUNCHED(gemm_tma_halo_mode(maps, p, bn, kb, e->sm_count, st, pred));
+      if (mode == MODE_GEMM) LAUNCHED(gemm_tma_gemm_mode(maps, p, bn, kb, pp, e->sm_count, st, pred));
+      else LAUNCHED(gemm_tma_halo_mode(maps, p, bn, kb, pp, e->sm_count, st, pred));
       CU(cudaEventRecord(r.b, st));
       e->prof.push_back(r);
       return PF_OK;
     }
-    if (mode == MODE_GEMM) LAUNCHED(gemm_tma_gemm_mode(maps, p, bn, kb, e->sm_count, st, pred));
-    else LAUNCHED(gemm_tma_halo_mode(maps, p, bn, kb, e->sm_count, st, pred));
+    if (mode == MODE_GEMM) LAUNCHED(gemm_tma_gemm_mode(maps, p, bn, kb, pp, e->sm_count, st, pred));
+    else LAUNCHED(gemm_tma_halo_mode(maps, p, bn, kb, pp, e->sm_count, st, pred));
     return PF_OK;
   }
   struct Epi {
@@ -413,15 +415,17 @@
     fill_epi(p, w, o, 0);
     TmaMaps maps{};
     int bn, kb;
-    TRY(pick_tile(MODE_GEMM, p, nullptr, bn, kb));
+    bool pp;
+    TRY(pick_tile(MODE_GEMM, p, nullptr, bn, kb, pp));
     const char* msg = nullptr;
-    if (!msg) msg = map2d(&maps.a_hi, A.hi, A.ld, M, A.ld, 128, kb);
-    if (!msg) msg = map2d(&maps.a_lo, A.lo, A.ld, M, A.ld, 128, kb);
+    const int a_rows = pp ? 64 : 128;
+    if (!msg) msg = map2d(&maps.a_hi, A.hi, A.ld, M, A.ld, a_rows, kb);
+    if (!msg) msg = map2d(&maps.a_lo, A.lo, A.ld, M, A.ld, a_rows, kb);
     if (!msg) msg = map2d(&maps.b_hi, w.hi, K, N, K, bn, kb);
     if (!msg) msg = map2d(&maps.b_lo, w.lo, K, N, K, bn, kb);
     if (msg) return fail(PF_ERR_CUDA, "%s", msg);
     maps.a2_hi = maps.a_hi; maps.a2_lo = maps.a_lo;
-    return launch_tma(MODE_GEMM, maps, p, bn, kb);
+    return launch_tma(MODE_GEMM, maps, p, bn, kb, pp);
   }
   int thalo(const SplitT& A, int a_c0, int a_gc, const SplitT* A2, int c_split, int a2_c0, int B, int H, int W, int Cin, const GemmW& w, int N,
             int groups, int bias_gstride, const Epi& o, const PredTail* pred = nullptr) {
@@ -434,7 +438,8 @@
     fill_epi(p, w, o, bias_gstride);
     TmaMaps maps{};
     int bn, kb;
-    TRY(pick_tile(MODE_HALO, p, pred, bn, kb));
+    bool pp;
+    TRY(pick_tile(MODE_HALO, p, pred, bn, kb, pp));
     const char* msg = nullptr;
     if (!msg) msg = map_halo(&maps.a_hi, A.hi, B, H, W, A.ld);
     if (!msg) msg = map_halo(&maps.a_lo, A.lo, B, H, W, A.ld);
@@ -445,7 +450,7 @@
     if (!msg) msg = map2d(&maps.b_hi, w.hi, p.K, (long long)groups * N, p.K, bn, kb);
     if (!msg) msg = map2d(&maps.b_lo, w.lo, p.K, (long long)groups * N, p.K, bn, kb);
     if (msg) return fail(PF_ERR_CUDA, "%s", msg);
-    return launch_tma(MODE_HALO, maps, p, bn, kb, pred);
+    return launch_tma(MODE_HALO, maps, p, bn, kb, pp, pred);
   }
   int tconv_gather(const SplitT& A, int B, int H, int W, int Cin, int KH, int stride, int pad, const GemmW& w, int N, const Epi& o) {
     const int OH = (H + 2 * pad - KH) / stride + 1, OW = (W + 2 * pad - KH) / stride + 1;
@@ -1323,7 +1328,8 @@
   tmp.device = dev;
   tmp.sm_count = prop.multiProcessorCount;
   Fwd F{&tmp, Arena{}, (cudaStream_t)stream, false, q.B};
-  F.force_bn = q.force_bn; F.force_kb = q.force_kb;
+  if (q.force_sched < 0 || q.force_sched > 2 || (q.force_sched && q.mode != MODE_GEMM)) return fail(PF_ERR_ARG, "pf_op_tma: force_sched %d", q.force_sched);
+  F.force_bn = q.force_bn; F.force_kb = q.force_kb; F.force_sched = q.force_sched;
   const SplitT A{(__nv_bfloat16*)q.a_hi, (__nv_bfloat16*)q.a_lo, q.lda};
   const SplitT A2{(__nv_bfloat16*)q.a2_hi, (__nv_bfloat16*)q.a2_lo, q.lda2};
   const GemmW w{(const __nv_bfloat16*)q.w_hi, (const __nv_bfloat16*)q.w_lo, q.bias};
@@ -1340,11 +1346,11 @@
     if (!s.w || !s.b || !s.out || !(s.mode == 1 ? s.nc == 2 : (s.mode == 2 && s.nc == 1))) return fail(PF_ERR_ARG, "pf_op_tma: prediction tail %d", g);
     pt[g] = PredTail{s.w, s.b, s.out, s.nc, s.mode};
   }
-  op->picked_bn = op->picked_kb = 0;
+  op->picked_bn = op->picked_kb = op->picked_sched = 0;
   const int r = q.mode == MODE_GEMM ? F.tgemm(A, q.M, q.K, q.a_c0, w, q.N, o)
                                     : F.thalo(A, q.a_c0, q.a_gc, q.a2_hi ? &A2 : nullptr, q.c_split, q.a2_c0, q.B, q.H, q.W, q.Cin, w, q.N, q.groups,
                                               q.bias_gstride, o, q.npred ? pt : nullptr);
-  if (r == PF_OK) { op->picked_bn = F.picked_bn; op->picked_kb = F.picked_kb; }
+  if (r == PF_OK) { op->picked_bn = F.picked_bn; op->picked_kb = F.picked_kb; op->picked_sched = F.picked_sched; }
   return r;
 }
 int pf_op_conv1_ring(const void* c_hi, const void* c_lo, int B, int H, int W, const float* wf, const float* bias, float* out,
diff --git a/perspectivefields_b200/csrc/tc_ptx.cuh b/perspectivefields_b200/csrc/tc_ptx.cuh
--- a/perspectivefields_b200/csrc/tc_ptx.cuh
+++ b/perspectivefields_b200/csrc/tc_ptx.cuh
@@ -41,24 +41,110 @@
 }
 
 #define PF_R8(i) "+f"(d[i]), "+f"(d[i + 1]), "+f"(d[i + 2]), "+f"(d[i + 3]), "+f"(d[i + 4]), "+f"(d[i + 5]), "+f"(d[i + 6]), "+f"(d[i + 7])
-__device__ __forceinline__ void wgmma_n64(float* d, uint64_t adesc, uint64_t bdesc, uint32_t scale_d) {
-  asm volatile(
+template <int N> struct Wgmma;
+template <> struct Wgmma<32> {
+  static __device__ __forceinline__ void mma(float* d, uint64_t adesc, uint64_t bdesc, uint32_t scale_d) {
+    asm volatile(
+      "{\n\t.reg .pred p;\n\tsetp.ne.b32 p, %18, 0;\n\t"
+      "wgmma.mma_async.sync.aligned.m64n32k16.f32.bf16.bf16 {"
+      "%0,%1,%2,%3,%4,%5,%6,%7,%8,%9,%10,%11,%12,%13,%14,%15"
+      "}, %16, %17, p, 1, 1, 0, 0;\n\t}\n"
+      : PF_R8(0), PF_R8(8)
+      : "l"(adesc), "l"(bdesc), "r"(scale_d));
+  }
+};
+template <> struct Wgmma<64> {
+  static __device__ __forceinline__ void mma(float* d, uint64_t adesc, uint64_t bdesc, uint32_t scale_d) {
+    asm volatile(
       "{\n\t.reg .pred p;\n\tsetp.ne.b32 p, %34, 0;\n\t"
-      "wgmma.mma_async.sync.aligned.m64n64k16.f32.bf16.bf16 "
-      "{%0,%1,%2,%3,%4,%5,%6,%7,%8,%9,%10,%11,%12,%13,%14,%15,%16,%17,%18,%19,%20,%21,%22,%23,%24,%25,%26,%27,%28,%29,%30,%31}, "
-      "%32, %33, p, 1, 1, 0, 0;\n\t}\n"
+      "wgmma.mma_async.sync.aligned.m64n64k16.f32.bf16.bf16 {"
+      "%0,%1,%2,%3,%4,%5,%6,%7,%8,%9,%10,%11,%12,%13,%14,%15,%16,%17,%18,%19,%20,%21,%22,%23,%24,%25,%26,%27,%28,%29,%30,%31"
+      "}, %32, %33, p, 1, 1, 0, 0;\n\t}\n"
       : PF_R8(0), PF_R8(8), PF_R8(16), PF_R8(24)
       : "l"(adesc), "l"(bdesc), "r"(scale_d));
-}
-__device__ __forceinline__ void wgmma_n32(float* d, uint64_t adesc, uint64_t bdesc, uint32_t scale_d) {
-  asm volatile(
-      "{\n\t.reg .pred p;\n\tsetp.ne.b32 p, %18, 0;\n\t"
-      "wgmma.mma_async.sync.aligned.m64n32k16.f32.bf16.bf16 "
-      "{%0,%1,%2,%3,%4,%5,%6,%7,%8,%9,%10,%11,%12,%13,%14,%15}, %16, %17, p, 1, 1, 0, 0;\n\t}\n"
-      : PF_R8(0), PF_R8(8)
+  }
+};
+template <> struct Wgmma<96> {
+  static __device__ __forceinline__ void mma(float* d, uint64_t adesc, uint64_t bdesc, uint32_t scale_d) {
+    asm volatile(
+      "{\n\t.reg .pred p;\n\tsetp.ne.b32 p, %50, 0;\n\t"
+      "wgmma.mma_async.sync.aligned.m64n96k16.f32.bf16.bf16 {"
+      "%0,%1,%2,%3,%4,%5,%6,%7,%8,%9,%10,%11,%12,%13,%14,%15,%16,%17,%18,%19,%20,%21,%22,%23,%24,%25,%26,%27,%28,%29,%30,%31,"
+      "%32,%33,%34,%35,%36,%37,%38,%39,%40,%41,%42,%43,%44,%45,%46,%47"
+      "}, %48, %49, p, 1, 1, 0, 0;\n\t}\n"
+      : PF_R8(0), PF_R8(8), PF_R8(16), PF_R8(24), PF_R8(32), PF_R8(40)
       : "l"(adesc), "l"(bdesc), "r"(scale_d));
-}
+  }
+};
+template <> struct Wgmma<128> {
+  static __device__ __forceinline__ void mma(float* d, uint64_t adesc, uint64_t bdesc, uint32_t scale_d) {
+    asm volatile(
+      "{\n\t.reg .pred p;\n\tsetp.ne.b32 p, %66, 0;\n\t"
+      "wgmma.mma_async.sync.aligned.m64n128k16.f32.bf16.bf16 {"
+      "%0,%1,%2,%3,%4,%5,%6,%7,%8,%9,%10,%11,%12,%13,%14,%15,%16,%17,%18,%19,%20,%21,%22,%23,%24,%25,%26,%27,%28,%29,%30,%31,"
+      "%32,%33,%34,%35,%36,%37,%38,%39,%40,%41,%42,%43,%44,%45,%46,%47,%48,%49,%50,%51,%52,%53,%54,%55,%56,%57,%58,%59,%60,%61,%62,%63"
+      "}, %64, %65, p, 1, 1, 0, 0;\n\t}\n"
+      : PF_R8(0), PF_R8(8), PF_R8(16), PF_R8(24), PF_R8(32), PF_R8(40), PF_R8(48), PF_R8(56)
+      : "l"(adesc), "l"(bdesc), "r"(scale_d));
+  }
+};
+template <> struct Wgmma<160> {
+  static __device__ __forceinline__ void mma(float* d, uint64_t adesc, uint64_t bdesc, uint32_t scale_d) {
+    asm volatile(
+      "{\n\t.reg .pred p;\n\tsetp.ne.b32 p, %82, 0;\n\t"
+      "wgmma.mma_async.sync.aligned.m64n160k16.f32.bf16.bf16 {"
+      "%0,%1,%2,%3,%4,%5,%6,%7,%8,%9,%10,%11,%12,%13,%14,%15,%16,%17,%18,%19,%20,%21,%22,%23,%24,%25,%26,%27,%28,%29,%30,%31,"
+      "%32,%33,%34,%35,%36,%37,%38,%39,%40,%41,%42,%43,%44,%45,%46,%47,%48,%49,%50,%51,%52,%53,%54,%55,%56,%57,%58,%59,%60,%61,%62,%63,"
+      "%64,%65,%66,%67,%68,%69,%70,%71,%72,%73,%74,%75,%76,%77,%78,%79"
+      "}, %80, %81, p, 1, 1, 0, 0;\n\t}\n"
+      : PF_R8(0), PF_R8(8), PF_R8(16), PF_R8(24), PF_R8(32), PF_R8(40), PF_R8(48), PF_R8(56), PF_R8(64), PF_R8(72)
+      : "l"(adesc), "l"(bdesc), "r"(scale_d));
+  }
+};
+template <> struct Wgmma<192> {
+  static __device__ __forceinline__ void mma(float* d, uint64_t adesc, uint64_t bdesc, uint32_t scale_d) {
+    asm volatile(
+      "{\n\t.reg .pred p;\n\tsetp.ne.b32 p, %98, 0;\n\t"
+      "wgmma.mma_async.sync.aligned.m64n192k16.f32.bf16.bf16 {"
+      "%0,%1,%2,%3,%4,%5,%6,%7,%8,%9,%10,%11,%12,%13,%14,%15,%16,%17,%18,%19,%20,%21,%22,%23,%24,%25,%26,%27,%28,%29,%30,%31,"
+      "%32,%33,%34,%35,%36,%37,%38,%39,%40,%41,%42,%43,%44,%45,%46,%47,%48,%49,%50,%51,%52,%53,%54,%55,%56,%57,%58,%59,%60,%61,%62,%63,"
+      "%64,%65,%66,%67,%68,%69,%70,%71,%72,%73,%74,%75,%76,%77,%78,%79,%80,%81,%82,%83,%84,%85,%86,%87,%88,%89,%90,%91,%92,%93,%94,%95"
+      "}, %96, %97, p, 1, 1, 0, 0;\n\t}\n"
+      : PF_R8(0), PF_R8(8), PF_R8(16), PF_R8(24), PF_R8(32), PF_R8(40), PF_R8(48), PF_R8(56), PF_R8(64), PF_R8(72), PF_R8(80), PF_R8(88)
+      : "l"(adesc), "l"(bdesc), "r"(scale_d));
+  }
+};
+template <> struct Wgmma<224> {
+  static __device__ __forceinline__ void mma(float* d, uint64_t adesc, uint64_t bdesc, uint32_t scale_d) {
+    asm volatile(
+      "{\n\t.reg .pred p;\n\tsetp.ne.b32 p, %114, 0;\n\t"
+      "wgmma.mma_async.sync.aligned.m64n224k16.f32.bf16.bf16 {"
+      "%0,%1,%2,%3,%4,%5,%6,%7,%8,%9,%10,%11,%12,%13,%14,%15,%16,%17,%18,%19,%20,%21,%22,%23,%24,%25,%26,%27,%28,%29,%30,%31,"
+      "%32,%33,%34,%35,%36,%37,%38,%39,%40,%41,%42,%43,%44,%45,%46,%47,%48,%49,%50,%51,%52,%53,%54,%55,%56,%57,%58,%59,%60,%61,%62,%63,"
+      "%64,%65,%66,%67,%68,%69,%70,%71,%72,%73,%74,%75,%76,%77,%78,%79,%80,%81,%82,%83,%84,%85,%86,%87,%88,%89,%90,%91,%92,%93,%94,%95,"
+      "%96,%97,%98,%99,%100,%101,%102,%103,%104,%105,%106,%107,%108,%109,%110,%111"
+      "}, %112, %113, p, 1, 1, 0, 0;\n\t}\n"
+      : PF_R8(0), PF_R8(8), PF_R8(16), PF_R8(24), PF_R8(32), PF_R8(40), PF_R8(48), PF_R8(56), PF_R8(64), PF_R8(72), PF_R8(80), PF_R8(88), PF_R8(96), PF_R8(104)
+      : "l"(adesc), "l"(bdesc), "r"(scale_d));
+  }
+};
+template <> struct Wgmma<256> {
+  static __device__ __forceinline__ void mma(float* d, uint64_t adesc, uint64_t bdesc, uint32_t scale_d) {
+    asm volatile(
+      "{\n\t.reg .pred p;\n\tsetp.ne.b32 p, %130, 0;\n\t"
+      "wgmma.mma_async.sync.aligned.m64n256k16.f32.bf16.bf16 {"
+      "%0,%1,%2,%3,%4,%5,%6,%7,%8,%9,%10,%11,%12,%13,%14,%15,%16,%17,%18,%19,%20,%21,%22,%23,%24,%25,%26,%27,%28,%29,%30,%31,"
+      "%32,%33,%34,%35,%36,%37,%38,%39,%40,%41,%42,%43,%44,%45,%46,%47,%48,%49,%50,%51,%52,%53,%54,%55,%56,%57,%58,%59,%60,%61,%62,%63,"
+      "%64,%65,%66,%67,%68,%69,%70,%71,%72,%73,%74,%75,%76,%77,%78,%79,%80,%81,%82,%83,%84,%85,%86,%87,%88,%89,%90,%91,%92,%93,%94,%95,"
+      "%96,%97,%98,%99,%100,%101,%102,%103,%104,%105,%106,%107,%108,%109,%110,%111,%112,%113,%114,%115,%116,%117,%118,%119,%120,%121,%122,%123,%124,%125,%126,%127"
+      "}, %128, %129, p, 1, 1, 0, 0;\n\t}\n"
+      : PF_R8(0), PF_R8(8), PF_R8(16), PF_R8(24), PF_R8(32), PF_R8(40), PF_R8(48), PF_R8(56), PF_R8(64), PF_R8(72), PF_R8(80), PF_R8(88), PF_R8(96), PF_R8(104), PF_R8(112), PF_R8(120)
+      : "l"(adesc), "l"(bdesc), "r"(scale_d));
+  }
+};
 #undef PF_R8
+template <int N>
+__device__ __forceinline__ void wgmma_bf16(float* d, uint64_t adesc, uint64_t bdesc, uint32_t scale_d) { Wgmma<N>::mma(d, adesc, bdesc, scale_d); }
 
 template <int KB>
 __device__ __forceinline__ uint64_t wgmma_tile_desc(uint32_t smem_addr) {
diff --git a/perspectivefields_b200/csrc/tma_host.cuh b/perspectivefields_b200/csrc/tma_host.cuh
--- a/perspectivefields_b200/csrc/tma_host.cuh
+++ b/perspectivefields_b200/csrc/tma_host.cuh
@@ -84,13 +84,18 @@
   kb = tma_pick_kb(bn, K, mode);
 }
 
+constexpr int kPingPongKMax = 512;
+inline bool tma_pick_pingpong(long long M, int N, int K, int bn, int sm_count) {
+  return K <= kPingPongKMax && cdivl(M, 64) * cdiv(N, bn) >= 2LL * sm_count;
+}
+
 struct PredTail { const float* w; const float* b; float* out; int nc, mode; };
 
-template <int BN, int MODE, int KB>
+template <int BN, int MODE, int KB, bool PP = false>
 inline cudaError_t gemm_tma_launch_bn(const TmaMaps& maps, const TmaGemmParams& p, int sm_count, cudaStream_t st, const PredTail* pred) {
-  using Cfg = TmaCfg<BN, MODE, KB>;
+  using Cfg = TmaCfg<BN, MODE, KB, PP>;
   const int tiles_x = MODE == MODE_HALO ? cdiv(p.W, kHtTileW) : 0, tiles_y = MODE == MODE_HALO ? cdiv(p.H, kHtTileH) : 0;
-  const long long m_tiles = MODE == MODE_GEMM ? cdiv(p.M, 128) : (long long)p.B * tiles_x * tiles_y;
+  const long long m_tiles = MODE == MODE_GEMM ? cdiv(p.M, Cfg::kTileM) : (long long)p.B * tiles_x * tiles_y;
   const long long total = m_tiles * cdiv(p.N, BN) * p.groups;
   const unsigned grid = (unsigned)(total < sm_count ? total : sm_count);
   if (MODE == MODE_HALO && ((p.Cin == 64 && 9 * (64 / KB) <= Cfg::kStages && (p.groups > 1 || cdiv(p.N, BN) > 1)) || pred)) {
@@ -112,13 +117,15 @@
       }
     return last;
   }
-  return launch_pdl(gemm_tma_kernel<BN, MODE, KB>, dim3(grid), dim3(kTmaThreads), Cfg::kSmemBytes, st, maps, p, tiles_x, tiles_y);
+  return launch_pdl(gemm_tma_kernel<BN, MODE, KB, PP>, dim3(grid), dim3(kTmaThreads), Cfg::kSmemBytes, st, maps, p, tiles_x, tiles_y);
 }
 
 #define PF_TMA_VARIANTS(X)                                                                                                  \
   X(256, MODE_GEMM, 32) X(224, MODE_GEMM, 32) X(192, MODE_GEMM, 32) X(160, MODE_GEMM, 32) X(128, MODE_GEMM, 32) X(96, MODE_GEMM, 32) \
   X(64, MODE_GEMM, 32) X(32, MODE_GEMM, 32) X(64, MODE_GEMM, 64) X(32, MODE_GEMM, 64)                                        \
   X(256, MODE_HALO, 32) X(128, MODE_HALO, 64) X(64, MODE_HALO, 64) X(32, MODE_HALO, 64)
+#define PF_TMA_PINGPONG_VARIANTS(X)                                                                                         \
+  X(256, 32) X(224, 32) X(192, 32) X(160, 32) X(128, 32) X(96, 32) X(64, 32) X(32, 32) X(64, 64) X(32, 64)
 
 inline cudaError_t gemm_tma_configure_device() {
   cudaError_t e = cudaSuccess;
@@ -126,19 +133,26 @@
   if (e == cudaSuccess) e = cudaFuncSetAttribute(gemm_tma_kernel<BN_, MODE_, KB_>, cudaFuncAttributeMaxDynamicSharedMemorySize, TmaCfg<BN_, MODE_, KB_>::kSmemBytes);
   PF_TMA_VARIANTS(PF_TMA_CFG)
 #undef PF_TMA_CFG
+#define PF_TMA_CFG_PP(BN_, KB_)                                                                                               \
+  if (e == cudaSuccess) e = cudaFuncSetAttribute(gemm_tma_kernel<BN_, MODE_GEMM, KB_, true>, cudaFuncAttributeMaxDynamicSharedMemorySize, TmaCfg<BN_, MODE_GEMM, KB_, true>::kSmemBytes);
+  PF_TMA_PINGPONG_VARIANTS(PF_TMA_CFG_PP)
+#undef PF_TMA_CFG_PP
   return e;
 }
 
-inline int tma_stages(int mode, int bn, int kb) {
-#define PF_TMA_NS(BN_, MODE_, KB_) if (mode == MODE_ && bn == BN_ && kb == KB_) return TmaCfg<BN_, MODE_, KB_>::kStages;
+inline int tma_stages(int mode, int bn, int kb, bool pp = false) {
+#define PF_TMA_NS(BN_, MODE_, KB_) if (!pp && mode == MODE_ && bn == BN_ && kb == KB_) return TmaCfg<BN_, MODE_, KB_>::kStages;
   PF_TMA_VARIANTS(PF_TMA_NS)
 #undef PF_TMA_NS
+#define PF_TMA_NS_PP(BN_, KB_) if (pp && mode == MODE_GEMM && bn == BN_ && kb == KB_) return TmaCfg<BN_, MODE_GEMM, KB_, true>::kStages;
+  PF_TMA_PINGPONG_VARIANTS(PF_TMA_NS_PP)
+#undef PF_TMA_NS_PP
   return 0;
 }
 
-inline const char* gemm_tma_check(int mode, const TmaGemmParams& p, int bn, int kb, bool pred) {
-  const int ns = tma_stages(mode, bn, kb);
-  if (!ns) return "no engine instantiation for this (mode, bn, kb)";
+inline const char* gemm_tma_check(int mode, const TmaGemmParams& p, int bn, int kb, bool pred, bool pp = false) {
+  const int ns = tma_stages(mode, bn, kb, pp);
+  if (!ns) return pp ? "no ping-pong engine instantiation for this (mode, bn, kb)" : "no engine instantiation for this (mode, bn, kb)";
   if (mode == MODE_GEMM) return p.K % kb ? "GEMM mode: K must be a multiple of the K step" : nullptr;
   if (p.phase4 && (p.N != 128 || bn != 128)) return "phase4 needs N = 128 in one 128-wide tile";
   if (pred && bn != (p.phase4 ? 128 : 32)) return "the fused prediction tail needs N = 32 (phase4: 128) in one tile";
@@ -147,11 +161,14 @@
   return nullptr;
 }
 
-inline cudaError_t gemm_tma_launch(int mode,const TmaMaps& maps, const TmaGemmParams& p, int bn, int kb, int sm_count, cudaStream_t st,
+inline cudaError_t gemm_tma_launch(int mode, const TmaMaps& maps, const TmaGemmParams& p, int bn, int kb, bool pp, int sm_count, cudaStream_t st,
                                    const PredTail* pred = nullptr) {
-#define PF_TMA_CASE(BN_, MODE_, KB_) if (mode == MODE_ && bn == BN_ && kb == KB_) return gemm_tma_launch_bn<BN_, MODE_, KB_>(maps, p, sm_count, st, pred);
+#define PF_TMA_CASE(BN_, MODE_, KB_) if (!pp && mode == MODE_ && bn == BN_ && kb == KB_) return gemm_tma_launch_bn<BN_, MODE_, KB_>(maps, p, sm_count, st, pred);
   PF_TMA_VARIANTS(PF_TMA_CASE)
 #undef PF_TMA_CASE
+#define PF_TMA_CASE_PP(BN_, KB_) if (pp && mode == MODE_GEMM && bn == BN_ && kb == KB_) return gemm_tma_launch_bn<BN_, MODE_GEMM, KB_, true>(maps, p, sm_count, st, pred);
+  PF_TMA_PINGPONG_VARIANTS(PF_TMA_CASE_PP)
+#undef PF_TMA_CASE_PP
   return cudaErrorInvalidValue;
 }
 
```

After: 790.4, median of 6. 1.17x the previous value.
